# kazuto1011/dusty-gan-v2

Hardware: AMD Instinct MI355X
Metric: range-images/sec (G+D step) on dusty_v2 64x512 (higher is better)
Workload: dtype bf16; 1 GPU; configs[2]: configs/gans/dusty_v2.yaml full G+D train step (G step + D step + lazy R1 + ADA + EMA + Adam), 64x512 synthetic; global_batch=64, per_gpu_batch=64, parallelism=dp1, hip_graph=True, d_epilogue_dtype=fp32, pe_table_precomputed=True

## Files before the change

dusty-gan-v2_amd/csrc/api.hip:

```cpp
#include "common.h"

extern "C" int dgv2_abi_version(void) { return 49; }
```

dusty-gan-v2_amd/csrc/common.h:

```cpp
#pragma once
#include <hip/hip_runtime.h>
#include <stdint.h>
#include <stdlib.h>

#include "../../include/dgv2.h"

typedef __bf16 bf16_t;
typedef __attribute__((ext_vector_type(8))) __bf16 bf16x8;
typedef __attribute__((ext_vector_type(4))) float f32x4;
typedef __attribute__((ext_vector_type(4))) short s16x4;
typedef __attribute__((ext_vector_type(8))) short s16x8;

#define DGV2_WAVE 64

template <int DT> struct dtype_of;
template <> struct dtype_of<DGV2_F32> { typedef float type; };
template <> struct dtype_of<DGV2_BF16> { typedef bf16_t type; };

__device__ __forceinline__ float to_f32(float v) { return v; }
__device__ __forceinline__ float to_f32(bf16_t v) { return (float)v; }
template <typename T> __device__ __forceinline__ T from_f32(float v);
template <> __device__ __forceinline__ float from_f32<float>(float v) { return v; }
template <> __device__ __forceinline__ bf16_t from_f32<bf16_t>(float v) { return (bf16_t)v; }

template <typename T> struct vec16 {
  static constexpr int N = 16 / sizeof(T);
  union {
    uint4 raw;
    T e[16 / sizeof(T)];
  };
  __device__ __forceinline__ void load(const T* p) { raw = *reinterpret_cast<const uint4*>(p); }
  __device__ __forceinline__ void store(T* p) const { *reinterpret_cast<uint4*>(p) = raw; }
  __device__ __forceinline__ void store_nt(T* p) const {
    typedef __attribute__((ext_vector_type(4))) unsigned u32x4;
    const u32x4 v = {raw.x, raw.y, raw.z, raw.w};
    __builtin_nontemporal_store(v, reinterpret_cast<u32x4*>(p));
  }
  __device__ __forceinline__ float get(int i) const { return to_f32(e[i]); }
  __device__ __forceinline__ void set(int i, float v) { e[i] = from_f32<T>(v); }
};

__device__ __forceinline__ int pack_pair_bf16(const float (&va)[4], const float (&vb)[4], int lc, uint4& out) {
  union { uint2 u; bf16_t e[4]; } pa, pb;
#pragma unroll
  for (int r = 0; r < 4; ++r) {
    pa.e[r] = (bf16_t)va[r];
    pb.e[r] = (bf16_t)vb[r];
  }
  const auto lo = __builtin_amdgcn_permlane16_swap(pa.u.x, pb.u.x, false, false);
  const auto hi = __builtin_amdgcn_permlane16_swap(pa.u.y, pb.u.y, false, false);
  out = make_uint4(lo[0], hi[0], lo[1], hi[1]);
  const bool odd = lc & 1;
  return odd ? 16 + 4 * (lc - 1) : 4 * lc;
}

struct fp8_t { uint8_t v; };
#define DGV2_FP8_MAX 448.0f
__device__ __forceinline__ uint2 pack_fp8x8(const float (&f)[8]) {
  float c[8];
#pragma unroll
  for (int i = 0; i < 8; ++i) c[i] = fminf(fmaxf(f[i], -DGV2_FP8_MAX), DGV2_FP8_MAX);
  int lo = __builtin_amdgcn_cvt_pk_fp8_f32(c[0], c[1], 0, false);
  lo = __builtin_amdgcn_cvt_pk_fp8_f32(c[2], c[3], lo, true);
  int hi = __builtin_amdgcn_cvt_pk_fp8_f32(c[4], c[5], 0, false);
  hi = __builtin_amdgcn_cvt_pk_fp8_f32(c[6], c[7], hi, true);
  return make_uint2((unsigned)lo, (unsigned)hi);
}
__device__ __forceinline__ void unpack_fp8x4(unsigned w, float (&f)[4]) {
  typedef __attribute__((ext_vector_type(2))) float f32x2_;
  const f32x2_ a = __builtin_amdgcn_cvt_pk_f32_fp8((int)w, false), b = __builtin_amdgcn_cvt_pk_f32_fp8((int)w, true);
  f[0] = a[0]; f[1] = a[1]; f[2] = b[0]; f[3] = b[1];
}

static inline bool aligned16(const void* p) { return (reinterpret_cast<uintptr_t>(p) & 15) == 0; }

__host__ __device__ __forceinline__ int floordiv(int a, int b) {
  int q = a / b;
  return (a % b != 0 && ((a < 0) != (b < 0))) ? q - 1 : q;
}
__host__ __device__ __forceinline__ int floormod(int a, int b) {
  int r = a % b;
  return r < 0 ? r + b : r;
}

__device__ __forceinline__ float wave_sum(float v) {
#pragma unroll
  for (int o = 32; o > 0; o >>= 1) v += __shfl_xor(v, o, 64);
  return v;
}

__device__ __forceinline__ float block_sum(float v, float* red) {
  v = wave_sum(v);
  if ((threadIdx.x & 63) == 0) red[threadIdx.x >> 6] = v;
  __syncthreads();
  float s = 0.f;
  if (threadIdx.x == 0)
    for (int i = 0; i < (int)(blockDim.x >> 6); ++i) s += red[i];
  return s;
}

__device__ __forceinline__ float sumsq_bf16x8(uint4 q) {
  const unsigned w[4] = {q.x, q.y, q.z, q.w};
  float s = 0.f;
#pragma unroll
  for (int i = 0; i < 4; ++i) {
    const float lo = __uint_as_float(w[i] << 16), hi = __uint_as_float(w[i] & 0xffff0000u);
    s = fmaf(lo, lo, s);
    s = fmaf(hi, hi, s);
  }
  return s;
}

#define DGV2_RETURN_LAST()                 \
  do {                                     \
    hipError_t e__ = hipGetLastError();    \
    return (int)e__;                       \
  } while (0)

#define DGV2_DISPATCH_DTYPE(dtype, ...)                      \
  do {                                                       \
    if ((dtype) == DGV2_F32) {                               \
      typedef float T;                                       \
      __VA_ARGS__;                                           \
    } else if ((dtype) == DGV2_BF16) {                       \
      typedef bf16_t T;                                      \
      __VA_ARGS__;                                           \
    } else {                                                 \
      return DGV2_EINVAL;                                    \
    }                                                        \
  } while (0)

static __global__ void dgv2_zero_kernel(uint32_t* __restrict__ p, size_t n) {
  for (size_t i = blockIdx.x * (size_t)blockDim.x + threadIdx.x; i < n; i += (size_t)gridDim.x * blockDim.x) p[i] = 0u;
}
static inline hipError_t dgv2_zero_async(void* p, size_t bytes, hipStream_t st) {
  const size_t n = bytes / 4;
  if (n == 0) return hipSuccess;
  size_t g = (n + 255) / 256;
  if (g > 1024) g = 1024;
  dgv2_zero_kernel<<<(int)g, 256, 0, st>>>(reinterpret_cast<uint32_t*>(p), n);
  return hipGetLastError();
}
#define hipMemsetAsync(p, value, bytes, st) dgv2_zero_async((p), (bytes), (st))

static inline bool nt_output(int64_t bytes) {
  static const int64_t min_mb = getenv("DGV2_NT_MIN_MB") ? atoll(getenv("DGV2_NT_MIN_MB")) : 64;
  return min_mb > 0 && bytes >= (min_mb << 20);
}

static inline int grid_for(int64_t work, int block, int cap = 256 * 16) {
  int64_t g = (work + block - 1) / block;
  if (g > cap) g = cap;
  if (g < 1) g = 1;
  return (int)g;
}
```

dusty-gan-v2_amd/csrc/fir_mfma.hip:

```cpp
#include <type_traits>

#include "gemm_core.h"

namespace {

constexpr int FM_CT = 32;
constexpr int FM_CB = 32;
constexpr int FM_WIN = FM_CT + 16;
#ifndef DGV2_FIR_RS
#define DGV2_FIR_RS 8
#endif
constexpr int FM_RS = DGV2_FIR_RS;
constexpr int FM_RING = 2 * FM_RS;
static_assert(FM_RS == 8 || FM_RS == 4, "rows per step");
constexpr int FM_XBYTES = FM_RS * FM_WIN * 64;
constexpr int FM_ZROW = 2048 + 64;
constexpr int FM_ZBYTES = FM_RING * FM_ZROW;
constexpr int FM_YROW = 2048 + 16;
constexpr int FM_YBYTES = FM_RS * FM_YROW;
constexpr int FM_NLD = FM_RS * FM_WIN * 4 / 256;

struct FMGeom {
  int B, C, H, W, nt;
  const uint4* bands;
  const bf16_t* ref;
  float alpha, ascale;
  float* partial;
  uint8_t* y8;
};

struct FMTabs {
  int H, W, Eh, Ew;
  const int* idx_h; const float* coef_h; const int* cnt_h;
  const int* idx_w; const float* coef_w; const int* cnt_w;
  int* err;
};

typedef __attribute__((ext_vector_type(4))) unsigned fm_u32x4;
typedef __attribute__((address_space(3))) s16x4 fm_lds_s16x4;

__device__ __forceinline__ unsigned fm_pack2(float a, float b) {
  union { bf16_t h[2]; unsigned u; } p;
  p.h[0] = (bf16_t)a;
  p.h[1] = (bf16_t)b;
  return p.u;
}

__global__ __launch_bounds__(64) void fir_bands_kernel(uint4* __restrict__ bands, FMTabs t) {
  const int lane = threadIdx.x, li = lane & 15, kg = lane >> 4;
  const int nh = t.H / FM_RS + 1;
  float v[8];
#pragma unroll
  for (int j = 0; j < 8; ++j) v[j] = 0.f;
  bool bad = false;
  if ((int)blockIdx.x < nh) {
    const int s = blockIdx.x, ho = s * FM_RS - FM_RS / 2 + li;
    if (li < FM_RS && ho >= 0 && ho < t.H) {
      const int n = t.cnt_h[ho];
      for (int e = 0; e < n; ++e) {
        const int r = t.idx_h[ho * t.Eh + e];
        const float cf = t.coef_h[ho * t.Eh + e];
        if (r < s * FM_RS - FM_RS || r >= s * FM_RS + FM_RS || r < 0 || r >= t.H) bad = true;
#pragma unroll
        for (int j = 0; j < 8; ++j)
          if ((r & (FM_RING - 1)) == 8 * kg + j) v[j] += cf;
      }
    }
  } else {
    const int wt = blockIdx.x - nh, wo = 16 * wt + li;
    const int n = t.cnt_w[wo];
    for (int e = 0; e < n; ++e) {
      int rel = t.idx_w[wo * t.Ew + e] - (16 * wt - 8);
      rel = rel < 0 ? rel + t.W : (rel >= t.W ? rel - t.W : rel);
      const float cf = t.coef_w[wo * t.Ew + e];
      if ((unsigned)rel >= 32u) bad = true;
#pragma unroll
      for (int j = 0; j < 8; ++j)
        if (rel == 8 * kg + j) v[j] += cf;
    }
  }
#pragma unroll
  for (int j = 0; j < 8; ++j)
    if ((float)(bf16_t)v[j] != v[j]) bad = true;
  bands[(int64_t)blockIdx.x * 64 + lane] =
      make_uint4(fm_pack2(v[0], v[1]), fm_pack2(v[2], v[3]), fm_pack2(v[4], v[5]), fm_pack2(v[6], v[7]));
  if (bad) atomicOr(t.err, DGV2_STATUS_FIR_TABLE);
}

template <bool ACT>
__global__ __launch_bounds__(256, 2) void fir_same_mfma_kernel(bf16_t* __restrict__ y, const bf16_t* __restrict__ x, FMGeom g) {
  extern __shared__ __attribute__((aligned(16))) unsigned char smem[];
  unsigned char* Xs = smem;
  unsigned char* Zs = Xs + FM_XBYTES;
  unsigned char* Ys = Zs + FM_ZBYTES;
  const int tid = threadIdx.x, wave = tid >> 6, lane = tid & 63;
  const int li = lane & 15, kg = lane >> 4;
  const int q = li >> 2, p = li & 3;
  int vid = blockIdx.x + gridDim.x * (blockIdx.y + gridDim.y * blockIdx.z);
  {
    const int nblk = gridDim.x * gridDim.y * gridDim.z;
    if ((nblk & 7) == 0) vid = (vid & 7) * (nblk >> 3) + (vid >> 3);
  }
  const int c0col = (vid % (int)gridDim.x) * FM_CT;
  const int cb0 = ((vid / (int)gridDim.x) % (int)gridDim.y) * FM_CB;
  const int b = vid / (int)(gridDim.x * gridDim.y);
  const int64_t img = (int64_t)b * g.H * g.W * g.C;
  const bf16_t* xb = x + img;

  for (int i = tid; i < FM_ZBYTES / 16; i += 256) reinterpret_cast<uint4*>(Zs)[i] = make_uint4(0, 0, 0, 0);
  const int nsteps = g.H / FM_RS;
  const uint4* bands_h = g.bands;
  uint4 tw[2];
  tw[0] = g.bands[(int64_t)(nsteps + 1 + c0col / 16) * 64 + lane];
  tw[1] = g.bands[(int64_t)(nsteps + 2 + c0col / 16) * 64 + lane];

  int goff[FM_NLD];
  int xoff[FM_NLD];
#pragma unroll
  for (int i = 0; i < FM_NLD; ++i) {
    const int id = tid + 256 * i;
    const int o8 = id & 3, j = (id >> 2) % FM_WIN, r = id / (4 * FM_WIN);
    int gc = c0col - 8 + j;
    gc = gc < 0 ? gc + g.W : (gc >= g.W ? gc - g.W : gc);
    goff[i] = gc * g.C + cb0 + o8 * 8;
    xoff[i] = ((r * FM_WIN + j) * 4 + (o8 ^ (((j >> 3) & 1) << 1))) * 16;
  }
  fm_u32x4 rg[FM_NLD];
  auto issue = [&](int s) {
#pragma unroll
    for (int i = 0; i < FM_NLD; ++i) {
      const int r = (tid + 256 * i) / (4 * FM_WIN);
      rg[i] = *reinterpret_cast<const fm_u32x4*>(xb + (int64_t)(s * FM_RS + r) * g.W * g.C + goff[i]);
    }
  };
  auto commit = [&]() {
#pragma unroll
    for (int i = 0; i < FM_NLD; ++i) *reinterpret_cast<fm_u32x4*>(Xs + xoff[i]) = rg[i];
  };
  issue(0);
  commit();
  if (1 < nsteps) issue(1);
  uint4 th = bands_h[lane];
  __syncthreads();

  float bsum[8];
#pragma unroll
  for (int j = 0; j < 8; ++j) bsum[j] = 0.f;

  for (int s = 0; s <= nsteps; ++s) {
    if (s < nsteps) {
      uint4 af[FM_RS];
#pragma unroll
      for (int job = 0; job < FM_RS; ++job) {
        const int rr = job >> 2, ct = (job >> 1) & 1, wt = job & 1;
        const int r = (FM_RS / 4) * wave + rr;
        const int j = 16 * wt + 8 * kg + q;
        const int o8 = (2 * ct + (p >> 1)) ^ ((kg & 1) << 1);
        const unsigned char* a0 = Xs + ((r * FM_WIN + j) * 4 + o8) * 16 + (p & 1) * 8;
        union { uint4 u; s16x4 h[2]; } a;
        a.h[0] = __builtin_amdgcn_ds_read_tr16_b64_v4i16((fm_lds_s16x4*)a0);
        a.h[1] = __builtin_amdgcn_ds_read_tr16_b64_v4i16((fm_lds_s16x4*)(a0 + 4 * 64));
        af[job] = a.u;
      }
      f32x4 acc[FM_RS];
#pragma unroll
      for (int job = 0; job < FM_RS; ++job) {
        acc[job] = (f32x4){0.f, 0.f, 0.f, 0.f};
        Mfma16<bf16_t>::run(acc[job], af[job], tw[job & 1]);
      }
#pragma unroll
      for (int job = 0; job < FM_RS; ++job) {
        const int rr = job >> 2, ct = (job >> 1) & 1, wt = job & 1;
        const int slot = (s * FM_RS + (FM_RS / 4) * wave + rr) & (FM_RING - 1);
        const int wp = 16 * wt + li;
        const int u = (4 * ct + kg) ^ ((wp >> 2) & 7) ^ ((slot >> 3) << 2);
        uint2 pk = make_uint2(fm_pack2(acc[job][0], acc[job][1]), fm_pack2(acc[job][2], acc[job][3]));
        *reinterpret_cast<uint2*>(Zs + slot * FM_ZROW + wp * 64 + u * 8) = pk;
      }
    }
    __syncthreads();
    if (s + 1 < nsteps) commit();
    if (s + 2 < nsteps) issue(s + 2);
    const uint4 th_next = bands_h[(int64_t)min(s + 1, nsteps) * 64 + lane];
    vec16<bf16_t> fref[FM_RS / 2];
    if constexpr (ACT) {
#pragma unroll
      for (int i = 0; i < FM_RS / 2; ++i) {
        const int id = tid + 256 * i;
        const int ho = min(max(s * FM_RS - FM_RS / 2 + (id >> 7), 0), g.H - 1);
        fref[i].load(g.ref + img + ((int64_t)ho * g.W + c0col + ((id >> 2) & 31)) * g.C + cb0 + (id & 3) * 8);
      }
    }

    {
      uint4 af[16];
#pragma unroll
      for (int job = 0; job < 16; ++job) {
        const int wp = 8 * wave + (job >> 1), ct = job & 1;
        const int hi = FM_RS == 8 ? (kg & 1) : 0;
        const int slot = 8 * hi + q;
        const int u = (4 * ct + p) ^ ((wp >> 2) & 7) ^ (hi << 2);
        const unsigned char* a0 = Zs + slot * FM_ZROW + wp * 64 + u * 8;
        union { uint4 u4; s16x4 h[2]; } a;
        a.h[0] = __builtin_amdgcn_ds_read_tr16_b64_v4i16((fm_lds_s16x4*)a0);
        a.h[1] = __builtin_amdgcn_ds_read_tr16_b64_v4i16((fm_lds_s16x4*)(a0 + 4 * FM_ZROW));
        af[job] = a.u4;
      }
      f32x4 acc[16];
#pragma unroll
      for (int job = 0; job < 16; ++job) {
        acc[job] = (f32x4){0.f, 0.f, 0.f, 0.f};
        Mfma16<bf16_t>::run(acc[job], af[job], th);
      }
      if (li < FM_RS) {
#pragma unroll
        for (int job = 0; job < 16; ++job) {
          const int wp = 8 * wave + (job >> 1), ct = job & 1;
          uint2 pk = make_uint2(fm_pack2(acc[job][0], acc[job][1]), fm_pack2(acc[job][2], acc[job][3]));
          *reinterpret_cast<uint2*>(Ys + li * FM_YROW + wp * 64 + (4 * ct + kg) * 8) = pk;
        }
      }
    }
    __syncthreads();

#pragma unroll
    for (int i = 0; i < FM_RS / 2; ++i) {
      const int id = tid + 256 * i;
      const int o8 = id & 3, px = (id >> 2) & 31, n = id >> 7;
      const int ho = s * FM_RS - FM_RS / 2 + n;
      if (ho < 0 || ho >= g.H) continue;
      vec16<bf16_t> o;
      o.raw = *reinterpret_cast<const uint4*>(Ys + n * FM_YROW + px * 64 + o8 * 16);
      const int64_t off = img + ((int64_t)ho * g.W + c0col + px) * g.C + cb0 + o8 * 8;
      if constexpr (ACT) {
#pragma unroll
        for (int j = 0; j < 8; ++j) {
          const float a = o.get(j);
          o.set(j, (fref[i].get(j) > 0.f ? a : a * g.alpha) * g.ascale);
          bsum[j] += o.get(j);
        }
      }
      if constexpr (!ACT) {
        if (g.y8) {
          float f[8];
#pragma unroll
          for (int j = 0; j < 8; ++j) f[j] = o.get(j);
          *reinterpret_cast<uint2*>(g.y8 + off) = pack_fp8x8(f);
          continue;
        }
      }
      if (g.nt) o.store_nt(y + off);
      else o.store(y + off);
    }
    th = th_next;
  }

  if constexpr (ACT) {
    float* fold = reinterpret_cast<float*>(Xs);
    __syncthreads();
#pragma unroll
    for (int j = 0; j < 8; ++j) fold[tid * 8 + j] = bsum[j];
    __syncthreads();
    if (tid < FM_CB) {
      const int o8 = tid >> 3, j = tid & 7;
      float s2 = 0.f;
      for (int t = o8; t < 256; t += 4) s2 += fold[t * 8 + j];
      g.partial[((int64_t)b * gridDim.x + c0col / FM_CT) * g.C + cb0 + tid] = s2;
    }
  }
}

__global__ __launch_bounds__(256) void fm_bias_reduce_kernel(float* __restrict__ gb, const float* __restrict__ partial,
                                                             int nblk, int C) {
  __shared__ float red[16];
  const int c = blockIdx.x;
  float s = 0.f;
#pragma unroll 4
  for (int k = threadIdx.x; k < nblk; k += 256) s += partial[(int64_t)k * C + c];
  s = block_sum(s, red);
  if (threadIdx.x == 0) gb[c] = s;
}

bool fm_covers(int B, int C, int H, int W) {
  return B > 0 && C % FM_CB == 0 && H % FM_RS == 0 && H >= FM_RS && W % FM_CT == 0 && W >= FM_CT && B < 65536 &&
         C / FM_CB < 65536;
}

constexpr size_t FM_LDS = (size_t)FM_XBYTES + FM_ZBYTES + FM_YBYTES;

int64_t fm_band_bytes(int H, int W) { return 1024 * ((int64_t)H / FM_RS + 1 + W / 16); }

}

extern "C" int dgv2_fir_same_mfma_prep(void* bands, int64_t bands_bytes, int64_t* bytes_needed, const int* idx_h,
                                       const float* coef_h, const int* cnt_h, int Eh, const int* idx_w, const float* coef_w,
                                       const int* cnt_w, int Ew, int H, int W, int* status, void* stream) {
  if (H < FM_RS || H % FM_RS || W < FM_CT || W % FM_CT || Eh < 1 || Ew < 1) return DGV2_ENOTSUP;
  const int64_t need = fm_band_bytes(H, W);
  if (bytes_needed) *bytes_needed = need;
  if (!bands) return bytes_needed ? 0 : DGV2_EINVAL;
  if (bands_bytes < need || !aligned16(bands) || !idx_h || !coef_h || !cnt_h || !idx_w || !coef_w || !cnt_w) return DGV2_EINVAL;
  if (!status) return DGV2_EINVAL;
  FMTabs t{H, W, Eh, Ew, idx_h, coef_h, cnt_h, idx_w, coef_w, cnt_w, status};
  fir_bands_kernel<<<(int)(need / 1024), 64, 0, (hipStream_t)stream>>>((uint4*)bands, t);
  DGV2_RETURN_LAST();
}

extern "C" int dgv2_fir_same_mfma(void* y, const void* x, const void* bands, int B, int C, int H, int W, void* stream) {
  if (!y || !x || !bands) return DGV2_EINVAL;
  if (!fm_covers(B, C, H, W)) return DGV2_ENOTSUP;
  if (!aligned16(x) || !aligned16(y) || !aligned16(bands)) return DGV2_EINVAL;
  FMGeom g{B, C, H, W, nt_output((int64_t)B * H * W * C * 2) ? 1 : 0, (const uint4*)bands, nullptr, 1.f, 1.f, nullptr, nullptr};
  auto kern = fir_same_mfma_kernel<false>;
  if (FM_LDS > 64 * 1024) {
    hipError_t e = hipFuncSetAttribute((const void*)kern, hipFuncAttributeMaxDynamicSharedMemorySize, (int)FM_LDS);
    if (e != hipSuccess) return (int)e;
  }
  kern<<<dim3(W / FM_CT, C / FM_CB, B), 256, FM_LDS, (hipStream_t)stream>>>((bf16_t*)y, (const bf16_t*)x, g);
  DGV2_RETURN_LAST();
}

extern "C" int dgv2_fir_same_mfma_q8(void* y8, const void* x, const void* bands, int B, int C, int H, int W, void* stream) {
  if (!y8 || !x || !bands) return DGV2_EINVAL;
  if (!fm_covers(B, C, H, W)) return DGV2_ENOTSUP;
  if (!aligned16(x) || (reinterpret_cast<uintptr_t>(y8) & 7) || !aligned16(bands)) return DGV2_EINVAL;
  FMGeom g{B, C, H, W, 0, (const uint4*)bands, nullptr, 1.f, 1.f, nullptr, (uint8_t*)y8};
  auto kern = fir_same_mfma_kernel<false>;
  if (FM_LDS > 64 * 1024) {
    hipError_t e = hipFuncSetAttribute((const void*)kern, hipFuncAttributeMaxDynamicSharedMemorySize, (int)FM_LDS);
    if (e != hipSuccess) return (int)e;
  }
  kern<<<dim3(W / FM_CT, C / FM_CB, B), 256, FM_LDS, (hipStream_t)stream>>>((bf16_t*)nullptr, (const bf16_t*)x, g);
  DGV2_RETURN_LAST();
}

extern "C" int dgv2_fir_same_mfma_actbwd(void* y, float* gb, float* scratch, int64_t scratch_elems, int64_t* blocks_needed,
                                         const void* x, const void* ref, const void* bands, int B, int C, int H, int W,
                                         float alpha, float scale, void* stream) {
  if (!fm_covers(B, C, H, W)) return DGV2_ENOTSUP;
  const int64_t blocks = (int64_t)B * (W / FM_CT);
  if (blocks_needed) *blocks_needed = blocks;
  if (!scratch) return blocks_needed ? 0 : DGV2_EINVAL;
  if (!y || !gb || !x || !ref || !bands) return DGV2_EINVAL;
  if (scratch_elems < blocks * C || !aligned16(x) || !aligned16(y) || !aligned16(ref) || !aligned16(bands)) return DGV2_EINVAL;
  FMGeom g{B, C, H, W, 0, (const uint4*)bands, (const bf16_t*)ref, alpha, scale, scratch, nullptr};
  auto kern = fir_same_mfma_kernel<true>;
  if (FM_LDS > 64 * 1024) {
    hipError_t e = hipFuncSetAttribute((const void*)kern, hipFuncAttributeMaxDynamicSharedMemorySize, (int)FM_LDS);
    if (e != hipSuccess) return (int)e;
  }
  hipStream_t st = (hipStream_t)stream;
  kern<<<dim3(W / FM_CT, C / FM_CB, B), 256, FM_LDS, st>>>((bf16_t*)y, (const bf16_t*)x, g);
  fm_bias_reduce_kernel<<<C, 256, 0, st>>>(gb, scratch, (int)blocks, C);
  DGV2_RETURN_LAST();
}
```

dusty-gan-v2_amd/csrc/resample.hip:

```cpp
#include "common.h"

namespace {

constexpr int MAXE = 32;
constexpr int TH = 4;
constexpr int TW = 16;

struct AxisParams {
  int L;
  int Lo;
  int k, up, down, p0;
  int wrap;
};

struct SparseRow {
  int cnt;
  int idx[MAXE];
  float coef[MAXE];
};

__device__ __forceinline__ int extend(int j, int L, int wrap) {
  if (wrap) return floormod(j, L);
  return j < 0 ? 0 : (j >= L ? L - 1 : j);
}
// ... 109 lines not shown
extern "C" int dgv2_resample(void* y, const void* x, const float* taps_h, const float* taps_w, int B, int H, int W,
                             int C, int Ho, int Wo, int ldx, int ldy, int kh, int up_h, int down_h, int p0_h, int kw,
                             int up_w, int down_w, int p0_w, int ring, int adjoint, int dtype, void* stream) {
  if (!y || !x || !taps_h || !taps_w) return DGV2_EINVAL;
  if (B <= 0 || H <= 0 || W <= 0 || C <= 0 || Ho <= 0 || Wo <= 0) return DGV2_EINVAL;
  if (kh < 1 || kh > 8 || kw < 1 || kw > 8 || up_h < 1 || up_w < 1 || down_h < 1 || down_w < 1) return DGV2_EINVAL;
  if (ldx < C || ldy < C) return DGV2_EINVAL;
  AxisParams ah = {H, Ho, kh, up_h, down_h, p0_h, 0};
  AxisParams aw = {W, Wo, kw, up_w, down_w, p0_w, ring ? 1 : 0};
  const int in_h = adjoint ? Ho : H, in_w = adjoint ? Wo : W;
  const int out_h = adjoint ? H : Ho, out_w = adjoint ? W : Wo;
  const int tiles = B * ((out_h + TH - 1) / TH) * ((out_w + TW - 1) / TW);
  hipStream_t st = (hipStream_t)stream;
  DGV2_DISPATCH_DTYPE(dtype, {
    constexpr int VN = vec16<T>::N;
    const bool vec = (C % VN == 0) && (ldx % VN == 0) && (ldy % VN == 0) && aligned16(x) && aligned16(y);
    if (vec)
      resample_kernel<T, true><<<tiles, 256, 0, st>>>((T*)y, (const T*)x, taps_h, taps_w, B, C, ldx, ldy, ah, aw,
                                                     adjoint, in_h, in_w, out_h, out_w);
    else
      resample_kernel<T, false><<<tiles, 256, 0, st>>>((T*)y, (const T*)x, taps_h, taps_w, B, C, ldx, ldy, ah, aw,
                                                      adjoint, in_h, in_w, out_h, out_w);
  });
  DGV2_RETURN_LAST();
}

namespace {

template <typename T, int CC>
__global__ __launch_bounds__(256) void resample_tab_smallc_kernel(
    T* __restrict__ y, const T* __restrict__ x, const int* __restrict__ idx_h, const float* __restrict__ coef_h,
    const int* __restrict__ cnt_h, int Eh, const int* __restrict__ idx_w, const float* __restrict__ coef_w,
    const int* __restrict__ cnt_w, int Ew, int B, int in_h, int in_w, int out_h, int out_w,
    const T* __restrict__ resid = nullptr, const float* __restrict__ rscale = nullptr,
    const float* __restrict__ rbias = nullptr) {
  struct alignas(sizeof(T) * CC) Px { T e[CC]; };
  float rs[CC], rb[CC];
#pragma unroll
  for (int j = 0; j < CC; ++j) {
    rs[j] = rscale ? rscale[j] : 1.f;
    rb[j] = rbias ? rbias[j] : 0.f;
  }
  const int64_t total = (int64_t)B * out_h * out_w;
  for (int64_t t = blockIdx.x * (int64_t)blockDim.x + threadIdx.x; t < total; t += (int64_t)gridDim.x * blockDim.x) {
    const int wo = (int)(t % out_w);
    const int64_t r = t / out_w;
    const int ho = (int)(r % out_h);
    const int b = (int)(r / out_h);
    const int nh = cnt_h[ho], nw = cnt_w[wo];
    const Px* xb = reinterpret_cast<const Px*>(x) + (int64_t)b * in_h * in_w;
    float acc[CC];
#pragma unroll
    for (int j = 0; j < CC; ++j) acc[j] = 0.f;
    if (Eh <= 2 && Ew <= 2) {
      const int e1h = Eh > 1 ? 1 : 0, e1w = Ew > 1 ? 1 : 0;
      const int ih0 = idx_h[ho * Eh], ih1 = idx_h[ho * Eh + e1h], iw0 = idx_w[wo * Ew], iw1 = idx_w[wo * Ew + e1w];
      const float ch0 = coef_h[ho * Eh], ch1 = coef_h[ho * Eh + e1h], cw0 = coef_w[wo * Ew], cw1 = coef_w[wo * Ew + e1w];
      const bool h1 = nh > 1, w1 = nw > 1;
      const Px* r0 = xb + (int64_t)ih0 * in_w;
      const Px* r1 = xb + (int64_t)(h1 ? ih1 : ih0) * in_w;
      const Px v00 = r0[iw0], v01 = r0[w1 ? iw1 : iw0], v10 = r1[iw0], v11 = r1[w1 ? iw1 : iw0];
      const bool l0 = nh > 0 && nw > 0;
#pragma unroll
      for (int j = 0; j < CC; ++j) {
        float s = 0.f;
        if (l0) s += (ch0 * cw0) * to_f32(v00.e[j]);
        if (l0 && w1) s += (ch0 * cw1) * to_f32(v01.e[j]);
        if (l0 && h1) s += (ch1 * cw0) * to_f32(v10.e[j]);
        if (l0 && h1 && w1) s += (ch1 * cw1) * to_f32(v11.e[j]);
        acc[j] = s;
      }
    } else {
      for (int a = 0; a < nh; ++a) {
        const float fa = coef_h[ho * Eh + a];
        const Px* xr = xb + (int64_t)idx_h[ho * Eh + a] * in_w;
        for (int c = 0; c < nw; ++c) {
          const float cf = fa * coef_w[wo * Ew + c];
          const Px v = xr[idx_w[wo * Ew + c]];
#pragma unroll
          for (int j = 0; j < CC; ++j) acc[j] += cf * to_f32(v.e[j]);
        }
      }
    }
    Px o;
    if (resid) {
      const Px rv = reinterpret_cast<const Px*>(resid)[t];
#pragma unroll
      for (int j = 0; j < CC; ++j) {
        const float rj = rscale ? to_f32(from_f32<T>(fmaf(to_f32(rv.e[j]), rs[j], rb[j]))) : to_f32(rv.e[j]);
        o.e[j] = from_f32<T>(rj + to_f32(from_f32<T>(acc[j])));
      }
    } else {
#pragma unroll
      for (int j = 0; j < CC; ++j) o.e[j] = from_f32<T>(acc[j]);
    }
    reinterpret_cast<Px*>(y)[t] = o;
  }
}

template <typename T, bool VEC>
__global__ __launch_bounds__(256) void resample_tab_kernel(
    T* __restrict__ y, const T* __restrict__ x, const int* __restrict__ idx_h, const float* __restrict__ coef_h,
    const int* __restrict__ cnt_h, int Eh, const int* __restrict__ idx_w, const float* __restrict__ coef_w,
    const int* __restrict__ cnt_w, int Ew, int B, int C, int ldx, int ldy, int in_h, int in_w, int out_h, int out_w) {
  constexpr int VN = VEC ? vec16<T>::N : 1;
  const int cvecs = (C + VN - 1) / VN;
  const int64_t total = (int64_t)B * out_h * out_w * cvecs;
  for (int64_t t = blockIdx.x * (int64_t)blockDim.x + threadIdx.x; t < total; t += (int64_t)gridDim.x * blockDim.x) {
    const int cv = (int)(t % cvecs);
    int64_t r = t / cvecs;
    const int wo = (int)(r % out_w);
    r /= out_w;
    const int ho = (int)(r % out_h);
    const int b = (int)(r / out_h);
    const int nh = cnt_h[ho], nw = cnt_w[wo];
    const int* ih = idx_h + ho * Eh;
    const float* ch = coef_h + ho * Eh;
    const int* iw = idx_w + wo * Ew;
    const float* cw = coef_w + wo * Ew;
    const T* xb = x + (int64_t)b * in_h * in_w * ldx + cv * VN;
    float acc[VN];
#pragma unroll
    for (int j = 0; j < VN; ++j) acc[j] = 0.f;
    for (int a = 0; a < nh; ++a) {
      const float fa = ch[a];
      const T* xr = xb + (int64_t)ih[a] * in_w * ldx;
      for (int c = 0; c < nw; ++c) {
        const float cf = fa * cw[c];
        const T* p = xr + iw[c] * ldx;
        if (VEC) {
          vec16<T> v;
          v.load(p);
#pragma unroll
          for (int j = 0; j < VN; ++j) acc[j] += cf * v.get(j);
        } else {
          acc[0] += cf * to_f32(p[0]);
        }
      }
    }
    T* q = y + (((int64_t)b * out_h + ho) * out_w + wo) * ldy + cv * VN;
    if (VEC) {
      vec16<T> o;
#pragma unroll
      for (int j = 0; j < VN; ++j) o.set(j, acc[j]);
      o.store(q);
    } else {
      q[0] = from_f32<T>(acc[0]);
    }
  }
}

constexpr int RS_RB = 4;

template <typename T, int EW, bool ACT = false>
__global__ __launch_bounds__(256) void resample_stream_kernel(
    T* __restrict__ y, const T* __restrict__ x, const int* __restrict__ idx_h, const float* __restrict__ coef_h,
    const int* __restrict__ cnt_h, int Eh, const int* __restrict__ idx_w, const float* __restrict__ coef_w,
    const int* __restrict__ cnt_w, int Ew, int B, int C, int ldx, int ldy, int in_h, int in_w, int out_h, int out_w,
    int SHA, float* __restrict__ sumsq, const T* __restrict__ ref = nullptr, float alpha = 1.f, float ascale = 1.f,
    float* __restrict__ bias_partial = nullptr, uint8_t* __restrict__ y8 = nullptr) {
#ifdef DGV2_ABLATE
  const int SH = SHA & 0xffff, ablate = (SHA >> 16) & 0xff;
#else
  const int SH = SHA & 0xffff;
  constexpr int ablate = 0;
#endif
  const bool nt = (SHA >> 30) & 1;
  __shared__ float red[16];
  float ss = 0.f;
  constexpr int VN = vec16<T>::N;
  __shared__ uint4 ring[RS_RB][256];
  const int tid = threadIdx.x;
  const int cvecs = C / VN;
  const int rowvecs = out_w * cvecs;
  const int colblocks = (rowvecs + 255) / 256;
  const int strips = (out_h + SH - 1) / SH;
  int bid = blockIdx.x;
  const int cb = bid % colblocks; bid /= colblocks;
  const int strip = bid % strips;
  const int b = bid / strips;
  const int col = cb * 256 + tid;
  const bool live = col < rowvecs;
  const int wo = live ? col / cvecs : 0;
  const int cv = live ? col - wo * cvecs : 0;

  const int nw = live ? cnt_w[wo] : 0;
  int xo[EW];
  float cw[EW];
  const int xo_any = nw > 0 ? idx_w[wo * Ew] * ldx + cv * VN : 0;
#pragma unroll
  for (int c = 0; c < EW; ++c) {
    xo[c] = xo_any;
    cw[c] = 0.f;
    if (c < nw) {
      xo[c] = idx_w[wo * Ew + c] * ldx + cv * VN;
      cw[c] = coef_w[wo * Ew + c];
    }
  }
  const T* xb = x + (int64_t)b * in_h * in_w * ldx;
  T* yp = y + (int64_t)b * out_h * out_w * ldy + (int64_t)wo * ldy + cv * VN;
  const T* rp = ACT ? ref + (int64_t)b * out_h * out_w * ldy + (int64_t)wo * ldy + cv * VN : nullptr;
  float bsum[VN];
#pragma unroll
  for (int j = 0; j < VN; ++j) bsum[j] = 0.f;
  const int ho0 = strip * SH;
  const int ho1 = min(ho0 + SH, out_h);
  int t0 = -1, t1 = -1, t2 = -1, t3 = -1;
  const int lane = threadIdx.x & 63;
  const int nent = (ho1 - ho0) * Eh;
  const int tb_idx = lane < nent ? idx_h[ho0 * Eh + lane] : 0;
  const float tb_cf = lane < nent ? coef_h[ho0 * Eh + lane] : 0.f;
  const int tb_cnt = lane < ho1 - ho0 ? cnt_h[ho0 + lane] : 0;
  int rlast = -1;
  for (int i = 0; i < ho1 - ho0; ++i) {
    const int n = __builtin_amdgcn_readlane(tb_cnt, i);
    for (int a = 0; a < n; ++a) rlast = max(rlast, __builtin_amdgcn_readlane(tb_idx, i * Eh + a));
  }
  int pr = -1;
  vec16<T> pv[EW];
  auto issue = [&](int r) {
    const T* xr = xb + (int64_t)r * in_w * ldx;
#pragma unroll
    for (int c = 0; c < EW; ++c) pv[c].load(xr + xo[c]);
    pr = r;
  };
  for (int ho = ho0; ho < ho1; ++ho) {
    const int n = __builtin_amdgcn_readlane(tb_cnt, ho - ho0);
    float acc[VN];
#pragma unroll
    for (int j = 0; j < VN; ++j) acc[j] = 0.f;
    for (int a = 0; a < n; ++a) {
      const int e = (ho - ho0) * Eh + a;
      const int r = __builtin_amdgcn_readlane(tb_idx, e);
      const float fa = __int_as_float(__builtin_amdgcn_readlane(__float_as_int(tb_cf), e));
      const int s = r & (RS_RB - 1);
      const int tag = s == 0 ? t0 : (s == 1 ? t1 : (s == 2 ? t2 : t3));
      if (tag != r) {
        if (pr != r && !(ablate & 2)) issue(r);
        float h[VN];
#pragma unroll
        for (int j = 0; j < VN; ++j) h[j] = 0.f;
#pragma unroll
        for (int c = 0; c < EW; ++c)
#pragma unroll
          for (int j = 0; j < VN; ++j) h[j] += cw[c] * pv[c].get(j);
        if (r + 1 <= rlast && !(ablate & 2)) issue(r + 1); else pr = -1;
        {
          vec16<T> hv;
#pragma unroll
          for (int j = 0; j < VN; ++j) hv.set(j, h[j]);
          ring[s][tid] = hv.raw;
        }
        t0 = s == 0 ? r : t0; t1 = s == 1 ? r : t1; t2 = s == 2 ? r : t2; t3 = s == 3 ? r : t3;
      }
      {
        vec16<T> hv;
        hv.raw = ring[s][tid];
#pragma unroll
        for (int j = 0; j < VN; ++j) acc[j] += fa * hv.get(j);
      }
    }
    if (live && !((ablate & 1) && acc[0] != 12345.678f)) {
      vec16<T> o;
      if constexpr (ACT) {
        vec16<T> f;
        f.load(rp + (int64_t)ho * out_w * ldy);
#pragma unroll
        for (int j = 0; j < VN; ++j) {
          o.set(j, (f.get(j) > 0.f ? acc[j] : acc[j] * alpha) * ascale);
          bsum[j] += o.get(j);
        }
      } else {
#pragma unroll
        for (int j = 0; j < VN; ++j) o.set(j, acc[j]);
      }
      if (y) {
        if (nt) o.store_nt(yp + (int64_t)ho * out_w * ldy);
        else o.store(yp + (int64_t)ho * out_w * ldy);
      }
      if constexpr (!ACT && sizeof(T) == 2) {
        if (y8) {
          float f[8];
#pragma unroll
          for (int j = 0; j < 8; ++j) f[j] = acc[j];
          *reinterpret_cast<uint2*>(y8 + ((int64_t)b * out_h + ho) * out_w * ldy + (int64_t)wo * ldy + cv * VN) = pack_fp8x8(f);
        }
      }
      if (sumsq) {
#pragma unroll
        for (int j = 0; j < VN; ++j) ss = fmaf(o.get(j), o.get(j), ss);
      }
    }
  }
  if (sumsq) {
    const float s = block_sum(ss, red);
    if (tid == 0) sumsq[blockIdx.x] = s;
  }
  if constexpr (ACT) {
    float* fold = reinterpret_cast<float*>(&ring[0][0]);
    __syncthreads();
#pragma unroll
    for (int j = 0; j < VN; ++j) fold[tid * VN + j] = live ? bsum[j] : 0.f;
    __syncthreads();
    const int off = (cb * 256) % cvecs;
    for (int c = tid; c < C; c += 256) {
      const int v = c / VN, j = c - v * VN;
      float s2 = 0.f;
      for (int t = (v - off + cvecs) % cvecs; t < 256; t += cvecs) s2 += fold[t * VN + j];
      bias_partial[(int64_t)blockIdx.x * C + c] = s2;
    }
  }
}

template <typename T>
void rs_launch(int Ew, int blocks, hipStream_t st, T* y, const T* x, const int* idx_h, const float* coef_h,
               const int* cnt_h, int Eh, const int* idx_w, const float* coef_w, const int* cnt_w, int B, int C, int ldx,
               int ldy, int in_h, int in_w, int out_h, int out_w, int sha, float* sumsq) {
  switch (Ew) {
    case 1: resample_stream_kernel<T, 1><<<blocks, 256, 0, st>>>(y, x, idx_h, coef_h, cnt_h, Eh, idx_w, coef_w, cnt_w, Ew, B, C, ldx, ldy, in_h, in_w, out_h, out_w, sha, sumsq); break;
    case 2: resample_stream_kernel<T, 2><<<blocks, 256, 0, st>>>(y, x, idx_h, coef_h, cnt_h, Eh, idx_w, coef_w, cnt_w, Ew, B, C, ldx, ldy, in_h, in_w, out_h, out_w, sha, sumsq); break;
    case 3: resample_stream_kernel<T, 3><<<blocks, 256, 0, st>>>(y, x, idx_h, coef_h, cnt_h, Eh, idx_w, coef_w, cnt_w, Ew, B, C, ldx, ldy, in_h, in_w, out_h, out_w, sha, sumsq); break;
    default: resample_stream_kernel<T, 4><<<blocks, 256, 0, st>>>(y, x, idx_h, coef_h, cnt_h, Eh, idx_w, coef_w, cnt_w, Ew, B, C, ldx, ldy, in_h, in_w, out_h, out_w, sha, sumsq); break;
  }
}

template <typename T>
void rs_launch_act(int Ew, int blocks, hipStream_t st, T* y, const T* x, const int* idx_h, const float* coef_h,
                   const int* cnt_h, int Eh, const int* idx_w, const float* coef_w, const int* cnt_w, int B, int C,
                   int ldx, int ldy, int in_h, int in_w, int out_h, int out_w, int sha, const T* ref, float alpha,
                   float ascale, float* partial) {
  switch (Ew) {
    case 1: resample_stream_kernel<T, 1, true><<<blocks, 256, 0, st>>>(y, x, idx_h, coef_h, cnt_h, Eh, idx_w, coef_w, cnt_w, Ew, B, C, ldx, ldy, in_h, in_w, out_h, out_w, sha, nullptr, ref, alpha, ascale, partial); break;
    case 2: resample_stream_kernel<T, 2, true><<<blocks, 256, 0, st>>>(y, x, idx_h, coef_h, cnt_h, Eh, idx_w, coef_w, cnt_w, Ew, B, C, ldx, ldy, in_h, in_w, out_h, out_w, sha, nullptr, ref, alpha, ascale, partial); break;
    case 3: resample_stream_kernel<T, 3, true><<<blocks, 256, 0, st>>>(y, x, idx_h, coef_h, cnt_h, Eh, idx_w, coef_w, cnt_w, Ew, B, C, ldx, ldy, in_h, in_w, out_h, out_w, sha, nullptr, ref, alpha, ascale, partial); break;
    default: resample_stream_kernel<T, 4, true><<<blocks, 256, 0, st>>>(y, x, idx_h, coef_h, cnt_h, Eh, idx_w, coef_w, cnt_w, Ew, B, C, ldx, ldy, in_h, in_w, out_h, out_w, sha, nullptr, ref, alpha, ascale, partial); break;
  }
}

__global__ __launch_bounds__(256) void rs_bias_reduce_kernel(float* __restrict__ gb, const float* __restrict__ partial,
                                                             int nblk, int C) {
  __shared__ float red[16];
  const int c = blockIdx.x;
  float s = 0.f;
#pragma unroll 4
  for (int k = threadIdx.x; k < nblk; k += 256) s += partial[(int64_t)k * C + c];
  s = block_sum(s, red);
  if (threadIdx.x == 0) gb[c] = s;
}

}

extern "C" int dgv2_resample_tab_actbwd(void* y, float* gb, float* scratch, int64_t scratch_elems, int64_t* blocks_needed,
                                        const void* x, const void* ref, const int* idx_h, const float* coef_h,
                                        const int* cnt_h, int Eh, const int* idx_w, const float* coef_w,
                                        const int* cnt_w, int Ew, int B, int C, int in_h, int in_w, int out_h,
                                        int out_w, float alpha, float scale, int dtype, void* stream) {
  if (B <= 0 || C <= 0 || in_h <= 0 || in_w <= 0 || out_h <= 0 || out_w <= 0 || Eh <= 0 || Ew <= 0) return DGV2_EINVAL;
  const int vn = dtype == DGV2_BF16 ? 8 : (dtype == DGV2_F32 ? 4 : 0);
  if (!vn) return DGV2_EINVAL;
  if (C % vn || 256 % (C / vn) || Ew > 4 || Eh > 64) return DGV2_ENOTSUP;
  int SH = out_h >= 32 ? 16 : (out_h >= 8 ? 8 : out_h);
  while (SH > 1 && SH * Eh > 64) SH >>= 1;
  const int64_t blocks = (int64_t)B * ((out_h + SH - 1) / SH) * (((int64_t)out_w * (C / vn) + 255) / 256);
  if (blocks >= (1LL << 31)) return DGV2_ENOTSUP;
  if (blocks_needed) *blocks_needed = blocks;
  if (!scratch) return blocks_needed ? 0 : DGV2_EINVAL;
  if (!y || !gb || !x || !ref || !idx_h || !coef_h || !cnt_h || !idx_w || !coef_w || !cnt_w) return DGV2_EINVAL;
  if (scratch_elems < blocks * C || !aligned16(x) || !aligned16(y) || !aligned16(ref)) return DGV2_EINVAL;
  hipStream_t st = (hipStream_t)stream;
  DGV2_DISPATCH_DTYPE(dtype, {
    rs_launch_act<T>(Ew, (int)blocks, st, (T*)y, (const T*)x, idx_h, coef_h, cnt_h, Eh, idx_w, coef_w, cnt_w, B, C, C, C,
                     in_h, in_w, out_h, out_w, SH, (const T*)ref, alpha, scale, scratch);
  });
  rs_bias_reduce_kernel<<<C, 256, 0, st>>>(gb, scratch, (int)blocks, C);
  DGV2_RETURN_LAST();
}

extern "C" int dgv2_resample_tab(void* y, const void* x, const int* idx_h, const float* coef_h, const int* cnt_h,
                                 int Eh, const int* idx_w, const float* coef_w, const int* cnt_w, int Ew, int B,
                                 int C, int ldx, int ldy, int in_h, int in_w, int out_h, int out_w, int dtype,
                                 void* stream) {
  return dgv2_resample_tab_sq(y, x, idx_h, coef_h, cnt_h, Eh, idx_w, coef_w, cnt_w, Ew, B, C, ldx, ldy, in_h, in_w, out_h,
                              out_w, dtype, nullptr, 0, nullptr, stream);
}

extern "C" int dgv2_resample_tab_add(void* y, const void* x, const void* resid, const int* idx_h, const float* coef_h,
                                     const int* cnt_h, int Eh, const int* idx_w, const float* coef_w, const int* cnt_w,
                                     int Ew, int B, int C, int in_h, int in_w, int out_h, int out_w, int dtype,
                                     void* stream) {
  return dgv2_resample_tab_add_affine(y, x, resid, nullptr, nullptr, idx_h, coef_h, cnt_h, Eh, idx_w, coef_w, cnt_w, Ew, B, C,
                                      in_h, in_w, out_h, out_w, dtype, stream);
}

extern "C" int dgv2_resample_tab_add_affine(void* y, const void* x, const void* resid, const float* rscale,
                                            const float* rbias, const int* idx_h, const float* coef_h, const int* cnt_h,
                                            int Eh, const int* idx_w, const float* coef_w, const int* cnt_w, int Ew, int B,
                                            int C, int in_h, int in_w, int out_h, int out_w, int dtype, void* stream) {
  if ((!rscale) != (!rbias)) return DGV2_EINVAL;
  if (!y || !x || !resid || !idx_h || !coef_h || !cnt_h || !idx_w || !coef_w || !cnt_w) return DGV2_EINVAL;
  if (B <= 0 || C <= 0 || in_h <= 0 || in_w <= 0 || out_h <= 0 || out_w <= 0 || Eh <= 0 || Ew <= 0) return DGV2_EINVAL;
  if (!(C == 1 || C == 2 || C == 4)) return DGV2_ENOTSUP;
  hipStream_t st = (hipStream_t)stream;
  DGV2_DISPATCH_DTYPE(dtype, {
    const uintptr_t al = sizeof(T) * C;
    if (reinterpret_cast<uintptr_t>(x) % al || reinterpret_cast<uintptr_t>(y) % al || reinterpret_cast<uintptr_t>(resid) % al)
      return DGV2_ENOTSUP;
    const int g2 = grid_for((int64_t)B * out_h * out_w, 256, 256 * 64);
    if (C == 1) resample_tab_smallc_kernel<T, 1><<<g2, 256, 0, st>>>((T*)y, (const T*)x, idx_h, coef_h, cnt_h, Eh, idx_w, coef_w, cnt_w, Ew, B, in_h, in_w, out_h, out_w, (const T*)resid, rscale, rbias);
    else if (C == 2) resample_tab_smallc_kernel<T, 2><<<g2, 256, 0, st>>>((T*)y, (const T*)x, idx_h, coef_h, cnt_h, Eh, idx_w, coef_w, cnt_w, Ew, B, in_h, in_w, out_h, out_w, (const T*)resid, rscale, rbias);
    else resample_tab_smallc_kernel<T, 4><<<g2, 256, 0, st>>>((T*)y, (const T*)x, idx_h, coef_h, cnt_h, Eh, idx_w, coef_w, cnt_w, Ew, B, in_h, in_w, out_h, out_w, (const T*)resid, rscale, rbias);
  });
  DGV2_RETURN_LAST();
}

extern "C" int dgv2_resample_tab_q8(void* y8, const void* x, const int* idx_h, const float* coef_h, const int* cnt_h,
                                    int Eh, const int* idx_w, const float* coef_w, const int* cnt_w, int Ew, int B,
                                    int C, int in_h, int in_w, int out_h, int out_w, void* stream) {
  if (!y8 || !x || !idx_h || !coef_h || !cnt_h || !idx_w || !coef_w || !cnt_w) return DGV2_EINVAL;
  if (B <= 0 || C <= 0 || in_h <= 0 || in_w <= 0 || out_h <= 0 || out_w <= 0 || Eh <= 0 || Ew <= 0) return DGV2_EINVAL;
  if ((C & 7) || Ew > 4 || Eh > 64 || !aligned16(x) || (reinterpret_cast<uintptr_t>(y8) & 7)) return DGV2_ENOTSUP;
  typedef bf16_t T;
  int SH = out_h >= 32 ? 16 : (out_h >= 8 ? 8 : out_h);
  while (SH > 1 && SH * Eh > 64) SH >>= 1;
  const int64_t blocks = (int64_t)B * ((out_h + SH - 1) / SH) * (((int64_t)out_w * (C / 8) + 255) / 256);
  if (blocks >= (1LL << 31)) return DGV2_EINVAL;
  hipStream_t st = (hipStream_t)stream;
  uint8_t* q = (uint8_t*)y8;
#define DGV2_RS_Q8(EW)                                                                                                   \
  resample_stream_kernel<T, EW><<<(int)blocks, 256, 0, st>>>((T*)nullptr, (const T*)x, idx_h, coef_h, cnt_h, Eh, idx_w,   \
                                                            coef_w, cnt_w, Ew, B, C, C, C, in_h, in_w, out_h, out_w, SH,  \
                                                            nullptr, nullptr, 1.f, 1.f, nullptr, q)
  switch (Ew) {
    case 1: DGV2_RS_Q8(1); break;
    case 2: DGV2_RS_Q8(2); break;
    case 3: DGV2_RS_Q8(3); break;
    default: DGV2_RS_Q8(4); break;
  }
#undef DGV2_RS_Q8
  DGV2_RETURN_LAST();
}

extern "C" int dgv2_resample_tab_sq(void* y, const void* x, const int* idx_h, const float* coef_h, const int* cnt_h,
                                    int Eh, const int* idx_w, const float* coef_w, const int* cnt_w, int Ew, int B,
                                    int C, int ldx, int ldy, int in_h, int in_w, int out_h, int out_w, int dtype,
                                    float* sumsq, int sumsq_cap, int* sumsq_used, void* stream) {
  if (sumsq_used) *sumsq_used = 0;
  const bool stat_only = !y;
  if ((stat_only && !(sumsq && sumsq_used)) || !x || !idx_h || !coef_h || !cnt_h || !idx_w || !coef_w || !cnt_w) return DGV2_EINVAL;
  if (B <= 0 || C <= 0 || in_h <= 0 || in_w <= 0 || out_h <= 0 || out_w <= 0 || Eh <= 0 || Ew <= 0) return DGV2_EINVAL;
  if (ldx < C || ldy < C) return DGV2_EINVAL;
  hipStream_t st = (hipStream_t)stream;
  DGV2_DISPATCH_DTYPE(dtype, {
    constexpr int VN = vec16<T>::N;
    const bool vec = (C % VN == 0) && (ldx % VN == 0) && (ldy % VN == 0) && aligned16(x) && aligned16(y);
    if (stat_only && !(vec && Ew <= 4 && Eh <= 64)) return DGV2_ENOTSUP;
    const int64_t total = (int64_t)B * out_h * out_w * ((C + (vec ? VN : 1) - 1) / (vec ? VN : 1));
    const int grid = grid_for(total, 256, 256 * 64);
    static const bool no_stream = getenv("DGV2_NO_RSTREAM") != nullptr;
#ifdef DGV2_ABLATE
    static const int rs_ablate = getenv("DGV2_RS_ABLATE") ? atoi(getenv("DGV2_RS_ABLATE")) : 0;
#else
    constexpr int rs_ablate = 0;
#endif
    if (vec && Ew <= 4 && Eh <= 64 && (!no_stream || stat_only)) {
      static const int sh_env = getenv("DGV2_RS_SH") ? atoi(getenv("DGV2_RS_SH")) : 0;
      int SH = out_h >= 32 ? 16 : (out_h >= 8 ? 8 : out_h);
      if (sh_env > 0 && sh_env < SH) SH = sh_env;
      while (SH > 1 && SH * Eh > 64) SH >>= 1;
      const int64_t blocks = (int64_t)B * ((out_h + SH - 1) / SH) * (((int64_t)out_w * (C / VN) + 255) / 256);
      if (blocks >= (1LL << 31)) return DGV2_EINVAL;
      float* sq = (sumsq && sumsq_used && blocks <= sumsq_cap) ? sumsq : nullptr;
      if (stat_only && !sq) return DGV2_ENOTSUP;
      if (sq) *sumsq_used = (int)blocks;
      rs_launch<T>(Ew, (int)blocks, st, (T*)y, (const T*)x, idx_h, coef_h, cnt_h, Eh, idx_w, coef_w, cnt_w, B, C, ldx, ldy, in_h,
                   in_w, out_h, out_w,
                   SH | (rs_ablate << 16) | ((y && nt_output((int64_t)B * out_h * out_w * C * sizeof(T))) ? (1 << 30) : 0), sq);
    } else if (!vec && (C == 1 || C == 2 || C == 4) && ldx == C && ldy == C &&
               (reinterpret_cast<uintptr_t>(x) % (sizeof(T) * C)) == 0 && (reinterpret_cast<uintptr_t>(y) % (sizeof(T) * C)) == 0) {
      const int g2 = grid_for((int64_t)B * out_h * out_w, 256, 256 * 64);
      if (C == 1) resample_tab_smallc_kernel<T, 1><<<g2, 256, 0, st>>>((T*)y, (const T*)x, idx_h, coef_h, cnt_h, Eh, idx_w, coef_w, cnt_w, Ew, B, in_h, in_w, out_h, out_w);
      else if (C == 2) resample_tab_smallc_kernel<T, 2><<<g2, 256, 0, st>>>((T*)y, (const T*)x, idx_h, coef_h, cnt_h, Eh, idx_w, coef_w, cnt_w, Ew, B, in_h, in_w, out_h, out_w);
      else resample_tab_smallc_kernel<T, 4><<<g2, 256, 0, st>>>((T*)y, (const T*)x, idx_h, coef_h, cnt_h, Eh, idx_w, coef_w, cnt_w, Ew, B, in_h, in_w, out_h, out_w);
    } else if (vec)
      resample_tab_kernel<T, true><<<grid, 256, 0, st>>>((T*)y, (const T*)x, idx_h, coef_h, cnt_h, Eh, idx_w, coef_w,
                                                        cnt_w, Ew, B, C, ldx, ldy, in_h, in_w, out_h, out_w);
    else
      resample_tab_kernel<T, false><<<grid, 256, 0, st>>>((T*)y, (const T*)x, idx_h, coef_h, cnt_h, Eh, idx_w, coef_w,
                                                         cnt_w, Ew, B, C, ldx, ldy, in_h, in_w, out_h, out_w);
  });
  DGV2_RETURN_LAST();
}
```

dusty-gan-v2_amd/csrc/stem.hip:

```cpp
#include "common.h"

namespace {

struct StemGeom {
  int B, H, W, O, ring;
  float alpha, scale;
  int nt;
};

__device__ __forceinline__ int stem_wcoord(int w, int W, int ring) {
  if (ring) return w < 0 ? w + W : (w >= W ? w - W : w);
  return w < 0 ? 0 : (w >= W ? W - 1 : w);
}

__device__ __forceinline__ void stem_blur(const float* __restrict__ xb, int h, int w, const StemGeom& g, float& v,
                                          float& u) {
  const float c = xb[h * g.W + w];
  const float up = xb[(h > 0 ? h - 1 : 0) * g.W + w], dn = xb[(h + 1 < g.H ? h + 1 : g.H - 1) * g.W + w];
  const float lf = xb[h * g.W + stem_wcoord(w - 1, g.W, g.ring)], rt = xb[h * g.W + stem_wcoord(w + 1, g.W, g.ring)];
  v = 0.25f * (up + dn) + 0.5f * c;
  u = 0.25f * (lf + rt) + 0.5f * c;
}

template <typename T>
__global__ __launch_bounds__(256) void stem_fwd_kernel(T* __restrict__ y, const float* __restrict__ x,
                                                       const float* __restrict__ w, const float* __restrict__ bias,
                                                       StemGeom g) {
  const int G = g.O / 8;
  const int64_t items = (int64_t)g.B * g.H * g.W * G;
  const int64_t stride = (int64_t)gridDim.x * blockDim.x;
  int64_t i = (int64_t)blockIdx.x * blockDim.x + threadIdx.x;
  const int grp = (int)(i % G);
  float w0[8], w1[8], bs[8];
#pragma unroll
  for (int j = 0; j < 8; ++j) {
    w0[j] = w[(grp * 8 + j) * 2];
    w1[j] = w[(grp * 8 + j) * 2 + 1];
    bs[j] = bias ? bias[grp * 8 + j] : 0.f;
  }
  const int HW = g.H * g.W;
  for (; i < items; i += stride) {
    const int64_t px = i / G;
    const int b = (int)(px / HW), r = (int)(px - (int64_t)b * HW);
    const int h = r / g.W, wc = r - h * g.W;
    float v, u;
    stem_blur(x + (int64_t)b * HW, h, wc, g, v, u);
    T* out = y + px * g.O + grp * 8;
    float f[8];
#pragma unroll
    for (int j = 0; j < 8; ++j) {
      const float t = w0[j] * v + w1[j] * u + bs[j];
      f[j] = (t > 0.f ? t : t * g.alpha) * g.scale;
    }
    if constexpr (sizeof(T) == 2) {
      vec16<T> o;
#pragma unroll
      for (int j = 0; j < 8; ++j) o.set(j, f[j]);
      if (g.nt) o.store_nt(out);
      else o.store(out);
    } else {
      *reinterpret_cast<float4*>(out) = make_float4(f[0], f[1], f[2], f[3]);
      *reinterpret_cast<float4*>(out + 4) = make_float4(f[4], f[5], f[6], f[7]);
    }
  }
}

template <typename T>
__global__ __launch_bounds__(256) void stem_fwd4_kernel(T* __restrict__ y, const float* __restrict__ x,
                                                        const float* __restrict__ w, const float* __restrict__ bias,
                                                        StemGeom g) {
  const int G = g.O / 8, W4 = g.W >> 2;
  const int64_t items = (int64_t)g.B * g.H * W4 * G;
  const int64_t stride = (int64_t)gridDim.x * blockDim.x;
  int64_t i = (int64_t)blockIdx.x * blockDim.x + threadIdx.x;
  const int grp = (int)(i % G);
  float w0[8], w1[8], bs[8];
#pragma unroll
  for (int j = 0; j < 8; ++j) {
    w0[j] = w[(grp * 8 + j) * 2];
    w1[j] = w[(grp * 8 + j) * 2 + 1];
    bs[j] = bias ? bias[grp * 8 + j] : 0.f;
  }
  const int HW4 = g.H * W4;
  for (; i < items; i += stride) {
    const int64_t q = i / G;
    const int b = (int)(q / HW4), r = (int)(q - (int64_t)b * HW4);
    const int h = r / W4, wc = (r - h * W4) << 2;
    const float* xb = x + ((int64_t)b * g.H) * g.W;
    const float4 c4 = *reinterpret_cast<const float4*>(xb + h * g.W + wc);
    const float4 u4 = *reinterpret_cast<const float4*>(xb + (h > 0 ? h - 1 : 0) * g.W + wc);
    const float4 d4 = *reinterpret_cast<const float4*>(xb + (h + 1 < g.H ? h + 1 : g.H - 1) * g.W + wc);
    const float lf = xb[h * g.W + stem_wcoord(wc - 1, g.W, g.ring)], rt = xb[h * g.W + stem_wcoord(wc + 4, g.W, g.ring)];
    const float c[6] = {lf, c4.x, c4.y, c4.z, c4.w, rt};
    const float up[4] = {u4.x, u4.y, u4.z, u4.w}, dn[4] = {d4.x, d4.y, d4.z, d4.w};
    T* out = y + (((int64_t)b * g.H + h) * g.W + wc) * g.O + grp * 8;
#pragma unroll
    for (int k = 0; k < 4; ++k) {
      const float v = 0.25f * (up[k] + dn[k]) + 0.5f * c[k + 1];
      const float u = 0.25f * (c[k] + c[k + 2]) + 0.5f * c[k + 1];
      float f[8];
#pragma unroll
      for (int j = 0; j < 8; ++j) {
        const float t = w0[j] * v + w1[j] * u + bs[j];
        f[j] = (t > 0.f ? t : t * g.alpha) * g.scale;
      }
      if constexpr (sizeof(T) == 2) {
        vec16<T> o;
#pragma unroll
        for (int j = 0; j < 8; ++j) o.set(j, f[j]);
        if (g.nt) o.store_nt(out + k * g.O);
        else o.store(out + k * g.O);
      } else {
        *reinterpret_cast<float4*>(out + k * g.O) = make_float4(f[0], f[1], f[2], f[3]);
        *reinterpret_cast<float4*>(out + k * g.O + 4) = make_float4(f[4], f[5], f[6], f[7]);
      }
    }
  }
}

template <typename T>
struct StemSkip {
  const T* gsk;
  const int* idx_h; const float* coef_h; const int* cnt_h; int Eh;
  const int* idx_w; const float* coef_w; const int* cnt_w; int Ew;
  int Hs, Ws;
};

template <typename T, bool SKIP>
__global__ __launch_bounds__(256) void stem_bwd_kernel(float* __restrict__ partial, float* __restrict__ gxb,
                                                       const T* __restrict__ gy, const T* __restrict__ y,
                                                       const float* __restrict__ x, const float* __restrict__ w,
                                                       StemGeom g, StemSkip<T> sk) {
  __shared__ float red[4][8][24];
  extern __shared__ __attribute__((aligned(16))) unsigned char stem_tabs[];
  const int* t_ih = nullptr; const float* t_ch = nullptr; const int* t_iw = nullptr; const float* t_cw = nullptr;
  if constexpr (SKIP) {
    const int nh_ = g.H * sk.Eh, nw_ = g.W * sk.Ew;
    int* a0 = reinterpret_cast<int*>(stem_tabs);
    float* a1 = reinterpret_cast<float*>(a0 + nh_);
    int* a2 = reinterpret_cast<int*>(a1 + nh_);
    float* a3 = reinterpret_cast<float*>(a2 + nw_);
    for (int t = threadIdx.x; t < nh_; t += 256) {
      a0[t] = sk.idx_h[t];
      a1[t] = sk.coef_h[t];
    }
    for (int t = threadIdx.x; t < nw_; t += 256) {
      a2[t] = sk.idx_w[t];
      a3[t] = sk.coef_w[t];
    }
    __syncthreads();
    t_ih = a0; t_ch = a1; t_iw = a2; t_cw = a3;
  }
  const int G = g.O / 8;
  const int64_t items = (int64_t)g.B * g.H * g.W * G;
  const int64_t stride = (int64_t)gridDim.x * blockDim.x;
  int64_t i = (int64_t)blockIdx.x * blockDim.x + threadIdx.x;
  const int grp = (int)(i % G);
  float w0[8], w1[8];
#pragma unroll
  for (int j = 0; j < 8; ++j) {
    w0[j] = w[(grp * 8 + j) * 2];
    w1[j] = w[(grp * 8 + j) * 2 + 1];
  }
  float acc[24];
#pragma unroll
  for (int j = 0; j < 24; ++j) acc[j] = 0.f;
  const int HW = g.H * g.W;
  const int64_t nloop = (items + stride - 1) / stride;
  for (int64_t it = 0; it < nloop; ++it, i += stride) {
    const bool live = i < items;
    const int64_t px = live ? i / G : 0;
    const int b = (int)(px / HW), r = (int)(px - (int64_t)b * HW);
    const int h = r / g.W, wc = r - h * g.W;
    float v, u;
    stem_blur(x + (int64_t)b * HW, h, wc, g, v, u);
    float gp[8], gs[8];
#pragma unroll
    for (int j = 0; j < 8; ++j) gs[j] = 0.f;
    if constexpr (SKIP) {
      const T* sb = sk.gsk + (int64_t)b * sk.Hs * sk.Ws * g.O + grp * 8;
      const int* ihp = t_ih + h * sk.Eh;
      const float* chp = t_ch + h * sk.Eh;
      const int* iwp = t_iw + wc * sk.Ew;
      const float* cwp = t_cw + wc * sk.Ew;
      const int e1h = sk.Eh > 1 ? 1 : 0, e1w = sk.Ew > 1 ? 1 : 0;
      const float ch0 = chp[0], ch1 = sk.Eh > 1 ? chp[1] : 0.f, cw0 = cwp[0], cw1 = sk.Ew > 1 ? cwp[1] : 0.f;
      const T* r0 = sb + (int64_t)ihp[0] * sk.Ws * g.O;
      const T* r1 = sb + (int64_t)ihp[e1h] * sk.Ws * g.O;
      const int64_t c0 = (int64_t)iwp[0] * g.O, c1 = (int64_t)iwp[e1w] * g.O;
      auto acc8 = [&](const T* sp, float cf) {
        if constexpr (sizeof(T) == 2) {
          vec16<T> v8;
          v8.load(sp);
#pragma unroll
          for (int j = 0; j < 8; ++j) gs[j] = fmaf(cf, v8.get(j), gs[j]);
        } else {
#pragma unroll
          for (int j = 0; j < 8; ++j) gs[j] = fmaf(cf, (float)sp[j], gs[j]);
        }
      };
      acc8(r0 + c0, ch0 * cw0);
      acc8(r0 + c1, ch0 * cw1);
      acc8(r1 + c0, ch1 * cw0);
      acc8(r1 + c1, ch1 * cw1);
      for (int a = 0; a < sk.Eh; ++a)
        for (int c = 0; c < sk.Ew; ++c) {
          if (a < 2 && c < 2) continue;
          const float cf = chp[a] * cwp[c];
          if (cf != 0.f) acc8(sb + (int64_t)ihp[a] * sk.Ws * g.O + (int64_t)iwp[c] * g.O, cf);
        }
    }
    if constexpr (sizeof(T) == 2) {
      vec16<T> a, c;
      a.load(gy + px * g.O + grp * 8);
      c.load(y + px * g.O + grp * 8);
#pragma unroll
      for (int j = 0; j < 8; ++j) gp[j] = (a.get(j) + gs[j]) * (c.get(j) > 0.f ? 1.f : g.alpha) * g.scale;
    } else {
#pragma unroll
      for (int j = 0; j < 8; ++j) {
        const float a = gy[px * g.O + grp * 8 + j], c = y[px * g.O + grp * 8 + j];
        gp[j] = (a + gs[j]) * (c > 0.f ? 1.f : g.alpha) * g.scale;
      }
    }
    float s0 = 0.f, s1 = 0.f;
#pragma unroll
    for (int j = 0; j < 8; ++j) {
      const float p = live ? gp[j] : 0.f;
      acc[j] += p;
      acc[8 + j] += p * v;
      acc[16 + j] += p * u;
      s0 += p * w0[j];
      s1 += p * w1[j];
    }
    for (int o = 1; o < G; o <<= 1) {
      s0 += __shfl_xor(s0, o, 64);
      s1 += __shfl_xor(s1, o, 64);
    }
    if (live && grp == 0) *reinterpret_cast<float2*>(gxb + px * 2) = make_float2(s0, s1);
  }
  const int lane = threadIdx.x & 63, wave = threadIdx.x >> 6;
#pragma unroll
  for (int j = 0; j < 24; ++j) {
    float t = acc[j];
    for (int o = 32; o >= G; o >>= 1) t += __shfl_xor(t, o, 64);
    if (lane < G) red[wave][lane][j] = t;
  }
  __syncthreads();
  for (int t = threadIdx.x; t < G * 24; t += 256) {
    const int gi = t / 24, j = t % 24;
    const float s = red[0][gi][j] + red[1][gi][j] + red[2][gi][j] + red[3][gi][j];
    partial[(int64_t)blockIdx.x * 3 * g.O + (j / 8) * g.O + gi * 8 + (j & 7)] = s;
  }
}

__global__ __launch_bounds__(256) void stem_reduce_kernel(float* __restrict__ gw, float* __restrict__ gb,
                                                          const float* __restrict__ partial, int nblk, int O) {
  __shared__ float red[4];
  const int e = blockIdx.x;
  float s = 0.f;
  for (int k = threadIdx.x; k < nblk; k += 256) s += partial[(int64_t)k * 3 * O + e];
  s = wave_sum(s);
  if ((threadIdx.x & 63) == 0) red[threadIdx.x >> 6] = s;
  __syncthreads();
  if (threadIdx.x == 0) {
    const float t = red[0] + red[1] + red[2] + red[3];
    if (e < O) gb[e] = t;
    else gw[(e % O) * 2 + (e / O - 1)] = t;
  }
}

__global__ __launch_bounds__(256) void stem_blur_adj_kernel(float* __restrict__ gx, const float* __restrict__ gxb,
                                                            StemGeom g) {
  const int64_t n = (int64_t)g.B * g.H * g.W;
  const int HW = g.H * g.W;
  for (int64_t i = (int64_t)blockIdx.x * blockDim.x + threadIdx.x; i < n; i += (int64_t)gridDim.x * blockDim.x) {
    const int b = (int)(i / HW), r = (int)(i - (int64_t)b * HW);
    const int h = r / g.W, w = r - h * g.W;
    const float* gb = gxb + (int64_t)b * HW * 2;
    auto G0 = [&](int hh, int ww) { return gb[(hh * g.W + ww) * 2]; };
    auto G1 = [&](int hh, int ww) { return gb[(hh * g.W + ww) * 2 + 1]; };
    float s = 0.5f * G0(h, w);
    if (h > 0) s += 0.25f * G0(h - 1, w);
    if (h + 1 < g.H) s += 0.25f * G0(h + 1, w);
    if (h == 0) s += 0.25f * G0(0, w);
    if (h == g.H - 1) s += 0.25f * G0(g.H - 1, w);
    s += 0.5f * G1(h, w);
    if (g.ring) {
      s += 0.25f * (G1(h, w > 0 ? w - 1 : g.W - 1) + G1(h, w + 1 < g.W ? w + 1 : 0));
    } else {
      if (w > 0) s += 0.25f * G1(h, w - 1);
      if (w + 1 < g.W) s += 0.25f * G1(h, w + 1);
      if (w == 0) s += 0.25f * G1(h, 0);
      if (w == g.W - 1) s += 0.25f * G1(h, g.W - 1);
    }
    gx[i] = s;
  }
}

constexpr int STEM_BWD_BLOCKS = 1024;

bool stem_ok(int B, int H, int W, int O) {
  return B > 0 && H >= 2 && W >= 2 && (O == 8 || O == 16 || O == 32 || O == 64) && (int64_t)H * W < (1 << 30);
}

}

extern "C" int dgv2_stem_fwd(void* y, const float* x, const float* w, const float* bias, int B, int H, int W, int O,
                             int ring, float alpha, float scale, int ydtype, void* stream) {
  if (!y || !x || !w || !stem_ok(B, H, W, O) || !aligned16(y)) return DGV2_EINVAL;
  StemGeom g{B, H, W, O, ring, alpha, scale, nt_output((int64_t)B * H * W * O * (ydtype == DGV2_BF16 ? 2 : 4)) ? 1 : 0};
  hipStream_t st = (hipStream_t)stream;
  static const bool no4 = getenv("DGV2_STEM_NO4") != nullptr;
  if (W % 4 == 0 && aligned16(x) && !no4) {
    const int64_t items = (int64_t)B * H * (W / 4) * (O / 8);
    const int grid = grid_for(items, 256, 256 * 32);
    if (ydtype == DGV2_BF16) stem_fwd4_kernel<bf16_t><<<grid, 256, 0, st>>>((bf16_t*)y, x, w, bias, g);
    else if (ydtype == DGV2_F32) stem_fwd4_kernel<float><<<grid, 256, 0, st>>>((float*)y, x, w, bias, g);
    else return DGV2_EINVAL;
    DGV2_RETURN_LAST();
  }
  const int64_t items = (int64_t)B * H * W * (O / 8);
  const int grid = grid_for(items, 256, 256 * 32);
  if (ydtype == DGV2_BF16) stem_fwd_kernel<bf16_t><<<grid, 256, 0, st>>>((bf16_t*)y, x, w, bias, g);
  else if (ydtype == DGV2_F32) stem_fwd_kernel<float><<<grid, 256, 0, st>>>((float*)y, x, w, bias, g);
  else return DGV2_EINVAL;
  DGV2_RETURN_LAST();
}

extern "C" int dgv2_stem_bwd_scratch(int64_t* elems, int B, int H, int W, int O) {
  if (!elems || !stem_ok(B, H, W, O)) return DGV2_EINVAL;
  *elems = (int64_t)STEM_BWD_BLOCKS * 3 * O + (int64_t)B * H * W * 2;
  return 0;
}

extern "C" int dgv2_stem_bwd(float* gx, float* gw, float* gb, float* scratch, int64_t scratch_elems, const void* gy,
                             const void* y, const float* x, const float* w, int B, int H, int W, int O, int ring,
                             float alpha, float scale, int dtype, void* stream) {
  return dgv2_stem_bwd_skip(gx, gw, gb, scratch, scratch_elems, gy, y, x, w, nullptr, nullptr, nullptr, nullptr, 0, nullptr,
                            nullptr, nullptr, 0, 0, 0, B, H, W, O, ring, alpha, scale, dtype, stream);
}

extern "C" int dgv2_stem_bwd_skip(float* gx, float* gw, float* gb, float* scratch, int64_t scratch_elems, const void* gy,
                                  const void* y, const float* x, const float* w, const void* gsk, const int* idx_h,
                                  const float* coef_h, const int* cnt_h, int Eh, const int* idx_w, const float* coef_w,
                                  const int* cnt_w, int Ew, int Hs, int Ws, int B, int H, int W, int O, int ring,
                                  float alpha, float scale, int dtype, void* stream) {
  if (!gw || !gb || !scratch || !gy || !y || !x || !w || !stem_ok(B, H, W, O)) return DGV2_EINVAL;
  if (!aligned16(gy) || !aligned16(y) || !aligned16(scratch)) return DGV2_EINVAL;
  if (gsk && (!idx_h || !coef_h || !cnt_h || !idx_w || !coef_w || !cnt_w || Eh < 1 || Ew < 1 || Hs < 1 || Ws < 1 ||
              !aligned16(gsk)))
    return DGV2_EINVAL;
  const size_t tab_bytes = gsk ? 8 * ((size_t)H * Eh + (size_t)W * Ew) : 0;
  if (tab_bytes > 48 * 1024) return DGV2_ENOTSUP;
  const int64_t need = (int64_t)STEM_BWD_BLOCKS * 3 * O + (int64_t)B * H * W * 2;
  if (scratch_elems < need) return DGV2_EINVAL;
  StemGeom g{B, H, W, O, ring, alpha, scale, 0};
  const int64_t items = (int64_t)B * H * W * (O / 8);
  const int grid = grid_for(items, 256, STEM_BWD_BLOCKS);
  float* partial = scratch;
  float* gxb = scratch + (int64_t)STEM_BWD_BLOCKS * 3 * O;
  hipStream_t st = (hipStream_t)stream;
  if (dtype == DGV2_BF16) {
    StemSkip<bf16_t> sk{(const bf16_t*)gsk, idx_h, coef_h, cnt_h, Eh, idx_w, coef_w, cnt_w, Ew, Hs, Ws};
    if (gsk) stem_bwd_kernel<bf16_t, true><<<grid, 256, tab_bytes, st>>>(partial, gxb, (const bf16_t*)gy, (const bf16_t*)y, x, w, g, sk);
    else stem_bwd_kernel<bf16_t, false><<<grid, 256, 0, st>>>(partial, gxb, (const bf16_t*)gy, (const bf16_t*)y, x, w, g, sk);
  } else if (dtype == DGV2_F32) {
    StemSkip<float> sk{(const float*)gsk, idx_h, coef_h, cnt_h, Eh, idx_w, coef_w, cnt_w, Ew, Hs, Ws};
    if (gsk) stem_bwd_kernel<float, true><<<grid, 256, tab_bytes, st>>>(partial, gxb, (const float*)gy, (const float*)y, x, w, g, sk);
    else stem_bwd_kernel<float, false><<<grid, 256, 0, st>>>(partial, gxb, (const float*)gy, (const float*)y, x, w, g, sk);
  } else {
    return DGV2_EINVAL;
  }
  stem_reduce_kernel<<<3 * O, 256, 0, st>>>(gw, gb, partial, grid, O);
  if (gx) stem_blur_adj_kernel<<<grid_for((int64_t)B * H * W, 256, 4096), 256, 0, st>>>(gx, gxb, g);
  DGV2_RETURN_LAST();
}
```

dusty-gan-v2_amd/dgv2_native/__init__.py:

```python
import ctypes
import os

import torch

_HERE = os.path.dirname(os.path.abspath(__file__))
LIB_PATH = os.environ.get("DGV2_LIB_PATH") or os.path.join(os.path.dirname(_HERE), "lib", "libdgv2.so")

F32, BF16 = 0, 1
ABI_VERSION = 49

_c_int, _c_i64, _c_f32, _c_ptr = ctypes.c_int, ctypes.c_int64, ctypes.c_float, ctypes.c_void_p

SIGNATURES = {
    "dgv2_abi_version": [],
    "dgv2_fused_bias_act": [_c_ptr] * 4 + [_c_i64] * 3 + [_c_int, _c_int, _c_f32, _c_f32, _c_int, _c_ptr],
    "dgv2_bias_grad": [_c_ptr, _c_ptr, _c_i64, _c_i64, _c_i64, _c_int, _c_ptr],
    "dgv2_bias_act_bwd": [_c_ptr] * 4 + [_c_i64, _c_int, _c_f32, _c_f32, _c_ptr, _c_i64, _c_int, _c_ptr],
    "dgv2_bias_act_bwd_rs": [_c_ptr] * 4 + [_c_i64, _c_int, _c_f32, _c_f32, _c_ptr, _c_ptr, _c_i64, _c_int, _c_ptr],
    "dgv2_surface_normal": [_c_ptr, _c_ptr] + [_c_int] * 5 + [_c_ptr],
    "dgv2_mbstd_cat_fwd": [_c_ptr] * 3 + [_c_int] * 7 + [_c_ptr],
    "dgv2_mbstd_cat_bwd": [_c_ptr] * 3 + [_c_int] * 7 + [_c_ptr],
    "dgv2_gemm_x3": [_c_ptr, _c_ptr, _c_i64, _c_ptr, _c_ptr, _c_int, _c_int, _c_i64, _c_int, _c_int, _c_i64, _c_i64, _c_i64,
                     _c_int, _c_f32, _c_ptr],
    "dgv2_pe_wgrad_scratch": [_c_ptr] + [_c_int] * 4,
    "dgv2_pe_wgrad": [_c_ptr, _c_ptr, _c_i64, _c_ptr, _c_ptr] + [_c_int] * 4 + [_c_i64, _c_int, _c_ptr],
    "dgv2_mbstd_cat_fwd_x": [_c_ptr] * 3 + [_c_int] * 8 + [_c_ptr],
    "dgv2_mbstd_cat_bwd_x": [_c_ptr] * 3 + [_c_int] * 8 + [_c_ptr],
    "dgv2_scale_cast": [_c_ptr] * 3 + [_c_i64, _c_int, _c_int, _c_int, _c_ptr],
    "dgv2_upfirdn2d": [_c_ptr] * 3 + [_c_int] * 15 + [_c_ptr],
    "dgv2_resample": [_c_ptr] * 4 + [_c_int] * 19 + [_c_ptr],
    "dgv2_resample_tab": [_c_ptr] * 5 + [_c_int] + [_c_ptr] * 3 + [_c_int] * 10 + [_c_ptr],
    "dgv2_resample_tab_add": [_c_ptr] * 6 + [_c_int] + [_c_ptr] * 3 + [_c_int] * 8 + [_c_ptr],
    "dgv2_resample_tab_add_affine": [_c_ptr] * 8 + [_c_int] + [_c_ptr] * 3 + [_c_int] * 8 + [_c_ptr],
    "dgv2_fourier_feature": [_c_ptr] * 5 + [_c_int] * 8 + [_c_ptr],
    "dgv2_downsample_angle": [_c_ptr] * 4 + [_c_int] * 5 + [_c_ptr],
    "dgv2_bmm_nn": [_c_ptr] * 3 + [_c_int] * 6 + [_c_i64, _c_ptr, _c_int, _c_f32, _c_f32, _c_int, _c_int, _c_ptr],
    "dgv2_bmm_tn": [_c_ptr] * 3 + [_c_int] * 7 + [_c_ptr],
    "dgv2_bmm_nn_cat": [_c_ptr] * 4 + [_c_int] * 5 + [_c_ptr, _c_int, _c_f32, _c_f32, _c_int, _c_int, _c_ptr],
    "dgv2_bmm_nn_cat_sq": [_c_ptr] * 4 + [_c_int] * 5 + [_c_ptr, _c_ptr, _c_int, _c_f32, _c_f32, _c_int, _c_int, _c_ptr, _c_int, _c_ptr,
                           _c_ptr],
    "dgv2_bmm_nn_sq": [_c_ptr] * 3 + [_c_int] * 6 + [_c_i64, _c_ptr, _c_ptr, _c_int, _c_f32, _c_f32, _c_ptr, _c_int, _c_int, _c_ptr, _c_int,
                       _c_ptr, _c_ptr],
    "dgv2_modconv_pe_fwd": [_c_ptr] * 4 + [_c_int] * 5 + [_c_ptr, _c_int, _c_f32, _c_f32, _c_int, _c_ptr],
    "dgv2_modconv_pe_fwd_sq": [_c_ptr] * 4 + [_c_int] * 5 + [_c_ptr, _c_ptr, _c_int, _c_f32, _c_f32, _c_int, _c_ptr, _c_int, _c_ptr,
                               _c_ptr],
    "dgv2_modconv_pe_fwd_head": [_c_ptr] * 4 + [_c_int] * 5 + [_c_ptr, _c_ptr, _c_int, _c_f32, _c_f32, _c_int, _c_ptr, _c_int, _c_ptr,
                                 _c_ptr, _c_ptr, _c_ptr],
    "dgv2_kitti_rows": [_c_ptr, _c_ptr, _c_ptr, _c_int, _c_int, _c_ptr],
    "dgv2_kitti_project": [_c_ptr] * 4 + [_c_int] * 4 + [_c_f32, _c_f32, _c_int, _c_ptr],
    "dgv2_fps_scratch": [_c_ptr, _c_int, _c_int],
    "dgv2_fps": [_c_ptr] * 3 + [_c_int] * 3 + [_c_ptr],
    "dgv2_gather_points": [_c_ptr] * 3 + [_c_int] * 4 + [_c_ptr],
    "dgv2_gather_points_grad": [_c_ptr] * 3 + [_c_int] * 4 + [_c_ptr],
    "dgv2_chamfer_fwd": [_c_ptr] * 6 + [_c_int] * 3 + [_c_ptr],
    "dgv2_nn_search": [_c_ptr] * 4 + [_c_int] * 4 + [_c_ptr],
    "dgv2_chamfer_bwd": [_c_ptr] * 8 + [_c_int] * 3 + [_c_ptr],
    "dgv2_emd_approxmatch": [_c_ptr] * 4 + [_c_int] * 3 + [_c_ptr],
    "dgv2_emd_matchcost": [_c_ptr] * 4 + [_c_int] * 3 + [_c_ptr],
    "dgv2_emd_matchcost_grad": [_c_ptr] * 5 + [_c_int] * 3 + [_c_ptr],
    "dgv2_nsgan_loss": [_c_ptr, _c_ptr, _c_ptr, _c_int, _c_int, _c_f32, _c_ptr, _c_ptr, _c_ptr],
    "dgv2_modconv_pe_dgrad_actbwd": [_c_ptr, _c_ptr, _c_ptr, _c_i64] + [_c_ptr] * 5 + [_c_f32, _c_f32] + [_c_int] * 4 + [_c_ptr],
    "dgv2_colmean_lerp": [_c_ptr, _c_ptr, _c_int, _c_int, _c_i64, _c_f32, _c_ptr],
    "dgv2_d_tail_fwd": [_c_ptr] * 6 + [_c_int, _c_int] + [_c_f32] * 4 + [_c_ptr],
    "dgv2_d_tail_bwd": [_c_ptr] * 7 + [_c_int, _c_int] + [_c_f32] * 4 + [_c_ptr],
    "dgv2_rng_fill": [_c_ptr] * 5 + [_c_int, _c_ptr, _c_ptr],
    "dgv2_modconv_up_fwd": [_c_ptr] * 4 + [_c_int] * 7 + [_c_ptr] * 6 + [_c_int, _c_f32, _c_f32, _c_int, _c_ptr, _c_int, _c_ptr,
                            _c_ptr],
    "dgv2_modconv_up_t_lag": [_c_ptr] * 4 + [_c_f32] + [_c_ptr] * 4 + [_c_int] * 9 + [_c_ptr, _c_int, _c_ptr, _c_ptr],
    "dgv2_fir_same_mfma_q8": [_c_ptr] * 3 + [_c_int] * 4 + [_c_ptr],
    "dgv2_resample_tab_q8": [_c_ptr] * 5 + [_c_int] + [_c_ptr] * 3 + [_c_int] * 7 + [_c_ptr],
    "dgv2_fp8_quant_weights": [_c_ptr] * 6 + [_c_int] + [_c_ptr] * 3,
    "dgv2_fp8_dequant": [_c_ptr, _c_ptr, _c_i64, _c_f32, _c_ptr],
    "dgv2_conv_taps_fp8": [_c_ptr] * 4 + [_c_int] * 14 + [_c_ptr, _c_int, _c_ptr, _c_ptr, _c_int, _c_f32, _c_f32, _c_ptr],
    "dgv2_modconv_up_t": [_c_ptr] * 5 + [_c_f32] + [_c_int] * 9 + [_c_ptr],
    "dgv2_up2_lag_sumsq": [_c_ptr] * 5 + [_c_int] * 5 + [_c_ptr, _c_int, _c_ptr, _c_ptr],
    "dgv2_resample_tab_actbwd": [_c_ptr, _c_ptr, _c_ptr, _c_i64, _c_ptr, _c_ptr, _c_ptr] + [_c_ptr] * 3 + [_c_int] + [_c_ptr] * 3
                                + [_c_int] * 7 + [_c_f32, _c_f32, _c_int, _c_ptr],
    "dgv2_fir_same_mfma_prep": [_c_ptr, _c_i64, _c_ptr] + [_c_ptr] * 3 + [_c_int] + [_c_ptr] * 3 + [_c_int] * 3 + [_c_ptr, _c_ptr],
    "dgv2_fir_same_mfma": [_c_ptr] * 3 + [_c_int] * 4 + [_c_ptr],
    "dgv2_fir_same_mfma_actbwd": [_c_ptr, _c_ptr, _c_ptr, _c_i64, _c_ptr, _c_ptr, _c_ptr, _c_ptr] + [_c_int] * 4
                                 + [_c_f32, _c_f32, _c_ptr],
    "dgv2_resample_tab_sq": [_c_ptr] * 5 + [_c_int] + [_c_ptr] * 3 + [_c_int] * 10 + [_c_ptr, _c_int, _c_ptr, _c_ptr],
    "dgv2_bmm_tn_cat": [_c_ptr] * 4 + [_c_int] * 6 + [_c_ptr],
    "dgv2_lerp_list": [_c_ptr] * 3 + [_c_int, _c_f32, _c_ptr],
    "dgv2_adam_prep": [_c_ptr, _c_ptr, _c_f32, _c_f32, _c_ptr],
    "dgv2_adam_step": [_c_ptr] * 5 + [_c_int, _c_ptr] + [_c_f32] * 4 + [_c_ptr],
    "dgv2_pack2d": [_c_ptr] * 4 + [_c_int] * 3 + [_c_ptr],
    "dgv2_unpack2d": [_c_ptr] * 4 + [_c_int] * 3 + [_c_ptr],
    "dgv2_ema_scalar": [_c_ptr] * 3 + [_c_int] + [_c_f32] * 3 + [_c_int, _c_ptr, _c_int, _c_ptr],
    "dgv2_ema_scalar_group": [_c_ptr, _c_ptr, _c_int, _c_ptr, _c_int] + [_c_f32] * 3 + [_c_int, _c_ptr, _c_ptr],
    "dgv2_bmm_nn_small": [_c_ptr] * 4 + [_c_int] * 5 + [_c_ptr],
    "dgv2_bmm_nn_small_act": [_c_ptr] * 4 + [_c_int] * 4 + [_c_ptr, _c_ptr, _c_f32, _c_f32, _c_ptr, _c_ptr, _c_i64, _c_ptr, _c_int,
                              _c_ptr],
    "dgv2_bmm_tn_small": [_c_ptr] * 3 + [_c_int] * 5 + [_c_ptr],
    "dgv2_head_bwd": [_c_ptr] * 5 + [_c_i64] + [_c_ptr] * 7 + [_c_f32, _c_f32] + [_c_int] * 5 + [_c_ptr],
    "dgv2_transpose_list": [_c_ptr] * 5 + [_c_int] * 3 + [_c_ptr],
    "dgv2_mod_prep_all_fwd": [_c_ptr] * 13 + [_c_ptr, _c_int, _c_int, _c_ptr],
    "dgv2_mod_prep_all_bwd": [_c_ptr, _c_i64] + [_c_ptr] * 15 + [_c_ptr, _c_int, _c_int, _c_ptr, _c_i64, _c_ptr],
    "dgv2_mod_prep_all_bwd_scratch": [_c_ptr, _c_ptr, _c_ptr, _c_int, _c_int],
    "dgv2_mod_prep_fwd": [_c_ptr] * 8 + [_c_int] * 9 + [_c_ptr],
    "dgv2_mod_prep_bwd": [_c_ptr] * 11 + [_c_int] * 9 + [_c_ptr],
    "dgv2_sum_squares": [_c_ptr, _c_ptr, _c_i64, _c_int, _c_int, _c_int, _c_ptr],
    "dgv2_conv_fwd": [_c_ptr] * 3 + [_c_int] * 10 + [_c_ptr, _c_int, _c_f32, _c_f32, _c_int, _c_ptr],
    "dgv2_conv_taps": [_c_ptr] * 3 + [_c_int] * 17 + [_c_ptr] + [_c_int] * 3 + [_c_ptr, _c_ptr, _c_int, _c_f32, _c_f32, _c_int,
                                                                               _c_ptr],
    "dgv2_conv_taps_ex": [_c_ptr] * 3 + [_c_int] * 14 + [_c_ptr, _c_int, _c_int, _c_ptr, _c_int, _c_ptr] + [_c_int] * 3
    + [_c_ptr, _c_ptr, _c_int, _c_f32, _c_f32, _c_int, _c_ptr],
    "dgv2_conv_taps_ld": [_c_ptr, _c_int, _c_ptr, _c_ptr] + [_c_int] * 14 + [_c_ptr, _c_int, _c_int, _c_ptr, _c_int, _c_ptr] + [_c_int] * 3
    + [_c_ptr, _c_ptr, _c_int, _c_f32, _c_f32, _c_int, _c_ptr],
    "dgv2_conv_wgrad_direct": [_c_ptr] * 3 + [_c_int] * 10 + [_c_ptr],
    "dgv2_bmm_tn_stream_scratch": [_c_ptr] + [_c_int] * 6,
    "dgv2_bmm_tn_stream": [_c_ptr, _c_ptr, _c_i64, _c_ptr, _c_ptr] + [_c_int] * 6 + [_c_ptr],
    "dgv2_bmm_tn_stream_x": [_c_ptr, _c_ptr, _c_i64, _c_ptr, _c_ptr] + [_c_int] * 7 + [_c_ptr],
    "dgv2_bmm_tn_stream_ld": [_c_ptr, _c_i64, _c_ptr, _c_i64, _c_ptr, _c_ptr] + [_c_int] * 7 + [_c_ptr],
    "dgv2_conv_weight_bank": [_c_ptr] * 8 + [_c_int, _c_int, _c_ptr],
    "dgv2_conv_weight_bank_ex": [_c_ptr] * 10 + [_c_int, _c_int, _c_ptr],
    "dgv2_glin_fwd": [_c_ptr] * 6 + [_c_int] * 3 + [_c_f32, _c_f32, _c_int, _c_f32, _c_int, _c_ptr, _c_ptr],
    "dgv2_glin_dinput": [_c_ptr, _c_int, _c_ptr, _c_i64, _c_ptr, _c_ptr, _c_ptr, _c_ptr, _c_int, _c_int, _c_int, _c_f32, _c_f32,
                         _c_int, _c_ptr],
    "dgv2_glin_dweight": [_c_ptr] * 7 + [_c_int] * 3 + [_c_f32, _c_f32, _c_f32, _c_ptr, _c_ptr],
    "dgv2_conv3x3_dgrad8": [_c_ptr] * 3 + [_c_int] * 5 + [_c_ptr, _c_int, _c_ptr],
    "dgv2_conv3x3_s2_dgrad8": [_c_ptr] * 3 + [_c_int] * 6 + [_c_ptr],
    "dgv2_conv3x3_x3_wgrad_scratch": [_c_ptr] + [_c_int] * 6,
    "dgv2_conv3x3_x3_wgrad": [_c_ptr, _c_ptr, _c_i64] + [_c_ptr] * 2 + [_c_int] * 7 + [_c_f32, _c_int, _c_ptr, _c_ptr],
    "dgv2_conv_x3_images": [_c_ptr] * 3 + [_c_int] * 2 + [_c_ptr],
    "dgv2_conv3x3_x3_dgrad": [_c_ptr] * 4 + [_c_int] * 6 + [_c_ptr, _c_ptr],
    "dgv2_conv3x3_x3_fwd": [_c_ptr] * 3 + [_c_int] * 6 + [_c_ptr, _c_ptr, _c_int, _c_f32, _c_f32, _c_ptr, _c_ptr],
    "dgv2_conv3x3_fwd8": [_c_ptr] * 3 + [_c_int] * 6 + [_c_ptr, _c_ptr, _c_int, _c_f32, _c_f32, _c_int, _c_ptr],
    "dgv2_conv_wgrad_stream_scratch": [_c_ptr] + [_c_int] * 9,
    "dgv2_conv_wgrad_stream": [_c_ptr, _c_ptr, _c_i64, _c_ptr, _c_ptr] + [_c_int] * 10 + [_c_ptr],
    "dgv2_conv_wgrad_stream_pl": [_c_ptr, _c_ptr, _c_i64, _c_ptr, _c_ptr] + [_c_int] * 9 + [_c_f32, _c_int, _c_int, _c_ptr],
    "dgv2_conv_dgrad": [_c_ptr] * 4 + [_c_int] * 11 + [_c_ptr],
    "dgv2_conv_wgrad": [_c_ptr] * 3 + [_c_int] * 11 + [_c_ptr],
    "dgv2_stem_fwd": [_c_ptr] * 4 + [_c_int] * 5 + [_c_f32, _c_f32, _c_int, _c_ptr],
    "dgv2_stem_bwd_scratch": [_c_ptr] + [_c_int] * 4,
    "dgv2_stem_bwd": [_c_ptr] * 4 + [_c_i64] + [_c_ptr] * 4 + [_c_int] * 5 + [_c_f32, _c_f32, _c_int, _c_ptr],
    "dgv2_stem_bwd_skip": [_c_ptr] * 4 + [_c_i64] + [_c_ptr] * 8 + [_c_int] + [_c_ptr] * 3 + [_c_int] * 8 + [_c_f32, _c_f32, _c_int,
                                                                                                        _c_ptr],
    "dgv2_gen_tail_fwd": [_c_ptr] * 7 + [_c_int] * 3 + [_c_f32] * 3 + [_c_ptr],
    "dgv2_gen_tail_bwd": [_c_ptr] * 11 + [_c_int] * 3 + [_c_f32] * 3 + [_c_ptr],
    "dgv2_ada_apply": [_c_ptr] * 8 + [_c_int] * 5 + [_c_ptr],
    "dgv2_ada_sample": [_c_ptr] * 7 + [_c_int] * 3 + [_c_ptr],
    "dgv2_ada_build": [_c_ptr] * 8 + [_c_int] * 4 + [_c_ptr],
    "dgv2_ada_sample_img": [_c_ptr] * 7 + [_c_int, _c_ptr],
    "dgv2_ada_fold": [_c_ptr] * 11 + [_c_int] * 6 + [_c_ptr],
    "dgv2_ada_apply_img": [_c_ptr] * 11 + [_c_int] * 5 + [_c_ptr],
    "dgv2_coords_convert": [_c_ptr] * 4 + [_c_int] * 3 + [_c_f32] * 3 + [_c_int, _c_ptr],
    "dgv2_msml_prepare": [_c_ptr] * 6 + [_c_int] * 5 + [_c_ptr],
    "dgv2_msml_fwd": [_c_ptr] * 7 + [_c_int] * 7 + [_c_ptr],
    "dgv2_msml_bwd": [_c_ptr] * 9 + [_c_int] * 7 + [_c_ptr],
    "dgv2_coords_convert_bwd": [_c_ptr] * 5 + [_c_int] * 3 + [_c_f32, _c_f32, _c_int, _c_ptr],
    "dgv2_fourier_feature_bwd": [_c_ptr] * 6 + [_c_int] * 8 + [_c_ptr],
}


def _load():
    if not os.path.exists(LIB_PATH):
        raise ImportError(
            f"{LIB_PATH} not found: build it with `make` (or __graft_entry__.build()). "
            "The MI355X path has no CPU fallback."
        )
    lib = ctypes.CDLL(LIB_PATH)
    for name, argtypes in SIGNATURES.items():
        fn = getattr(lib, name)
        fn.argtypes = argtypes
        fn.restype = ctypes.c_int
    got = lib.dgv2_abi_version()
    if got != ABI_VERSION:
        raise ImportError(f"libdgv2.so ABI version {got}, binding expects {ABI_VERSION}")
    return lib


lib = _load()


def dtype_code(t):
    if t.dtype == torch.float32:
        return F32
    if t.dtype == torch.bfloat16:
        return BF16
    raise RuntimeError(f"dgv2: unsupported dtype {t.dtype} (float32 / bfloat16 only)")


def check(*tensors):
    for t in tensors:
        if t is None:
            continue
        if not t.is_cuda:
            raise RuntimeError("dgv2: tensor must be a CUDA/HIP tensor (no CPU fallback)")
        if not t.is_contiguous():
            raise RuntimeError("dgv2: tensor must be contiguous")


def ptr(t):
    return None if t is None else t.data_ptr()


def stream():
    return torch.cuda.current_stream().cuda_stream


ENOTSUP = -3


def call(name, *args):
    rc = getattr(lib, name)(*args)
    if rc != 0:
        raise RuntimeError(f"{name} failed with code {rc}")


def try_call(name, *args):
    rc = getattr(lib, name)(*args)
    if rc == ENOTSUP:
        return False
    if rc != 0:
        raise RuntimeError(f"{name} failed with code {rc}")
    return True


STATUS_X_INEXACT, STATUS_FIR_TABLE = 1, 2
_STATUS_TEXT = {
    STATUS_X_INEXACT: "a launch with an x_exact promise (fp32 conv on conv_x3.hip / its weight gradient: 'these input "
                      "channels hold bf16-representable values') staged a value that is not: that launch computed on the "
                      "bf16 rounding of its input",
    STATUS_FIR_TABLE: "dgv2_fir_same_mfma_prep met a table entry outside its contract: the band operands are unusable",
}
_status_words = {}


def status_word(device=None):
    idx = torch.cuda.current_device() if device is None else torch.device(device).index
    idx = torch.cuda.current_device() if idx is None else idx
    w = _status_words.get(idx)
    if w is None:
# ... 22 lines not shown
```

dusty-gan-v2_amd/gans/models/dusty_v2.py:

```python
import math
import os

import numpy as np
import torch
import torch.nn as nn
import torch.nn.functional as F
from torch.nn.modules.utils import _pair

from . import base, dusty_v1, ops
from .ops import native
from .ops.fourier import _CONST_CACHE

LOW = torch.bfloat16


class MappingNetwork(nn.Sequential):

    def __init__(self, in_ch, out_ch, depth=2):
        self.in_ch, self.out_ch, self.depth = in_ch, out_ch, depth
        layers = [ops.PixelNorm()]
        ch = in_ch
        for _ in range(depth):
            layers.append(nn.Sequential(
                ops.EqualLR(nn.Linear(ch, out_ch), gain=math.sqrt(2), lr_mul=0.01),
# ... 570 lines not shown
            hd_h, hd8 = self.conv1.forward_cl(x, act=self.bias_act1, bank=bank, down=spec, q8=True)
        c = 1.0 / math.sqrt(2)
        xs = native.resample_q8(x, self.blur_down)
        h = self.conv2.forward_cl((hd_h, hd8), act=self.bias_act2, act_scale=self.bias_act2.scale * c, bank=bank,
                                  fp8=fp8[self.conv2])
        return self.skip.forward_cl(xs, geom=self.skip_geom, resid=h, wscale=c, bank=bank, fp8=fp8[self.skip])

    def forward_cl(self, x, bank=None, fp8=None, xs=None):
        if (xs is None and fp8 is not None and self.conv2 in fp8 and bank is not None and bank.get(self.conv1) is not None
                and isinstance(self.resample, ops.Resample) and native.fp8_ok(x, self.conv2.out_ch)):
            return self._forward_fp8(x, bank, fp8)
        hd = None
        if bank is not None and bank.get(self.conv1) is not None and isinstance(self.resample, ops.Resample):
            if x.requires_grad and xs is None:
                hd, x = self.conv1.forward_cl(x, act=self.bias_act1, bank=bank, fork=True, down=self.resample.spec)
            else:
                hd = self.conv1.forward_cl(x, act=self.bias_act1, bank=bank, down=self.resample.spec)
        else:
            h = self.conv1.forward_cl(x, act=self.bias_act1, bank=bank)
        c = 1.0 / math.sqrt(2)
        if xs is None:
            xs = native.resample(x, self.blur_down)
        if native.conv_resid_ok(xs, self.skip_geom) and self.skip._params_bias()[0] is None:
            h = self.conv2.forward_cl(self.resample.forward_cl(h) if hd is None else hd, act=self.bias_act2,
                                      act_scale=self.bias_act2.scale * c, bank=bank)
            return self.skip.forward_cl(xs, geom=self.skip_geom, resid=h, wscale=c, bank=bank)
        h = self.conv2.forward_cl(self.resample.forward_cl(h) if hd is None else hd, act=self.bias_act2, bank=bank)
        s = self.skip.forward_cl(xs, geom=self.skip_geom, bank=bank)
        return (h + s) * c

    def forward(self, x):
        return ops.from_cl(self.forward_cl(ops.to_cl(x)))


class Discriminator(nn.Module):

    def __init__(self, in_ch: int, ch_base: int = 32, ch_max: int = 512, mbdis_group: int = 4, mbdis_feat: int = 1,
                 resolution=(64, 512), ring=True, num_fp16_layers=-1, pre_blur=True):
        super().__init__()
        res_in = _pair(256 if resolution is None else resolution)
        n_down = int(np.log2(min(res_in) / 4))
        res_out = tuple(map(lambda x: x >> n_down, res_in))

        def ch(i):
            return min(ch_base << i, ch_max)

        kw = dict(bias=False, ring=ring, equal_lr=True)
        self.num_fp16_layers = num_fp16_layers
        self.epilogue_dtype = os.environ.get("DGV2_D_EPILOGUE", "fp32")
        self.fp8_branches = os.environ.get("DGV2_FP8", "0") == "1"
        c_in = in_ch * 2 if pre_blur else in_ch
        layers = [ops.BlurVH(ring=ring)] if pre_blur else []
        layers += [ops.Conv2d(c_in, ch(0), 1, 1, 0, **kw)]
        layers += [ops.FusedLeakyReLU(ch(0))]
        layers += [ResidualBlock(ch(i), ch(i + 1)) for i in range(n_down)]
        self.layers = nn.Sequential(*layers)
        self.epilogue = nn.Sequential(
            ops.MinibatchStdDev(group=mbdis_group, features=mbdis_feat),
            ops.Conv2d(ch(4) + mbdis_feat, ch(4), 3, 1, 1, **kw),
            ops.FusedLeakyReLU(ch(4)),
            nn.Flatten(),
            ops.EqualLR(nn.Linear(ch(4) * int(np.prod(res_out)), ch(4), bias=False)),
            ops.FusedLeakyReLU(ch(4)),
            ops.EqualLR(nn.Linear(ch(4), 1)),
        )

    def _weight_bank(self):
        if self.num_fp16_layers not in (-1, 0):
            return None
        dt = LOW if self.num_fp16_layers == -1 else torch.float32
        vec = 32 if dt == LOW else 16
        items = []
        for layer in self.layers:
            if isinstance(layer, ResidualBlock):
                items += layer.bank_entries(vec)
        mb, conv = self.epilogue[0], self.epilogue[1]
        cin = conv.in_ch
        edt = self._epilogue_dtype()
        evec = 32 if edt == LOW else 16
        epi = (conv, conv.bank_entry(pad_in_to=(cin + evec - 1) // evec * evec))
        if edt == dt:
            items.append(epi)
        if len(items) > 32:
            return None
        prepared = native.conv_weight_bank([e for _, e in items], dt,
                                           image8=[dt == LOW and (True if m.geom.stride == 1 else "fwd") for m, _ in items])
        bank = {m: native.PreparedConv(e[1], e[2], *images) for (m, e), images in zip(items, prepared)}
        if edt != dt:
            images, = native.conv_weight_bank([epi[1]], edt, image8=[True])
            bank[conv] = native.PreparedConv(epi[1][1], epi[1][2], *images)
        return bank

    def _fp8_bank(self):
        items = []
        for layer in self.layers:
            if isinstance(layer, ResidualBlock):
                items += layer.fp8_entries(32)
        if not items or len(items) > 16:
            return None
        prepared = native.fp8_quant_weights([e for _, e in items])
        return {m: wd for (m, _), wd in zip(items, prepared)}

    def _epilogue_dtype(self):
        if self.epilogue_dtype not in ("fp32", "bf16"):
            raise ValueError(f"epilogue_dtype must be 'fp32' or 'bf16', got {self.epilogue_dtype!r}")
        return LOW if (self.epilogue_dtype == "bf16" and self.num_fp16_layers == -1) else torch.float32

    def _fused_stem(self, h, layers, down=None):
        blur, conv, act = layers[0], layers[1], layers[2]
        w, b, _ = conv._params()
        low = self.num_fp16_layers > 1 or self.num_fp16_layers == -1
        return native.stem(h, w, act.bias, blur.blur_h.spec.ring, act.negative_slope, act.scale,
                           LOW if low else torch.float32, down=down)

    _cut = None

    def head_parameters(self):
        return [p for m in self.epilogue[4:] for p in m.parameters()]

    def take_cut(self):
        cut, self._cut = self._cut, None
        return cut

    _bank_keep = None

    def forward(self, h, splits=1, double_backward=False, features_only=False, cut=False, reuse_bank=False):
        layers = list(self.layers)
        i = 0
        keep = self._bank_keep if (reuse_bank and not double_backward and h.is_cuda) else None
        if keep is not None and keep[0] == (self.num_fp16_layers, self._epilogue_dtype(), self.fp8_branches):
            bank, fp8 = keep[1], keep[2]
        else:
            r1_bank = double_backward and _R1_BANK and self.num_fp16_layers == -1
            bank = None if ((double_backward and not r1_bank) or not h.is_cuda) else self._weight_bank()
            fp8 = self._fp8_bank() if (bank is not None and self.fp8_branches and self.num_fp16_layers == -1) else None
            if bank is not None:
                self._bank_keep = ((self.num_fp16_layers, self._epilogue_dtype(), self.fp8_branches), bank, fp8)
        fused = (not double_backward and h.is_cuda and h.shape[1] == 1 and len(layers) > 3
                 and isinstance(layers[0], ops.BlurVH) and isinstance(layers[1], ops.Conv2d)
                 and isinstance(layers[2], ops.FusedLeakyReLU) and layers[2].bias is not None
                 and layers[1]._params_bias()[0] is None and tuple(layers[1].raw_weight().shape[1:]) == (2, 1, 1)
                 and layers[1].raw_weight().shape[0] in (8, 16, 32, 64))
        xs0 = None
        if fused:
            blk0 = layers[3] if len(layers) > 3 and isinstance(layers[3], ResidualBlock) else None
            want = (blk0 is not None and _STEM_SKIP and torch.is_grad_enabled() and fp8 is None
                    and (self.num_fp16_layers == -1 or self.num_fp16_layers == 0))
            x = self._fused_stem(h, layers, down=blk0.blur_down if want else None)
            if want:
                x, xs0 = x
            i = 3
        else:
            x = ops.to_cl(h.float())
        while i < len(layers):
            low = (self.num_fp16_layers > i) or (self.num_fp16_layers == -1)
            x = x.to(LOW if low else torch.float32)
            layer = layers[i]
            nxt = layers[i + 1] if i + 1 < len(layers) else None
            if isinstance(layer, ops.Conv2d) and isinstance(nxt, ops.FusedLeakyReLU):
                x = layer.forward_cl(x, act=nxt)
                i += 2
            elif isinstance(layer, ResidualBlock):
                x = layer.forward_cl(x, bank=bank, fp8=fp8, xs=xs0)
                xs0 = None
                i += 1
            else:
                x = layer.forward_cl(x)
                i += 1
        if features_only:
            return x
        mb, conv, act1, _, lin1, act2, lin2 = self.epilogue
        edt = self._epilogue_dtype()
        trunk_low, n_trunk = x.dtype == LOW, int(x.shape[3])
        cin = x.shape[3] + mb.features
        vec = 32 if edt == LOW else 16
        cpad = (cin + vec - 1) // vec * vec
        if (not double_backward and cpad > x.shape[3]
                and native.mbstd_cat_ok(x, mb.group, splits, mb.features, cpad, out_dtype=edt)):
            x = native.mbstd_cat(x, mb.group, splits, cpad, out_dtype=edt)
        else:
            x = mb.forward_cl(x.to(edt).float(), pad_to=cpad, splits=splits).to(edt)
        if edt == torch.float32 and trunk_low and x.dtype == torch.float32:
            x._dgv2_exact = n_trunk
        x = conv.forward_cl(x, pad_in_to=cpad, act=act1, bank=bank)
        x = native.flatten_nchw(x) if (x.is_cuda and not double_backward) else ops.from_cl(x).flatten(1)
        if cut:
            leaf = x.detach().requires_grad_(True)
            self._cut = (x, leaf)
            x = leaf
        if edt == LOW and lin1.module.bias is None and lin1.gain_ == 1.0:
            x = native.linear_low(x, lin1.module.weight, lin1.scale) if x.is_cuda else \
                F.linear(x, lin1.module.weight.to(LOW)).float() * lin1.scale
        elif x.is_cuda and lin1.module.bias is None and lin1.gain_ == 1.0 and x.shape[1] >= 8192:
            x = native.linear_f32(x.float(), lin1.module.weight, lin1.scale)
        else:
            x = lin1(x.float())
        if not double_backward and native.d_tail_ok(x, act2, lin2):
            return native.d_tail(x, act2, lin2)
        x = act2.forward_cl(x)
        return lin2(x)
```

dusty-gan-v2_amd/gans/models/ops/native/conv.py:

```python
import contextlib
import os
from typing import NamedTuple, Optional

import torch
from torch.autograd import Function

import dgv2_native as N
from . import act_resample as _act_resample
from .act_resample import *
from .modgemm import *


class ConvGeom:
    def __init__(self, kh, kw, stride, pad, ring):
        self.kh, self.kw, self.stride, self.pad, self.ring = kh, kw, stride, pad, int(bool(ring))

    def out_hw(self, H, W):
        return (H + 2 * self.pad - self.kh) // self.stride + 1, (W + 2 * self.pad - self.kw) // self.stride + 1

    @property
    def ring3x3(self):
        return bool(self.ring) and (self.kh, self.kw, self.pad) == (3, 3, 1)


# ... 628 lines not shown
    @staticmethod
    def backward(ctx, g):
        (x,) = ctx.saved_tensors
        group, splits, cpad, out_dtype = ctx.cfg
        B, H, W, C = x.shape
        if torch.is_grad_enabled():
            m = B // (splits * group)
            xf, gf = x.float(), g.float()
            y = xf.reshape(splits, group, m, H, W, C)
            d = y - y.mean(1, keepdim=True)
            sd = torch.sqrt((d * d).mean(1, keepdim=True) + 1e-8)
            gst = gf[..., C].reshape(splits, group, m, H * W).sum(dim=(1, 3))
            term = gst[:, None, :, None, None, None] / float(H * W * C) * d / (group * sd)
            return (gf[..., :C] + term.reshape(B, H, W, C)).to(x.dtype), None, None, None, None
        g = g.contiguous().to(out_dtype)
        gx = torch.empty_like(x)
        N.call("dgv2_mbstd_cat_bwd_x", N.ptr(gx), N.ptr(g), N.ptr(x), B, H * W, C, cpad, splits, group, _dt(x), _dt(g),
               N.stream())
        return gx, None, None, None, None


def mbstd_cat_ok(x, group, splits, features, cpad, out_dtype=None):
    vn = 8 if x.dtype == torch.bfloat16 else 4
    B, C = x.shape[0], x.shape[3]
    g = min(B // splits, group)
    mixed_ok = out_dtype in (None, x.dtype) or (x.dtype == torch.bfloat16 and out_dtype == torch.float32)
    return (x.is_cuda and features == 1 and x.dtype in (torch.bfloat16, torch.float32) and C % vn == 0 and cpad % vn == 0
            and cpad > C and 1 <= g <= 8 and B % (splits * g) == 0 and mixed_ok)


def mbstd_cat(x, group, splits, cpad, out_dtype=None):
    g = min(x.shape[0] // splits, group)
    return _MbstdCat.apply(x, g, splits, cpad, out_dtype)


class _FlattenNCHW(Function):

    @staticmethod
    def forward(ctx, x):
        x = x.contiguous()
        B, H, W, C = x.shape
        out = torch.empty((B, C * H * W), device=x.device, dtype=x.dtype)
        N.check(x)
        N.call("dgv2_transpose_list", _ptr_array([out]), _ptr_array([x]), _int_array([H * W]), _int_array([C]),
               _int_array([C]), 1, B, x.element_size(), N.stream())
        ctx.shape = (B, H, W, C)
        return out

    @staticmethod
    def backward(ctx, g):
        B, H, W, C = ctx.shape
        if torch.is_grad_enabled():
            return g.reshape(B, C, H, W).permute(0, 2, 3, 1).contiguous()
        g = g.contiguous()
        gx = torch.empty((B, H, W, C), device=g.device, dtype=g.dtype)
        N.call("dgv2_transpose_list", _ptr_array([gx]), _ptr_array([g]), _int_array([C]), _int_array([H * W]),
               _int_array([H * W]), 1, B, g.element_size(), N.stream())
        return gx


def flatten_nchw(x):
    return _FlattenNCHW.apply(x)


class _ScaledHandle(Function):

    @staticmethod
    def forward(ctx, param, scale, cpad):
        ctx.scale, ctx.C = scale, param.shape[1]
        O, C, kh, kw = param.shape
        return torch.empty((O, kh, kw, max(C, cpad)), device=param.device, dtype=param.dtype)

    @staticmethod
    def backward(ctx, g):
        gp = g[..., :ctx.C].permute(0, 3, 1, 2)
        out = torch.empty(gp.shape, device=g.device, dtype=g.dtype)
        return torch.mul(gp, ctx.scale, out=out), None, None


def scaled_handle(param, scale, cpad=0, bank=None):
    h = _ScaledHandle.apply(param, float(scale), int(cpad))
    h._dgv2_bank = (bank, None)
    return h


def conv8t_image_ok(p, cpad, dtype):
    return (dtype == torch.bfloat16 and tuple(p.shape[2:]) == (3, 3) and cpad % 64 == 0 and p.shape[0] % 32 == 0
            and p.shape[0] >= 64)


def conv8_image_ok(p, cpad, dtype):
    return (dtype == torch.bfloat16 and tuple(p.shape[2:]) == (3, 3) and p.shape[0] % 64 == 0 and cpad % 32 == 0
            and cpad >= 64)


def convx3_image_ok(p, cpad, dtype):
    return (dtype == torch.float32 and _CONV_X3 and tuple(p.shape[2:]) == (3, 3) and p.shape[0] % 64 == 0 and cpad % 8 == 0
            and cpad >= 64)


def convx3t_image_ok(p, cpad, dtype):
    return (dtype == torch.float32 and _CONV_X3 and tuple(p.shape[2:]) == (3, 3) and p.shape[0] % 32 == 0 and p.shape[0] >= 64
            and cpad >= 64 and p.shape[1] % 64 <= 4 and p.shape[1] // 64 == cpad // 64)


def conv_weight_bank(entries, dtype, image8=None):
    L = len(entries)
    dev = entries[0][0].device
    dims = [(p.shape[0], p.shape[1], int(cp), p.shape[2] * p.shape[3]) for p, _, cp in entries]
    sizes = [o * kk * cp for o, _, cp, kk in dims]
    flat_f = torch.empty(sum(sizes), device=dev, dtype=dtype)
    flat_t = torch.empty(sum(sizes), device=dev, dtype=dtype)
    x3 = dtype == torch.float32
    flags = image8 if image8 is not None else [False] * L
    want = [bool(f) and (convx3_image_ok if x3 else conv8_image_ok)(p, cp, dtype) for f, (p, _, cp) in zip(flags, entries)]
    want_t = [f is True and (convx3t_image_ok if x3 else conv8t_image_ok)(p, cp, dtype) for f, (p, _, cp) in zip(flags, entries)]
    if x3:
        n8 = [3 * (o // 64) * ((cp + 31) // 32) * 2304 * 8 for o, _, cp, _ in dims]
        n8t = [3 * (cp // 64) * (o // 32) * 2304 * 8 for o, _, cp, _ in dims]
    else:
        n8 = n8t = sizes
    idt = torch.bfloat16 if x3 else dtype
    flat_8 = torch.empty(sum(n for n, f in zip(n8, want) if f), device=dev, dtype=idt) if any(want) else None
    flat_8t = torch.empty(sum(n for n, f in zip(n8t, want_t) if f), device=dev, dtype=idt) if any(want_t) else None
    wfs, wts, w8s, w8ts, off, off8, off8t = [], [], [], [], 0, 0, 0
    for (o, c, cp, kk), n, m8, m8t, f, ft in zip(dims, sizes, n8, n8t, want, want_t):
        wfs.append(flat_f[off:off + n].view(o, kk, cp))
        wts.append(flat_t[off:off + n].view(cp, kk, o))
        w8s.append(flat_8[off8:off8 + m8] if f else None)
        w8ts.append(flat_8t[off8t:off8t + m8t] if ft else None)
        if ft and x3:
            w8ts[-1]._dgv2_clive = int(c)
        off += n
        off8 += m8 if f else 0
        off8t += m8t if ft else 0
    srcs = [p.detach() for p, _, _ in entries]
    N.check(*srcs)
    rest = (_ptr_array(srcs), _int_array([d[0] for d in dims]), _int_array([d[1] for d in dims]),
            _int_array([d[2] for d in dims]), _int_array([d[3] for d in dims]),
            (_ct.c_float * L)(*[float(s) for _, s, _ in entries]), L, N.dtype_code(flat_f), N.stream())
    if image8 is None:
        N.call("dgv2_conv_weight_bank", _ptr_array(wfs), _ptr_array(wts), *rest)
        return list(zip(wfs, wts))
    N.call("dgv2_conv_weight_bank_ex", _ptr_array(wfs), _ptr_array(wts), _ptr_array(w8s), _ptr_array(w8ts), *rest)
    return list(zip(wfs, wts, w8s, w8ts))


_ACTBWD_BLOCKS = {}


_FUSED_ACTBWD = os.environ.get("DGV2_NO_FUSED_ACTBWD") is None


def _resample_actbwd(g, out, spec, in_hw, alpha, scale):
    if not _FUSED_ACTBWD or g.dtype != out.dtype:
        return None
    B, H, W, C = out.shape
    Ho, Wo = spec.out_size(H, W)
    (ih_idx, ih_coef, ih_cnt, Eh), (iw_idx, iw_coef, iw_cnt, Ew) = spec.tables(H, W, True, g.device)
    tabs = (N.ptr(ih_idx), N.ptr(ih_coef), N.ptr(ih_cnt), Eh, N.ptr(iw_idx), N.ptr(iw_coef), N.ptr(iw_cnt), Ew)
    bands = None
    if _act_resample._FIR_MFMA and g.dtype == torch.bfloat16 and (Ho, Wo) == (H, W) and C % 32 == 0:
        bands = spec.bands(H, W, True, g.device)
    mfma = bands is not None
    entry = "dgv2_fir_same_mfma_actbwd" if mfma else "dgv2_resample_tab_actbwd"
    tabs = (N.ptr(bands),) if mfma else tabs
    geo = (B, C, H, W) if mfma else (B, C, Ho, Wo, H, W)
    tail = (alpha, scale) if mfma else (alpha, scale, _dt(g))
    key = (entry, B, H, W, C, Eh, Ew, _dt(g))
    if key not in _ACTBWD_BLOCKS:
        nb = _ct.c_int64(0)
        ok = N.try_call(entry, None, None, None, 0, _ct.addressof(nb), None, None, *tabs, *geo, *tail, N.stream())
        _ACTBWD_BLOCKS[key] = nb.value if ok else 0
    nblk = _ACTBWD_BLOCKS[key]
    if nblk == 0:
        return None
    g = g.contiguous()
    N.check(g, out)
    gpre = torch.empty_like(out)
    gb = torch.empty(C, device=g.device, dtype=torch.float32)
    scratch = torch.empty(nblk * C, device=g.device, dtype=torch.float32)
    N.call(entry, N.ptr(gpre), N.ptr(gb), N.ptr(scratch), scratch.numel(), None, N.ptr(g), N.ptr(out), *tabs, *geo, *tail,
           N.stream())
    return gpre, gb


class _Conv(Function):

    @staticmethod
    def forward(ctx, x, w, bias, resid, x8, ep):
        ctx.set_materialize_grads(False)
        assert (ep.act is not None) == (bias is not None) and ep.resid == (resid is not None) and not (ep.act and ep.resid)
        assert ep.act is not None or (ep.down is None and not ep.fork), "blur/down and fork belong to the activation's forms"
        assert ep.fp8 is None or (ep.down is None and not ep.fork), "an e4m3 input has no blur/down or fork form"
        alpha, scale = ep.act or (0.2, 1.0)
        act = 0 if ep.act is None else 3
        if bias is not None:
            ctx.size_b = bias.numel()
            bias = bias.detach().float().contiguous()
        if resid is not None:
            resid = resid.contiguous()
        if ep.fp8 is not None:
            from .fp8 import _conv_fwd_fp8
            _weights(ctx, w, torch.bfloat16)
            x = x8
            out = _conv_fwd_fp8(x8, ep.fp8[0], ep.fp8[1], ep.geom, bias, act, alpha, scale, resid)
        else:
            x = x.contiguous()
            wc, w8 = _weights(ctx, w, x.dtype)
            out = _conv_fwd_raw(x, wc, ep.geom, bias, act, alpha, scale, resid, w8, ep.x_exact)
        ctx.save_for_backward(x, w, *(() if ep.act is None else (out,)))
        ctx.ep = ep
        if ep.down is None:
            y = (out,)
        elif ep.q8:
            from .fp8 import _handle, _resample_q8_raw
            y8 = _resample_q8_raw(out, ep.down, tuple(out.shape[1:3]))
            if y8 is None:
                raise RuntimeError("dgv2: no e4m3 resampling kernel covers this shape (check native.fp8_ok first)")
            ctx.mark_non_differentiable(y8)
            y = (_handle(y8.shape, x.device), y8)
        else:
            y = (_resample_raw(out, ep.down, False, tuple(out.shape[1:3])),)
        if ep.fork:
            y += (x.view_as(x),)
        return y if len(y) > 1 else y[0]

    @staticmethod
    def backward(ctx, gy, *rest):
        ep = ctx.ep
        gx_sibling = rest[-1] if ep.fork else None
        if gy is None:
            return gx_sibling, None, None, None, None, None
        x, w, *out = ctx.saved_tensors
        want_gw = ctx.needs_input_grad[1] if ep.first_order else want_param_grad(ctx, 1)
        gb = None
        if ep.act is not None:
            out, (alpha, scale) = out[0], ep.act
            fused = None
            if ep.down is not None:
                in_hw = tuple(out.shape[1:3])
                if not torch.is_grad_enabled():
                    fused = _resample_actbwd(gy.to(out.dtype), out, ep.down, in_hw, alpha, scale)
                if fused is None:
                    gy = _Resample.apply(gy, ep.down, True, in_hw)
            want_gb = ep.first_order or want_param_grad(ctx, 2)
            gy, gb = fused or _BiasActBackward.apply(gy, out, want_gb, alpha, scale, 1, ctx.size_b)
        wt, w8t, gscale = ctx.bank
        gx, gw = gx_sibling, None
        if ep.fp8 is not None:
            from .fp8 import fp8_dequant
            if ep.resid:
                gy = gy.contiguous()
            if ctx.needs_input_grad[0]:
                gx = _dgrad(gy, w, ep.geom, tuple(x.shape), wt, None, gscale)
            if want_gw:
                gw = _ConvWgrad.apply(gy, fp8_dequant(x), ep.geom, gscale)
        else:
            if ctx.needs_input_grad[0]:
                gx = _dgrad(gy, w, ep.geom, tuple(x.shape), wt, gx_sibling, gscale, w8t)
            if want_gw:
                x3 = None
                if gy.dtype == torch.float32 and w8t is not None and w8t.dtype == torch.bfloat16:
                    x3 = getattr(w8t, "_dgv2_clive", None)
                gw = _ConvWgrad.apply(gy, x, ep.geom, gscale, x3, ep.x_exact, _wgrad_out(w, gscale))
        return gx, gw, gb, (gy if ep.resid and ctx.needs_input_grad[3] else None), None, None


def conv_ring_ep(x, w, ep, bias=None, resid=None):
    x, x8 = x if ep.fp8 is not None else (x, None)
    return _Conv.apply(x, w, bias, resid, x8, ep)


def conv_ring(x, w, geom):
    return conv_ring_ep(x, w, ConvEpilogue(geom))


def conv_resid_ok(x, geom):
    return _direct_ok(geom, x.shape[3] % _kstep(x) == 0)

__all__ = [n_ for n_ in dir() if not n_.startswith("__")]
```

dusty-gan-v2_amd/gans/models/ops/native/stem_tail_ada.py:

```python
import math
import os

import torch
from torch.autograd import Function

import dgv2_native as N
from .act_resample import *
from .modgemm import *
from .conv import *


class _Stem(Function):

    @staticmethod
    def forward(ctx, x, w, bias, ring, alpha, scale, out_dtype, down=None):
        H, W_ = ctx_hw = _stem_hw(x)
        B = x.shape[0]
        x3 = x.detach().float().reshape(B, -1).contiguous()
        O = w.shape[0]
        w32 = w.detach().float().reshape(O, 2).contiguous()
        b32 = bias.detach().float().contiguous()
        y = torch.empty((B, H, W_, O), device=x.device, dtype=out_dtype)
        N.check(x3, w32, b32)
        N.call("dgv2_stem_fwd", N.ptr(y), N.ptr(x3), N.ptr(w32), N.ptr(b32), B, H, W_, O, int(ring), alpha, scale,
               _dt(y), N.stream())
        ctx.save_for_backward(x3, w32, y)
        ctx.cfg = (ctx_hw, ring, alpha, scale, tuple(x.shape), w.shape, down)
        if down is None:
            return y
        ctx.set_materialize_grads(False)
        return y, _resample_raw(y, down, False, (H, W_))

    @staticmethod
    @torch.autograd.function.once_differentiable
    def backward(ctx, gy, gsk=None):
        x3, w32, y = ctx.saved_tensors
        (H, W_), ring, alpha, scale, xshape, wshape, down = ctx.cfg
        B, O = x3.shape[0], w32.shape[0]
        if gy is None:
            gy = torch.zeros_like(y)
        gy = gy.contiguous().to(y.dtype)
        key = (B, H, W_, O)
        if key not in _STEM_SCRATCH:
            n = _ct.c_int64(0)
            N.call("dgv2_stem_bwd_scratch", _ct.addressof(n), B, H, W_, O)
            _STEM_SCRATCH[key] = n.value
        scratch = torch.empty(_STEM_SCRATCH[key], device=gy.device, dtype=torch.float32)
        gw = torch.empty((O, 2), device=gy.device, dtype=torch.float32)
        gb = torch.empty(O, device=gy.device, dtype=torch.float32)
        gx = torch.empty((B, H * W_), device=gy.device, dtype=torch.float32) if ctx.needs_input_grad[0] else None
        if gsk is not None:
            gsk = gsk.contiguous().to(y.dtype)
            Hs, Ws = down.out_size(H, W_)
            (ih, chh, nh, Eh), (iw, cw, nw, Ew) = down.tables(H, W_, True, gy.device)
            N.check(gsk)
            N.call("dgv2_stem_bwd_skip", N.ptr(gx), N.ptr(gw), N.ptr(gb), N.ptr(scratch), scratch.numel(), N.ptr(gy), N.ptr(y),
                   N.ptr(x3), N.ptr(w32), N.ptr(gsk), N.ptr(ih), N.ptr(chh), N.ptr(nh), Eh, N.ptr(iw), N.ptr(cw), N.ptr(nw), Ew,
                   Hs, Ws, B, H, W_, O, int(ring), alpha, scale, _dt(y), N.stream())
        else:
            N.call("dgv2_stem_bwd", N.ptr(gx), N.ptr(gw), N.ptr(gb), N.ptr(scratch), scratch.numel(), N.ptr(gy), N.ptr(y),
                   N.ptr(x3), N.ptr(w32), B, H, W_, O, int(ring), alpha, scale, _dt(y), N.stream())
        return (None if gx is None else gx.reshape(xshape)), gw.reshape(wshape), gb, None, None, None, None, None


_STEM_SCRATCH = {}


def _stem_hw(x):
    if x.ndim != 4 or 1 not in (x.shape[1], x.shape[3]):
        raise RuntimeError("dgv2 stem: expected a one-channel image batch")
    return (x.shape[2], x.shape[3]) if x.shape[1] == 1 else (x.shape[1], x.shape[2])


def stem(x, w, bias, ring=True, alpha=0.2, scale=math.sqrt(2.0), out_dtype=torch.float32, down=None):
    return _Stem.apply(x, w, bias, bool(ring), float(alpha), float(scale), out_dtype, down)


class _GenTail(Function):
    @staticmethod
    def forward(ctx, skip, shift, u, out_scale, raydrop_const, temperature):
        skip = skip.contiguous()
        B, H, W, _ = skip.shape
        N.check(skip, shift, u)
        outs = [torch.empty((B, 1, H, W), device=skip.device, dtype=torch.float32) for _ in range(4)]
        ctx.set_materialize_grads(False)
        image, image_orig, logit, mask = outs
        N.call("dgv2_gen_tail_fwd", N.ptr(image), N.ptr(image_orig), N.ptr(logit), N.ptr(mask), N.ptr(skip),
               N.ptr(shift), N.ptr(u), B, H, W, out_scale, raydrop_const, temperature, N.stream())
        ctx.save_for_backward(image_orig, logit, mask, u, shift)
        ctx.cfg = (out_scale, raydrop_const, temperature)
        return image, image_orig, logit, mask

    @staticmethod
    def backward(ctx, g_image, g_image_orig, g_logit, g_mask):
        image_orig, logit, mask, u, shift = ctx.saved_tensors
        out_scale, raydrop_const, temperature = ctx.cfg
        B, _, H, W = image_orig.shape
        gs = [None if g is None else g.contiguous().float() for g in (g_image, g_image_orig, g_logit, g_mask)]
        g_skip = torch.empty((B, H, W, 2), device=u.device, dtype=torch.float32)
        scratch = torch.empty_like(g_skip) if shift is not None else None
        N.call("dgv2_gen_tail_bwd", N.ptr(g_skip), N.ptr(scratch), N.ptr(gs[0]), N.ptr(gs[1]), N.ptr(gs[2]),
               N.ptr(gs[3]), N.ptr(image_orig), N.ptr(logit), N.ptr(mask), N.ptr(u), N.ptr(shift), B, H, W,
               out_scale, raydrop_const, temperature, N.stream())
        return g_skip, None, None, None, None, None


def gen_tail(skip, shift, u, out_scale=0.25, raydrop_const=-1.0, temperature=1.0):
    return _GenTail.apply(skip, shift, u, float(out_scale), float(raydrop_const), float(temperature))


def gumbel_uniform(shape, device):
    return torch.rand(shape, device=device).clamp_(_EPS_U, 1.0 - _EPS_U)


class _AdaApply(Function):
    @staticmethod
    def forward(ctx, x, Ay, kx, off, sgn, a, c, transpose, out=None):
        x = x.contiguous().float()
        B, _, H, W = x.shape
        N.check(x, Ay, kx, off, sgn, a, c, out)
        if out is not None and (out.shape != x.shape or out.dtype != torch.float32):
            raise ValueError("ada_apply: `out` must be a contiguous fp32 tensor shaped like the input")
        y = torch.empty_like(x) if out is None else out
        N.call("dgv2_ada_apply", N.ptr(y), N.ptr(x), N.ptr(Ay), N.ptr(kx), N.ptr(off), N.ptr(sgn), N.ptr(a),
               N.ptr(c), B, H, W, kx.shape[1], int(transpose), N.stream())
        ctx.save_for_backward(Ay, kx, off, sgn, a, c)
        ctx.transpose = transpose
        return y

    @staticmethod
    def backward(ctx, g):
        Ay, kx, off, sgn, a, _ = ctx.saved_tensors
        gx = _AdaApply.apply(g, Ay, kx, off, sgn, a, None, not ctx.transpose)
        return gx, None, None, None, None, None, None, None, None


def ada_apply(x, Ay, kx, off, sgn, a, c, out=None):
    if out is not None and torch.is_grad_enabled() and x.requires_grad:
        raise RuntimeError("ada_apply(out=...) is for passes that record no graph")
    return _AdaApply.apply(x, Ay, kx, off, sgn, a, c, False, out)


def ada_sample(B, H, W, p, policy, device, u=None, n=None):
    u = torch.rand(B, 16, device=device) if u is None else u.float().contiguous()
    n = torch.randn(B, 8, device=device) if n is None else n.float().contiguous()
    if tuple(u.shape) != (B, 16) or tuple(n.shape) != (B, 8):
        raise ValueError(f"ada_sample: u {tuple(u.shape)} / n {tuple(n.shape)} for B = {B}")
    N.check(u, n)
    gaff = torch.empty((B, 4), device=device, dtype=torch.float32)
    a = torch.empty(B, device=device, dtype=torch.float32)
    c = torch.empty(B, device=device, dtype=torch.float32)
    pol = (_ct.c_float * 11)(*policy)
    N.call("dgv2_ada_sample", N.ptr(gaff), N.ptr(a), N.ptr(c), N.ptr(u), N.ptr(n), N.ptr(p), pol, B, H, W, N.stream())
    return gaff, a, c


def ada_build(gaff, M1y, M1x, taps, H, W, K):
    B = gaff.shape[0]
    dev = gaff.device
    Ay = torch.empty((B, H, H), device=dev, dtype=torch.float32)
    kx = torch.empty((B, K), device=dev, dtype=torch.float32)
    off = torch.empty(B, device=dev, dtype=torch.int32)
    sgn = torch.empty(B, device=dev, dtype=torch.int32)
    N.check(gaff, M1y, M1x, taps)
    N.call("dgv2_ada_build", N.ptr(Ay), N.ptr(kx), N.ptr(off), N.ptr(sgn), N.ptr(gaff), N.ptr(M1y), N.ptr(M1x),
           N.ptr(taps), B, H, W, K, N.stream())
    return Ay, kx, off, sgn


class _AdaApplyImg(Function):

    @staticmethod
    def forward(ctx, x, Ay, kx, off, sgn, a, c, cut, sigma, eps, transpose, out=None):
        x = x.contiguous().float()
        B, _, H, W = x.shape
        N.check(x, Ay, kx, off, sgn, a, c, cut, sigma, eps, out)
        if out is not None and (out.shape != x.shape or out.dtype != torch.float32):
            raise ValueError("ada_apply_img: `out` must be a contiguous fp32 tensor shaped like the input")
        if eps is not None and (eps.numel() != x.numel() or eps.dtype != torch.float32):
            raise ValueError("ada_apply_img: `eps` must be an fp32 tensor with one normal per pixel")
        y = torch.empty_like(x) if out is None else out
        N.call("dgv2_ada_apply_img", N.ptr(y), N.ptr(x), N.ptr(Ay), N.ptr(kx), N.ptr(off), N.ptr(sgn), N.ptr(a), N.ptr(c),
               N.ptr(cut), N.ptr(sigma), N.ptr(eps), B, H, W, kx.shape[1], int(transpose), N.stream())
        ctx.save_for_backward(Ay, kx, off, sgn, a, cut)
        ctx.transpose = transpose
        return y

    @staticmethod
    def backward(ctx, g):
        Ay, kx, off, sgn, a, cut = ctx.saved_tensors
        gx = _AdaApplyImg.apply(g, Ay, kx, off, sgn, a, None, cut, None, None, not ctx.transpose)
        return (gx,) + (None,) * 11


def ada_apply_img(x, Ay, kx, off, sgn, a, c, cut=None, sigma=None, eps=None, out=None):
    if out is not None and torch.is_grad_enabled() and x.requires_grad:
        raise RuntimeError("ada_apply_img(out=...) is for passes that record no graph")
    if (sigma is None) != (eps is None):
        raise ValueError("ada_apply_img: sigma and eps come together")
    return _AdaApplyImg.apply(x, Ay, kx, off, sgn, a, c, cut, sigma, eps, False, out)


def ada_sample_img(B, p, policy, device, u2=None, n2=None):
    u2 = torch.rand(B, 8, device=device) if u2 is None else u2.float().contiguous()
    n2 = torch.randn(B, 8, device=device) if n2 is None else n2.float().contiguous()
    if tuple(u2.shape) != (B, 8) or tuple(n2.shape) != (B, 8):
        raise ValueError(f"ada_sample_img: u2 {tuple(u2.shape)} / n2 {tuple(n2.shape)} for B = {B}")
    N.check(u2, n2, p)
    g = torch.empty((B, 4), device=device, dtype=torch.float32)
    sigma = torch.empty(B, device=device, dtype=torch.float32)
    cut = torch.empty((B, 4), device=device, dtype=torch.float32)
    pol = (_ct.c_float * 3)(*policy)
    N.call("dgv2_ada_sample_img", N.ptr(g), N.ptr(sigma), N.ptr(cut), N.ptr(u2), N.ptr(n2), N.ptr(p), pol, B, N.stream())
    return g, sigma, cut
# ... 45 lines not shown
```

include/dgv2.h:

```cpp
#ifndef DGV2_H
#define DGV2_H

#include <stdint.h>

#ifdef __cplusplus
extern "C" {
#endif

#define DGV2_F32 0
#define DGV2_BF16 1
#define DGV2_FP8 2
#define DGV2_EINVAL (-1)
#define DGV2_ENOTSUP (-3)

#define DGV2_STATUS_X_INEXACT 1
#define DGV2_STATUS_FIR_TABLE 2

int dgv2_abi_version(void);

int dgv2_fused_bias_act(void* y, const void* x, const void* bias, const void* ref,
                        int64_t size_x, int64_t step_b, int64_t size_b,
                        int act, int grad, float alpha, float scale, int dtype, void* stream);

int dgv2_bias_grad(float* gb, const void* x, int64_t size_x, int64_t step_b, int64_t size_b,
                   int dtype, void* stream);

int dgv2_bias_act_bwd(void* gx, float* gb, const void* gy, const void* ref, int64_t rows, int C,
                      float alpha, float scale, float* scratch, int64_t scratch_elems, int dtype,
                      void* stream);
int dgv2_bias_act_bwd_rs(void* gx, float* gb, const void* gy, const void* ref, int64_t rows, int C,
                         float alpha, float scale, const float* row_scale, float* scratch,
                         int64_t scratch_elems, int dtype, void* stream);
int dgv2_scale_cast(void* y, const void* x, const float* row_scale, int64_t n, int C, int xdtype, int ydtype,
                    void* stream);

int dgv2_upfirdn2d(void* out, const void* in, const float* kernel,
                   int major, int in_h, int in_w, int minor, int kh, int kw,
                   int up_x, int up_y, int down_x, int down_y,
                   int pad_x0, int pad_x1, int pad_y0, int pad_y1, int dtype, void* stream);

int dgv2_resample(void* y, const void* x, const float* taps_h, const float* taps_w,
                  int B, int H, int W, int C, int Ho, int Wo, int ldx, int ldy,
                  int kh, int up_h, int down_h, int p0_h,
                  int kw, int up_w, int down_w, int p0_w,
                  int ring, int adjoint, int dtype, void* stream);

int dgv2_resample_tab(void* y, const void* x, const int* idx_h, const float* coef_h, const int* cnt_h,
                      int Eh, const int* idx_w, const float* coef_w, const int* cnt_w, int Ew,
                      int B, int C, int ldx, int ldy, int in_h, int in_w, int out_h, int out_w,
                      int dtype, void* stream);

int dgv2_resample_tab_add(void* y, const void* x, const void* resid, const int* idx_h, const float* coef_h,
                          const int* cnt_h, int Eh, const int* idx_w, const float* coef_w, const int* cnt_w, int Ew,
                          int B, int C, int in_h, int in_w, int out_h, int out_w, int dtype, void* stream);
int dgv2_resample_tab_add_affine(void* y, const void* x, const void* resid, const float* rscale, const float* rbias,
                                 const int* idx_h, const float* coef_h, const int* cnt_h, int Eh, const int* idx_w,
                                 const float* coef_w, const int* cnt_w, int Ew, int B, int C, int in_h, int in_w, int out_h,
                                 int out_w, int dtype, void* stream);

int dgv2_resample_tab_sq(void* y, const void* x, const int* idx_h, const float* coef_h, const int* cnt_h,
                         int Eh, const int* idx_w, const float* coef_w, const int* cnt_w, int Ew,
                         int B, int C, int ldx, int ldy, int in_h, int in_w, int out_h, int out_w,
                         int dtype, float* sumsq, int sumsq_cap, int* sumsq_used, void* stream);

int dgv2_resample_tab_actbwd(void* y, float* gb, float* scratch, int64_t scratch_elems, int64_t* blocks_needed,
                             const void* x, const void* ref, const int* idx_h, const float* coef_h,
                             const int* cnt_h, int Eh, const int* idx_w, const float* coef_w, const int* cnt_w,
                             int Ew, int B, int C, int in_h, int in_w, int out_h, int out_w, float alpha,
                             float scale, int dtype, void* stream);

int dgv2_fir_same_mfma_prep(void* bands, int64_t bands_bytes, int64_t* bytes_needed, const int* idx_h, const float* coef_h,
                            const int* cnt_h, int Eh, const int* idx_w, const float* coef_w, const int* cnt_w, int Ew,
                            int H, int W, int* status, void* stream);
int dgv2_fir_same_mfma(void* y, const void* x, const void* bands, int B, int C, int H, int W, void* stream);
int dgv2_fir_same_mfma_actbwd(void* y, float* gb, float* scratch, int64_t scratch_elems, int64_t* blocks_needed,
                              const void* x, const void* ref, const void* bands, int B, int C, int H, int W, float alpha,
                              float scale, void* stream);

int dgv2_fourier_feature(void* out, const float* angle, const float* shift,
                         const float* freqs, const float* phase,
                         int B, int Ba, int H, int W, int F, int ld, int c0, int dtype, void* stream);

int dgv2_downsample_angle(float* out, const float* in, const float* shift, const float* taps,
                          int B, int Ba, int H, int W, int ring, void* stream);

int dgv2_bmm_nn(void* y, const void* x, const void* w, int B, int P, int I, int O,
                int ldx, int ldy, int64_t wstride, const float* bias, int act, float alpha, float scale,
                int dtype, int ydtype, void* stream);
int dgv2_bmm_tn(float* gw, const void* gy, const void* x, int B, int P, int I, int O,
                int ldgy, int ldx, int dtype, void* stream);

int dgv2_bmm_nn_cat(void* y, const void* xa, const void* xs, const void* w, int B, int P, int Ka, int Ks,
                    int O, const float* bias, int act, float alpha, float scale, int dtype, int ydtype,
                    void* stream);
int dgv2_modconv_up_fwd(void* y, const void* t, const void* xs, const void* wimg, int B, int Hout, int Wout, int Hin,
                        int Win, int Ks, int O, const int* idx_h, const float* coef_h, const int* idx_w,
                        const float* coef_w, const float* bias, const float* in_scale, int act, float alpha, float scale,
                        int dtype, float* sumsq, int sumsq_cap, int* sumsq_used, void* stream);
int dgv2_modconv_up_t(void* tcm, void* wimg, const void* h, const void* w, const float* row_scale, float gain, int B,
                      int Hlow, int Wlow, int Ka, int Ks, int O, int I, int koff, int dtype, void* stream);
int dgv2_modconv_up_t_lag(void* tcm, void* wimg, const void* h, const void* w, float gain, const float* ghd,
                          const float* gho, const float* gwd, const float* gwo, int B, int Hlow, int Wlow, int Ka, int Ks,
                          int O, int I, int koff, int dtype, float* sumsq, int sumsq_cap, int* sumsq_used, void* stream);
int dgv2_up2_lag_sumsq(const void* h, const float* ghd, const float* gho, const float* gwd, const float* gwo, int B,
                       int Hin, int Win, int C, int dtype, float* sumsq, int sumsq_cap, int* sumsq_used, void* stream);
int dgv2_bmm_nn_sq(void* y, const void* x, const void* w, int B, int P, int I, int O, int ldx, int ldy,
                   int64_t wstride, const float* row_scale, const float* bias, int act, float alpha, float scale,
                   const void* resid , int dtype, int ydtype,
                   float* sumsq, int sumsq_cap, int* sumsq_used, void* stream);
int dgv2_bmm_nn_cat_sq(void* y, const void* xa, const void* xs, const void* w, int B, int P, int Ka, int Ks,
                       int O, const float* row_scale, const float* bias, int act, float alpha, float scale, int dtype, int ydtype,
                       float* sumsq, int sumsq_cap, int* sumsq_used, void* stream);
int dgv2_bmm_tn_cat(float* gw, const void* gy, const void* xa, const void* xs, int B, int P, int Ka, int Ks,
                    int O, int dtype, void* stream);
int dgv2_bmm_tn_small(float* gw, const void* gy, const void* x, int B, int P, int I, int O, int dtype,
                      void* stream);
int dgv2_bmm_nn_small(void* y, const void* x, const void* w, const void* resid, int B, int P, int O, int K,
                      int dtype, void* stream);
int dgv2_bmm_nn_small_act(void* y, const void* x, const void* w, const void* resid, int B, int P, int O, int K,
                          const void* ref, const float* row_scale, float alpha, float ascale, float* gb,
                          float* scratch, int64_t scratch_elems, int64_t* blocks_needed, int dtype, void* stream);
int dgv2_head_bwd(void* y, float* gw, float* gbh, float* gb_up, float* scratch, int64_t scratch_elems,
                  int64_t* blocks_needed, const float* gyf, const float* cvec, const void* w, const void* resid,
                  const void* ref, const float* row_scale, float alpha, float ascale, int B, int P, int O, int K, int dtype,
                  void* stream);

int dgv2_modconv_pe_fwd(void* y, const void* xa, const void* xs, const void* w, int B, int P, int Ka, int Ks,
                        int O, const float* bias, int act, float alpha, float scale, int dtype, void* stream);
int dgv2_modconv_pe_fwd_sq(void* y, const void* xa, const void* xs, const void* w, int B, int P, int Ka, int Ks,
                           int O, const float* row_scale, const float* bias, int act, float alpha, float scale, int dtype, float* sumsq,
                           int sumsq_cap, int* sumsq_used, void* stream);
int dgv2_modconv_pe_fwd_head(void* y, const void* xa, const void* xs, const void* w, int B, int P, int Ka, int Ks,
                             int O, const float* row_scale, const float* bias, int act, float alpha, float scale, int dtype,
                             float* sumsq, int sumsq_cap, int* sumsq_used, const void* head_w, float* head_out, void* stream);

int dgv2_modconv_pe_dgrad_actbwd(void* gpre, float* gb, float* scratch, int64_t scratch_elems, int64_t* rows_needed,
                                 const void* gy, const void* wt, const void* yref, const float* up_scale, float alpha,
                                 float scale, int B, int P, int K, int dtype, void* stream);

int dgv2_lerp_list(float* const* dst, const float* const* src, const int* n, int L, float weight, void* stream);
int dgv2_adam_prep(float* sc, float* step, float b1, float b2, void* stream);
int dgv2_adam_step(float* const* p, const float* const* g, float* const* m, float* const* v, const int* n,
                   int L, const float* sc, float lr, float b1, float b2, float eps, void* stream);

int dgv2_pack2d(float* packed, const float* const* src, const int* rows, const int* cols, int L, int Rmax,
                int Cmax, void* stream);
int dgv2_unpack2d(float* const* dst, const float* packed, const int* rows, const int* cols, int L, int Rmax,
                  int Cmax, void* stream);

int dgv2_ema_scalar(float* ema, float* snapshot, const float* sumsq, int nsum, float add, float inv_count,
                    float weight, int update, float* cvec, int ncvec, void* stream);
int dgv2_ema_scalar_group(float* const* emas, const int* rows, int n, const float* sumsq, int nsum, float add,
                          float inv_count, float weight, int update, float* cvec, void* stream);
int dgv2_mod_prep_fwd(void* wb, float* dsave, float* stats, const float* W, const float* s,
                      const float* ema_var, const float* shift, const float* fw, int B, int O, int I,
                      int Otot, int row_off, int demod, int cin, int F, int wb_dtype, void* stream);
int dgv2_mod_prep_bwd(float* gW, float* gs, float* corr, const float* G, const float* W, const float* s,
                      const float* stats, const float* dsave, const float* ema_var, const float* shift,
                      const float* fw, int B, int O, int I, int Otot, int row_off, int demod, int cin,
                      int F, int corr_elems, void* stream);

int dgv2_mod_prep_all_fwd(void* const* wb, float* const* dsave, float* stats, float* rot, const float* const* W,
                          const float* const* s, const float* const* fw, const int* O, const int* I,
                          const int* Otot, const int* row_off, const int* cin, const int* flags,
                          const float* shift, int B, int L, void* stream);
int dgv2_mod_prep_all_bwd(float* flat, int64_t flat_elems, float* const* out, const int* ncorr,
                          const float* const* G, const float* const* W, const float* const* s,
                          const float* stats, const float* rot, float* const* dsave,
                          const float* const* fw, const int* O, const int* I, const int* Otot,
                          const int* row_off, const int* cin, const int* flags, const float* shift, int B,
                          int L, float* scratch, int64_t scratch_elems, void* stream);
int dgv2_mod_prep_all_bwd_scratch(int64_t* elems, const int* O, const int* I, int B, int L);

int dgv2_transpose_list(void* const* dst, const void* const* src, const int* rows, const int* cols,
                        const int* ld, int L, int B, int elem_size, void* stream);

int dgv2_sum_squares(float* acc, const void* x, int64_t N, int C, int ld, int dtype, void* stream);

int dgv2_mbstd_cat_fwd(void* out, float* scratch, const void* x, int B, int P, int C, int Cp, int splits,
                       int group, int dtype, void* stream);
int dgv2_mbstd_cat_bwd(void* gx, const void* gout, const void* x, int B, int P, int C, int Cp, int splits,
                       int group, int dtype, void* stream);
int dgv2_gemm_x3(float* c, float* scratch, int64_t scratch_elems, const float* a, const float* b, int I, int J,
                 int64_t T, int a_trans, int b_trans, int64_t lda, int64_t ldb, int64_t ldo, int splits, float scale,
                 void* stream);
int dgv2_pe_wgrad_scratch(int64_t* elems, int B, int P, int O, int Ks);
int dgv2_pe_wgrad(float* gw, float* scratch, int64_t scratch_elems, const void* g, const void* pe, int B, int P, int O,
                  int Ks, int64_t ldo, int col0, void* stream);
int dgv2_mbstd_cat_fwd_x(void* out, float* scratch, const void* x, int B, int P, int C, int Cp, int splits, int group,
                         int xdtype, int ydtype, void* stream);
int dgv2_mbstd_cat_bwd_x(void* gx, const void* gout, const void* x, int B, int P, int C, int Cp, int splits, int group,
                         int xdtype, int gdtype, void* stream);

int dgv2_conv_fwd(void* y, const void* x, const void* w, int B, int H, int W, int C, int O,
                  int kh, int kw, int stride, int pad, int ring,
                  const float* bias, int act, float alpha, float scale, int dtype, void* stream);
int dgv2_conv_dgrad(void* gx, void* gxp_scratch, const void* gy, const void* wt,
                    int B, int H, int W, int C, int O,
                    int kh, int kw, int stride, int pad, int ring, int dtype, void* stream);
int dgv2_conv_wgrad(float* gw, const void* gy, const void* x, int B, int H, int W, int C, int O,
                    int kh, int kw, int stride, int pad, int ring, int dtype, void* stream);

int dgv2_conv_wgrad_direct(float* gw, const void* gy, const void* x, int B, int H, int W, int C, int O,
                           int k, int stride, int pad, int ring, int dtype, void* stream);

int dgv2_bmm_tn_stream_scratch(int64_t* elems, int B, int H, int W, int C, int O, int dtype);
int dgv2_bmm_tn_stream(float* gw, float* scratch, int64_t scratch_elems, const void* gy, const void* x,
                       int B, int H, int W, int C, int O, int dtype, void* stream);
int dgv2_bmm_tn_stream_x(float* gw, float* scratch, int64_t scratch_elems, const void* gy, const void* x,
                         int x_shared, int B, int H, int W, int C, int O, int dtype, void* stream);
int dgv2_bmm_tn_stream_ld(float* gw, int64_t ldo, float* scratch, int64_t scratch_elems, const void* gy, const void* x,
                          int x_shared, int B, int H, int W, int C, int O, int dtype, void* stream);

int dgv2_conv_weight_bank(void* const* wf, void* const* wt, const float* const* src, const int* O,
                          const int* C, const int* Cpad, const int* kk, const float* scale, int L,
                          int dtype, void* stream);
int dgv2_conv_weight_bank_ex(void* const* wf, void* const* wt, void* const* w8, void* const* w8t,
                             const float* const* src, const int* O, const int* C, const int* Cpad, const int* kk,
                             const float* scale, int L, int dtype, void* stream);
int dgv2_conv3x3_fwd8(void* y, const void* x, const void* w8, int B, int Hin, int Win, int Cin, int O, int stride,
                      const float* bias, const void* resid, int act, float alpha, float scale, int dtype, void* stream);
int dgv2_conv3x3_dgrad8(void* gx, const void* gy, const void* w8t, int B, int H, int W, int C, int O, const void* resid,
                        int dtype, void* stream);
int dgv2_conv3x3_s2_dgrad8(void* gx, const void* gy, const void* wt, int B, int Hg, int Wg, int C, int O, int dtype,
                           void* stream);

int dgv2_conv3x3_x3_fwd(void* y, const void* x, const void* w3, int B, int H, int W, int Cx, int x_exact, int O,
                        const float* bias, const void* resid, int act, float alpha, float scale, int* status,
                        void* stream);
int dgv2_conv3x3_x3_dgrad(void* gx, const void* gy, const void* w3t, const void* wt, int B, int H, int W, int C, int ldx,
                          int O, const void* resid, void* stream);
int dgv2_conv3x3_x3_wgrad(float* gw, float* scratch, int64_t scratch_elems, const void* gy, const void* x, int B, int H,
                          int W, int C, int clive, int x_exact, int O, float scale, int param_layout, int* status,
                          void* stream);
int dgv2_conv3x3_x3_wgrad_scratch(int64_t* elems, int B, int H, int W, int C, int clive, int O);
int dgv2_conv_x3_images(void* w3, void* w3t, const void* w, int O, int Cp, void* stream);

int dgv2_conv_wgrad_stream_scratch(int64_t* elems, int B, int H, int W, int C, int O, int k, int stride,
                                   int pad, int dtype);
int dgv2_conv_wgrad_stream(float* gw, float* scratch, int64_t scratch_elems, const void* gy, const void* x,
                           int B, int H, int W, int C, int O, int k, int stride, int pad, int ring,
                           int dtype, void* stream);
int dgv2_conv_wgrad_stream_pl(float* gw, float* scratch, int64_t scratch_elems, const void* gy, const void* x,
                              int B, int H, int W, int C, int O, int k, int stride, int pad, int ring,
                              float scale, int param_layout, int dtype, void* stream);

int dgv2_conv_taps(void* y, const void* x, const void* w, int B, int Hin, int Win, int Cin,
                   int Hg, int Wg, int O, int Hy, int Wy, int in_stride, int ioff_h, int ioff_w,
                   int out_stride, int ooff_h, int ooff_w, int ntaps, int wtaps, const int* taps_host,
                   int hzero, int ring, int accumulate, const float* bias, const void* resid, int act,
                   float alpha, float scale, int dtype, void* stream);
int dgv2_conv_taps_ex(void* y, const void* x, const void* w, int B, int Hin, int Win, int Cin, int Hg,
                      int Wg, int O, int Hy, int Wy, int in_stride, int ioff_h, int ioff_w,
                      int out_stride, int ncls, const int* cls_host, int ntaps, int wtaps,
                      const int* taps_host, int nextra, const int* extras_host, int hzero, int ring,
                      int accumulate, const float* bias, const void* resid, int act, float alpha,
                      float scale, int dtype, void* stream);
int dgv2_conv_taps_ld(void* y, int ldy, const void* x, const void* w, int B, int Hin, int Win, int Cin, int Hg,
                      int Wg, int O, int Hy, int Wy, int in_stride, int ioff_h, int ioff_w, int out_stride, int ncls,
                      const int* cls_host, int ntaps, int wtaps, const int* taps_host, int nextra,
                      const int* extras_host, int hzero, int ring, int accumulate, const float* bias,
                      const void* resid, int act, float alpha, float scale, int dtype, void* stream);

int dgv2_stem_fwd(void* y, const float* x, const float* w, const float* bias, int B, int H, int W, int O,
                  int ring, float alpha, float scale, int ydtype, void* stream);
int dgv2_stem_bwd_scratch(int64_t* elems, int B, int H, int W, int O);
int dgv2_stem_bwd(float* gx, float* gw, float* gb, float* scratch, int64_t scratch_elems, const void* gy,
                  const void* y, const float* x, const float* w, int B, int H, int W, int O, int ring,
                  float alpha, float scale, int dtype, void* stream);
int dgv2_stem_bwd_skip(float* gx, float* gw, float* gb, float* scratch, int64_t scratch_elems, const void* gy, const void* y,
                       const float* x, const float* w, const void* gsk, const int* idx_h, const float* coef_h,
                       const int* cnt_h, int Eh, const int* idx_w, const float* coef_w, const int* cnt_w, int Ew, int Hs,
                       int Ws, int B, int H, int W, int O, int ring, float alpha, float scale, int dtype, void* stream);

int dgv2_gen_tail_fwd(float* image, float* image_orig, float* logit, float* mask,
                      const float* skip, const float* shift, const float* u,
                      int B, int H, int W, float out_scale, float raydrop_const, float temperature,
                      void* stream);
int dgv2_gen_tail_bwd(float* g_skip, float* scratch, const float* g_image, const float* g_image_orig,
                      const float* g_logit, const float* g_mask,
                      const float* image_orig, const float* logit, const float* mask, const float* u,
                      const float* shift, int B, int H, int W, float out_scale, float raydrop_const,
                      float temperature, void* stream);

int dgv2_ada_apply(float* y, const float* x, const float* Ay, const float* kx, const int* off,
                   const int* sgn, const float* a, const float* c, int B, int H, int W, int K,
                   int transpose, void* stream);

int dgv2_ada_sample(float* gaff, float* a, float* c, const float* u, const float* n, const float* p,
                    const float* policy_host, int B, int H, int W, void* stream);
int dgv2_ada_build(float* Ay, float* kx, int* off, int* sgn, const float* gaff, const float* M1y,
                   const float* M1x, const float* taps, int B, int H, int W, int K, void* stream);

int dgv2_ada_sample_img(float* g, float* sigma, float* cut, const float* u2, const float* n2, const float* p,
                        const float* policy_host, int B, void* stream);
int dgv2_ada_fold(float* Ay2, float* kx2, int* off2, float* c2, const float* Ay, const float* kx, const int* off,
                  const int* sgn, const float* c, const float* g, const float* fbank, int B, int H, int W, int K,
                  int NB, int T, void* stream);
int dgv2_ada_apply_img(float* y, const float* x, const float* Ay, const float* kx, const int* off, const int* sgn,
                       const float* a, const float* c, const float* cut, const float* sigma, const float* eps, int B,
                       int H, int W, int K, int transpose, void* stream);

int dgv2_coords_convert(float* out, const float* in, const float* mask, const float* angle,
                        int B, int H, int W, float min_depth, float max_depth, float raydrop_const,
                        int mode, void* stream);

int dgv2_surface_normal(float* out, const float* points, int B, int H, int W, int d, int mode, void* stream);

int dgv2_nsgan_loss(float* stats, float* gy, const float* y, int n_real, int n_fake, float gy_scale, float* sign_cum,
                    float* n_cum, void* stream);

int dgv2_d_tail_fwd(float* y, float* a, const float* h, const float* b1, const float* w2, const float* b2, int B, int K,
                    float alpha, float act_scale, float scale2, float gain2, void* stream);
int dgv2_d_tail_bwd(float* gh, float* gb1, float* gw2, float* gb2, const float* gy, const float* a, const float* w2,
                    int B, int K, float alpha, float act_scale, float scale2, float gain2, void* stream);

int dgv2_colmean_lerp(float* dst, const float* src, int B, int K, int64_t ld, float w, void* stream);

int dgv2_rng_fill(float* const* out, const int64_t* count, const int* kind, const float* a, const float* b, int nseg,
                  uint64_t* state, void* stream);

int dgv2_kitti_rows(int* row, int* counts, const float* pts, int n, int H, void* stream);
int dgv2_kitti_project(float* out, unsigned long long* key, const float* pts, const int* row, int n, int H, int W,
                       int Wout, float min_depth, float max_depth, int apply_mask, void* stream);

int dgv2_fps_scratch(int64_t* floats, int B, int n);
int dgv2_fps(int* idxs, float* temp, const float* xyz, int B, int n, int m, void* stream);
int dgv2_gather_points(float* out, const float* points, const int* idx, int B, int C, int n, int m, void* stream);
int dgv2_gather_points_grad(float* grad_points, const float* grad_out, const int* idx, int B, int C, int n, int m,
                            void* stream);

int dgv2_chamfer_fwd(float* dist1, int* idx1, float* dist2, int* idx2, const float* xyz1, const float* xyz2, int B,
                     int n, int m, void* stream);
int dgv2_nn_search(float* dist, int* idx, const float* xyz, const float* ref, int B, int n, int m, int ref_shared,
                   void* stream);
int dgv2_chamfer_bwd(float* gxyz1, float* gxyz2, const float* xyz1, const float* xyz2, const float* gdist1,
                     const float* gdist2, const int* idx1, const int* idx2, int B, int n, int m, void* stream);

int dgv2_emd_approxmatch(float* match, float* temp, const float* xyz1, const float* xyz2, int B, int n, int m,
                         void* stream);
int dgv2_emd_matchcost(float* cost, const float* match, const float* xyz1, const float* xyz2, int B, int n, int m,
                       void* stream);
int dgv2_emd_matchcost_grad(float* grad1, float* grad2, const float* match, const float* xyz1, const float* xyz2, int B,
                            int n, int m, void* stream);

int dgv2_fir_same_mfma_q8(void* y8, const void* x, const void* bands, int B, int C, int H, int W, void* stream);
int dgv2_resample_tab_q8(void* y8, const void* x, const int* idx_h, const float* coef_h, const int* cnt_h, int Eh,
                         const int* idx_w, const float* coef_w, const int* cnt_w, int Ew, int B, int C, int in_h,
                         int in_w, int out_h, int out_w, void* stream);
int dgv2_fp8_quant_weights(void* const* w8, const void* const* src, const int* O, const int* C, const int* kk,
                           const float* eq, int n, float* descale, void* amax, void* stream);
int dgv2_fp8_dequant(void* y, const void* x, int64_t n, float scale, void* stream);
int dgv2_conv_taps_fp8(void* y, const void* x8, const void* w8, const float* acc_scale, int B, int Hin, int Win, int Cin,
                       int Hg, int Wg, int O, int Hy, int Wy, int in_stride, int ioff_h, int ioff_w, int ntaps, int wtaps,
                       const int* taps_host, int ring, const float* bias, const void* resid, int act, float alpha,
                       float scale, void* stream);

int dgv2_glin_fwd(float* const* y, const float* const* x, const float* const* w, const float* const* bias, const int* N,
                  const int* lda, int L, int B, int K, float alpha, float beta, int act, float slope, int prenorm,
                  float* rnorm, void* stream);
int dgv2_glin_dinput(float* dx, int ldx, float* scratch, int64_t scratch_elems, const float* const* g,
                     const float* const* yact, const float* const* w, const int* N, int L, int B, int K, float alpha,
                     float slope, int accumulate, void* stream);
int dgv2_glin_dweight(float* const* dw, float* const* dbias, const float* const* g, const float* const* yact,
                      const float* const* x, const int* N, const int* ldx, int L, int B, int K, float alpha, float beta,
                      float slope, const float* rnorm, void* stream);

int dgv2_msml_prepare(float* refp, float* maskp, float* normp, float* invm, const float* ref, const float* mask, int B,
                      int C, int H, int W, int L, void* stream);
int dgv2_msml_fwd(float* loss, float* genp, const float* gen, const float* refp, const float* maskp, const float* normp,
                  const float* invm, int B, int C, int H, int W, int L, int metric, int relative, void* stream);
int dgv2_msml_bwd(float* ggen, float* gscratch, const float* gloss, const float* gen, const float* genp,
                  const float* refp, const float* maskp, const float* normp, const float* invm, int B, int C, int H, int W,
                  int L, int metric, int relative, void* stream);
int dgv2_coords_convert_bwd(float* gx, const float* gout, const float* in, const float* mask, const float* angle, int B,
                            int H, int W, float min_depth, float max_depth, int mode, void* stream);
int dgv2_fourier_feature_bwd(float* g_angle, const void* g, const float* angle, const float* shift, const float* freqs,
                             const float* phase, int B, int Ba, int H, int W, int F, int ld, int c0, int dtype,
                             void* stream);

#ifdef __cplusplus
}
#endif
#endif
```

Measured before the change: 5352 range-images/s.

## Save 1-bit leaky-ReLU sign masks instead of bf16 activations for backward

Forward kernels for the stem, the resample and the FIR MFMA path now also write a bitmask holding the sign of each activation, one bit per channel. The matching backward kernels read these mask bits in place of the bf16 reference tensor when choosing the leaky-ReLU slope. Autograd saves the mask rather than the full activation. This cuts saved-activation memory and backward read bandwidth by about 16x for those tensors, at the cost of extra mask writes in forward. The masked nodes can no longer be differentiated a second time, so a guard is added for that case.

```diff
diff --git a/dusty-gan-v2_amd/csrc/api.hip b/dusty-gan-v2_amd/csrc/api.hip
--- a/dusty-gan-v2_amd/csrc/api.hip
+++ b/dusty-gan-v2_amd/csrc/api.hip
@@ -1,3 +1,3 @@
 #include "common.h"
 
-extern "C" int dgv2_abi_version(void) { return 49; }
+extern "C" int dgv2_abi_version(void) { return 50; }
diff --git a/dusty-gan-v2_amd/csrc/common.h b/dusty-gan-v2_amd/csrc/common.h
--- a/dusty-gan-v2_amd/csrc/common.h
+++ b/dusty-gan-v2_amd/csrc/common.h
@@ -39,6 +39,17 @@
   __device__ __forceinline__ float get(int i) const { return to_f32(e[i]); }
   __device__ __forceinline__ void set(int i, float v) { e[i] = from_f32<T>(v); }
 };
+
+__device__ __forceinline__ unsigned act_mask_byte(const uint4& v) {
+  const unsigned w[4] = {v.x, v.y, v.z, v.w};
+  unsigned m = 0;
+#pragma unroll
+  for (int k = 0; k < 4; ++k) {
+    m |= (__uint_as_float(w[k] << 16) > 0.f ? 1u : 0u) << (2 * k);
+    m |= (__uint_as_float(w[k] & 0xffff0000u) > 0.f ? 1u : 0u) << (2 * k + 1);
+  }
+  return m;
+}
 
 __device__ __forceinline__ int pack_pair_bf16(const float (&va)[4], const float (&vb)[4], int lc, uint4& out) {
   union { uint2 u; bf16_t e[4]; } pa, pb;
diff --git a/dusty-gan-v2_amd/csrc/fir_mfma.hip b/dusty-gan-v2_amd/csrc/fir_mfma.hip
--- a/dusty-gan-v2_amd/csrc/fir_mfma.hip
+++ b/dusty-gan-v2_amd/csrc/fir_mfma.hip
@@ -27,6 +27,7 @@
   float alpha, ascale;
   float* partial;
   uint8_t* y8;
+  void* mask;
 };
 
 struct FMTabs {
@@ -87,7 +88,7 @@
   if (bad) atomicOr(t.err, DGV2_STATUS_FIR_TABLE);
 }
 
-template <bool ACT>
+template <bool ACT, bool MASK = false>
 __global__ __launch_bounds__(256, 2) void fir_same_mfma_kernel(bf16_t* __restrict__ y, const bf16_t* __restrict__ x, FMGeom g) {
   extern __shared__ __attribute__((aligned(16))) unsigned char smem[];
   unsigned char* Xs = smem;
@@ -133,12 +134,26 @@
       rg[i] = *reinterpret_cast<const fm_u32x4*>(xb + (int64_t)(s * FM_RS + r) * g.W * g.C + goff[i]);
     }
   };
-  auto commit = [&]() {
+  auto commit = [&](int s) {
 #pragma unroll
     for (int i = 0; i < FM_NLD; ++i) *reinterpret_cast<fm_u32x4*>(Xs + xoff[i]) = rg[i];
+    if constexpr (!ACT && MASK) {
+      unsigned* mk = static_cast<unsigned*>(g.mask);
+#pragma unroll
+      for (int i = 0; i < FM_NLD; ++i) {
+        const int id = tid + 256 * i;
+        const int j = (id >> 2) % FM_WIN, r = id / (4 * FM_WIN);
+        const uint4 v = make_uint4(rg[i][0], rg[i][1], rg[i][2], rg[i][3]);
+        int m = (int)(act_mask_byte(v) << (8 * (id & 3)));
+        m |= __builtin_amdgcn_mov_dpp(m, 0xB1, 0xf, 0xf, true);
+        m |= __builtin_amdgcn_mov_dpp(m, 0x4E, 0xf, 0xf, true);
+        if ((id & 3) == 0 && j >= 8 && j < 8 + FM_CT)
+          mk[(((int64_t)b * g.H + s * FM_RS + r) * g.W + c0col + j - 8) * (g.C >> 5) + (cb0 >> 5)] = (unsigned)m;
+      }
+    }
   };
   issue(0);
-  commit();
+  commit(0);
   if (1 < nsteps) issue(1);
   uint4 th = bands_h[lane];
   __syncthreads();
@@ -179,16 +194,21 @@
       }
     }
     __syncthreads();
-    if (s + 1 < nsteps) commit();
+    if (s + 1 < nsteps) commit(s + 1);
     if (s + 2 < nsteps) issue(s + 2);
     const uint4 th_next = bands_h[(int64_t)min(s + 1, nsteps) * 64 + lane];
     vec16<bf16_t> fref[FM_RS / 2];
+    unsigned fbits[FM_RS / 2];
     if constexpr (ACT) {
 #pragma unroll
       for (int i = 0; i < FM_RS / 2; ++i) {
         const int id = tid + 256 * i;
         const int ho = min(max(s * FM_RS - FM_RS / 2 + (id >> 7), 0), g.H - 1);
-        fref[i].load(g.ref + img + ((int64_t)ho * g.W + c0col + ((id >> 2) & 31)) * g.C + cb0 + (id & 3) * 8);
+        if constexpr (MASK)
+          fbits[i] = static_cast<const uint8_t*>(g.mask)[(((int64_t)b * g.H + ho) * g.W + c0col + ((id >> 2) & 31)) * (g.C >> 3) +
+                                                         (cb0 >> 3) + (id & 3)];
+        else
+          fref[i].load(g.ref + img + ((int64_t)ho * g.W + c0col + ((id >> 2) & 31)) * g.C + cb0 + (id & 3) * 8);
       }
     }
 
@@ -236,7 +256,10 @@
 #pragma unroll
         for (int j = 0; j < 8; ++j) {
           const float a = o.get(j);
-          o.set(j, (fref[i].get(j) > 0.f ? a : a * g.alpha) * g.ascale);
+          bool pos;
+          if constexpr (MASK) pos = (fbits[i] >> j) & 1u;
+          else pos = fref[i].get(j) > 0.f;
+          o.set(j, (pos ? a : a * g.alpha) * g.ascale);
           bsum[j] += o.get(j);
         }
       }
@@ -310,7 +333,7 @@
   if (!y || !x || !bands) return DGV2_EINVAL;
   if (!fm_covers(B, C, H, W)) return DGV2_ENOTSUP;
   if (!aligned16(x) || !aligned16(y) || !aligned16(bands)) return DGV2_EINVAL;
-  FMGeom g{B, C, H, W, nt_output((int64_t)B * H * W * C * 2) ? 1 : 0, (const uint4*)bands, nullptr, 1.f, 1.f, nullptr, nullptr};
+  FMGeom g{B, C, H, W, nt_output((int64_t)B * H * W * C * 2) ? 1 : 0, (const uint4*)bands, nullptr, 1.f, 1.f, nullptr, nullptr, nullptr};
   auto kern = fir_same_mfma_kernel<false>;
   if (FM_LDS > 64 * 1024) {
     hipError_t e = hipFuncSetAttribute((const void*)kern, hipFuncAttributeMaxDynamicSharedMemorySize, (int)FM_LDS);
@@ -320,11 +343,26 @@
   DGV2_RETURN_LAST();
 }
 
+extern "C" int dgv2_fir_same_mfma_mask(void* y, void* mask, const void* x, const void* bands, int B, int C, int H, int W,
+                                       void* stream) {
+  if (!y || !mask || !x || !bands) return DGV2_EINVAL;
+  if (!fm_covers(B, C, H, W)) return DGV2_ENOTSUP;
+  if (!aligned16(x) || !aligned16(y) || !aligned16(bands) || (reinterpret_cast<uintptr_t>(mask) & 3)) return DGV2_EINVAL;
+  FMGeom g{B, C, H, W, nt_output((int64_t)B * H * W * C * 2) ? 1 : 0, (const uint4*)bands, nullptr, 1.f, 1.f, nullptr, nullptr, mask};
+  auto kern = fir_same_mfma_kernel<false, true>;
+  if (FM_LDS > 64 * 1024) {
+    hipError_t e = hipFuncSetAttribute((const void*)kern, hipFuncAttributeMaxDynamicSharedMemorySize, (int)FM_LDS);
+    if (e != hipSuccess) return (int)e;
+  }
+  kern<<<dim3(W / FM_CT, C / FM_CB, B), 256, FM_LDS, (hipStream_t)stream>>>((bf16_t*)y, (const bf16_t*)x, g);
+  DGV2_RETURN_LAST();
+}
+
 extern "C" int dgv2_fir_same_mfma_q8(void* y8, const void* x, const void* bands, int B, int C, int H, int W, void* stream) {
   if (!y8 || !x || !bands) return DGV2_EINVAL;
   if (!fm_covers(B, C, H, W)) return DGV2_ENOTSUP;
   if (!aligned16(x) || (reinterpret_cast<uintptr_t>(y8) & 7) || !aligned16(bands)) return DGV2_EINVAL;
-  FMGeom g{B, C, H, W, 0, (const uint4*)bands, nullptr, 1.f, 1.f, nullptr, (uint8_t*)y8};
+  FMGeom g{B, C, H, W, 0, (const uint4*)bands, nullptr, 1.f, 1.f, nullptr, (uint8_t*)y8, nullptr};
   auto kern = fir_same_mfma_kernel<false>;
   if (FM_LDS > 64 * 1024) {
     hipError_t e = hipFuncSetAttribute((const void*)kern, hipFuncAttributeMaxDynamicSharedMemorySize, (int)FM_LDS);
@@ -334,17 +372,19 @@
   DGV2_RETURN_LAST();
 }
 
-extern "C" int dgv2_fir_same_mfma_actbwd(void* y, float* gb, float* scratch, int64_t scratch_elems, int64_t* blocks_needed,
-                                         const void* x, const void* ref, const void* bands, int B, int C, int H, int W,
-                                         float alpha, float scale, void* stream) {
+static int fm_actbwd(void* y, float* gb, float* scratch, int64_t scratch_elems, int64_t* blocks_needed, const void* x,
+                     const void* ref, const void* bands, int B, int C, int H, int W, float alpha, float scale, bool masked,
+                     void* stream) {
   if (!fm_covers(B, C, H, W)) return DGV2_ENOTSUP;
   const int64_t blocks = (int64_t)B * (W / FM_CT);
   if (blocks_needed) *blocks_needed = blocks;
   if (!scratch) return blocks_needed ? 0 : DGV2_EINVAL;
   if (!y || !gb || !x || !ref || !bands) return DGV2_EINVAL;
-  if (scratch_elems < blocks * C || !aligned16(x) || !aligned16(y) || !aligned16(ref) || !aligned16(bands)) return DGV2_EINVAL;
-  FMGeom g{B, C, H, W, 0, (const uint4*)bands, (const bf16_t*)ref, alpha, scale, scratch, nullptr};
-  auto kern = fir_same_mfma_kernel<true>;
+  if (scratch_elems < blocks * C || !aligned16(x) || !aligned16(y) || !aligned16(bands)) return DGV2_EINVAL;
+  if (masked ? (reinterpret_cast<uintptr_t>(ref) & 3) != 0 : !aligned16(ref)) return DGV2_EINVAL;
+  FMGeom g{B, C, H, W, 0, (const uint4*)bands, masked ? nullptr : (const bf16_t*)ref, alpha, scale, scratch, nullptr,
+           masked ? const_cast<void*>(ref) : nullptr};
+  auto kern = masked ? fir_same_mfma_kernel<true, true> : fir_same_mfma_kernel<true>;
   if (FM_LDS > 64 * 1024) {
     hipError_t e = hipFuncSetAttribute((const void*)kern, hipFuncAttributeMaxDynamicSharedMemorySize, (int)FM_LDS);
     if (e != hipSuccess) return (int)e;
@@ -354,3 +394,15 @@
   fm_bias_reduce_kernel<<<C, 256, 0, st>>>(gb, scratch, (int)blocks, C);
   DGV2_RETURN_LAST();
 }
+
+extern "C" int dgv2_fir_same_mfma_actbwd(void* y, float* gb, float* scratch, int64_t scratch_elems, int64_t* blocks_needed,
+                                         const void* x, const void* ref, const void* bands, int B, int C, int H, int W,
+                                         float alpha, float scale, void* stream) {
+  return fm_actbwd(y, gb, scratch, scratch_elems, blocks_needed, x, ref, bands, B, C, H, W, alpha, scale, false, stream);
+}
+
+extern "C" int dgv2_fir_same_mfma_actbwd_mask(void* y, float* gb, float* scratch, int64_t scratch_elems,
+                                              int64_t* blocks_needed, const void* x, const void* mask, const void* bands,
+                                              int B, int C, int H, int W, float alpha, float scale, void* stream) {
+  return fm_actbwd(y, gb, scratch, scratch_elems, blocks_needed, x, mask, bands, B, C, H, W, alpha, scale, true, stream);
+}
diff --git a/dusty-gan-v2_amd/csrc/resample.hip b/dusty-gan-v2_amd/csrc/resample.hip
--- a/dusty-gan-v2_amd/csrc/resample.hip
+++ b/dusty-gan-v2_amd/csrc/resample.hip
@@ -285,13 +285,14 @@
 
 constexpr int RS_RB = 4;
 
-template <typename T, int EW, bool ACT = false>
+template <typename T, int EW, bool ACT = false, bool MASK = false>
 __global__ __launch_bounds__(256) void resample_stream_kernel(
     T* __restrict__ y, const T* __restrict__ x, const int* __restrict__ idx_h, const float* __restrict__ coef_h,
     const int* __restrict__ cnt_h, int Eh, const int* __restrict__ idx_w, const float* __restrict__ coef_w,
     const int* __restrict__ cnt_w, int Ew, int B, int C, int ldx, int ldy, int in_h, int in_w, int out_h, int out_w,
     int SHA, float* __restrict__ sumsq, const T* __restrict__ ref = nullptr, float alpha = 1.f, float ascale = 1.f,
-    float* __restrict__ bias_partial = nullptr, uint8_t* __restrict__ y8 = nullptr) {
+    float* __restrict__ bias_partial = nullptr, uint8_t* __restrict__ y8 = nullptr, uint8_t* __restrict__ amask = nullptr,
+    int cself = -1) {
 #ifdef DGV2_ABLATE
   const int SH = SHA & 0xffff, ablate = (SHA >> 16) & 0xff;
 #else
@@ -332,7 +333,10 @@
   }
   const T* xb = x + (int64_t)b * in_h * in_w * ldx;
   T* yp = y + (int64_t)b * out_h * out_w * ldy + (int64_t)wo * ldy + cv * VN;
-  const T* rp = ACT ? ref + (int64_t)b * out_h * out_w * ldy + (int64_t)wo * ldy + cv * VN : nullptr;
+  const T* rp = ACT && !MASK ? ref + (int64_t)b * out_h * out_w * ldy + (int64_t)wo * ldy + cv * VN : nullptr;
+  uint8_t* mp = MASK ? amask + (int64_t)b * out_h * out_w * cvecs + (int64_t)wo * cvecs + cv : nullptr;
+  bool selfok = false;
+  if constexpr (MASK && !ACT) selfok = cself >= 0 && cself < nw && idx_w[wo * Ew + cself] == wo;
   float bsum[VN];
 #pragma unroll
   for (int j = 0; j < VN; ++j) bsum[j] = 0.f;
@@ -377,6 +381,19 @@
         for (int c = 0; c < EW; ++c)
 #pragma unroll
           for (int j = 0; j < VN; ++j) h[j] += cw[c] * pv[c].get(j);
+        if constexpr (MASK && !ACT) {
+          if (r >= ho0 && r < ho1 && live) {
+            uint4 own = make_uint4(0, 0, 0, 0);
+            if (selfok) {
+#pragma unroll
+              for (int c = 0; c < EW; ++c)
+                if (c == cself) own = pv[c].raw;
+            } else {
+              own = *reinterpret_cast<const uint4*>(xb + ((int64_t)r * in_w + wo) * ldx + cv * VN);
+            }
+            mp[(int64_t)r * out_w * cvecs] = (uint8_t)act_mask_byte(own);
+          }
+        }
         if (r + 1 <= rlast && !(ablate & 2)) issue(r + 1); else pr = -1;
         {
           vec16<T> hv;
@@ -397,10 +414,15 @@
       vec16<T> o;
       if constexpr (ACT) {
         vec16<T> f;
-        f.load(rp + (int64_t)ho * out_w * ldy);
+        unsigned fbits = 0;
+        if constexpr (MASK) fbits = mp[(int64_t)ho * out_w * cvecs];
+        else f.load(rp + (int64_t)ho * out_w * ldy);
 #pragma unroll
         for (int j = 0; j < VN; ++j) {
-          o.set(j, (f.get(j) > 0.f ? acc[j] : acc[j] * alpha) * ascale);
+          bool pos;
+          if constexpr (MASK) pos = (fbits >> j) & 1u;
+          else pos = f.get(j) > 0.f;
+          o.set(j, (pos ? acc[j] : acc[j] * alpha) * ascale);
           bsum[j] += o.get(j);
         }
       } else {
@@ -455,6 +477,30 @@
     case 3: resample_stream_kernel<T, 3><<<blocks, 256, 0, st>>>(y, x, idx_h, coef_h, cnt_h, Eh, idx_w, coef_w, cnt_w, Ew, B, C, ldx, ldy, in_h, in_w, out_h, out_w, sha, sumsq); break;
     default: resample_stream_kernel<T, 4><<<blocks, 256, 0, st>>>(y, x, idx_h, coef_h, cnt_h, Eh, idx_w, coef_w, cnt_w, Ew, B, C, ldx, ldy, in_h, in_w, out_h, out_w, sha, sumsq); break;
   }
+}
+
+void rs_launch_mask(bool act, int Ew, int blocks, hipStream_t st, bf16_t* y, const bf16_t* x, const int* idx_h,
+                    const float* coef_h, const int* cnt_h, int Eh, const int* idx_w, const float* coef_w, const int* cnt_w,
+                    int B, int C, int in_h, int in_w, int out_h, int out_w, int sha, uint8_t* amask, int cself, float alpha,
+                    float ascale, float* partial) {
+#define DGV2_RS_MASK(EW)                                                                                                  \
+  do {                                                                                                                    \
+    if (act)                                                                                                              \
+      resample_stream_kernel<bf16_t, EW, true, true><<<blocks, 256, 0, st>>>(                                             \
+          y, x, idx_h, coef_h, cnt_h, Eh, idx_w, coef_w, cnt_w, Ew, B, C, C, C, in_h, in_w, out_h, out_w, sha, nullptr,   \
+          nullptr, alpha, ascale, partial, nullptr, amask, -1);                                                           \
+    else                                                                                                                  \
+      resample_stream_kernel<bf16_t, EW, false, true><<<blocks, 256, 0, st>>>(                                            \
+          y, x, idx_h, coef_h, cnt_h, Eh, idx_w, coef_w, cnt_w, Ew, B, C, C, C, in_h, in_w, out_h, out_w, sha, nullptr,   \
+          nullptr, 1.f, 1.f, nullptr, nullptr, amask, cself);                                                             \
+  } while (0)
+  switch (Ew) {
+    case 1: DGV2_RS_MASK(1); break;
+    case 2: DGV2_RS_MASK(2); break;
+    case 3: DGV2_RS_MASK(3); break;
+    default: DGV2_RS_MASK(4); break;
+  }
+#undef DGV2_RS_MASK
 }
 
 template <typename T>
@@ -483,11 +529,11 @@
 
 }
 
-extern "C" int dgv2_resample_tab_actbwd(void* y, float* gb, float* scratch, int64_t scratch_elems, int64_t* blocks_needed,
-                                        const void* x, const void* ref, const int* idx_h, const float* coef_h,
-                                        const int* cnt_h, int Eh, const int* idx_w, const float* coef_w,
-                                        const int* cnt_w, int Ew, int B, int C, int in_h, int in_w, int out_h,
-                                        int out_w, float alpha, float scale, int dtype, void* stream) {
+static int rs_actbwd(void* y, float* gb, float* scratch, int64_t scratch_elems, int64_t* blocks_needed, const void* x,
+                     const void* ref, const int* idx_h, const float* coef_h, const int* cnt_h, int Eh, const int* idx_w,
+                     const float* coef_w, const int* cnt_w, int Ew, int B, int C, int in_h, int in_w, int out_h, int out_w,
+                     float alpha, float scale, int dtype, bool masked, void* stream) {
+  if (masked && (dtype != DGV2_BF16 || C % 32)) return DGV2_ENOTSUP;
   if (B <= 0 || C <= 0 || in_h <= 0 || in_w <= 0 || out_h <= 0 || out_w <= 0 || Eh <= 0 || Ew <= 0) return DGV2_EINVAL;
   const int vn = dtype == DGV2_BF16 ? 8 : (dtype == DGV2_F32 ? 4 : 0);
   if (!vn) return DGV2_EINVAL;
@@ -499,13 +545,56 @@
   if (blocks_needed) *blocks_needed = blocks;
   if (!scratch) return blocks_needed ? 0 : DGV2_EINVAL;
   if (!y || !gb || !x || !ref || !idx_h || !coef_h || !cnt_h || !idx_w || !coef_w || !cnt_w) return DGV2_EINVAL;
-  if (scratch_elems < blocks * C || !aligned16(x) || !aligned16(y) || !aligned16(ref)) return DGV2_EINVAL;
+  if (scratch_elems < blocks * C || !aligned16(x) || !aligned16(y)) return DGV2_EINVAL;
+  if (masked ? (reinterpret_cast<uintptr_t>(ref) & 3) != 0 : !aligned16(ref)) return DGV2_EINVAL;
   hipStream_t st = (hipStream_t)stream;
+  if (masked) {
+    rs_launch_mask(true, Ew, (int)blocks, st, (bf16_t*)y, (const bf16_t*)x, idx_h, coef_h, cnt_h, Eh, idx_w, coef_w, cnt_w, B, C,
+                   in_h, in_w, out_h, out_w, SH, static_cast<uint8_t*>(const_cast<void*>(ref)), -1, alpha, scale, scratch);
+    rs_bias_reduce_kernel<<<C, 256, 0, st>>>(gb, scratch, (int)blocks, C);
+    DGV2_RETURN_LAST();
+  }
   DGV2_DISPATCH_DTYPE(dtype, {
     rs_launch_act<T>(Ew, (int)blocks, st, (T*)y, (const T*)x, idx_h, coef_h, cnt_h, Eh, idx_w, coef_w, cnt_w, B, C, C, C,
                      in_h, in_w, out_h, out_w, SH, (const T*)ref, alpha, scale, scratch);
   });
   rs_bias_reduce_kernel<<<C, 256, 0, st>>>(gb, scratch, (int)blocks, C);
+  DGV2_RETURN_LAST();
+}
+
+extern "C" int dgv2_resample_tab_actbwd(void* y, float* gb, float* scratch, int64_t scratch_elems, int64_t* blocks_needed,
+                                        const void* x, const void* ref, const int* idx_h, const float* coef_h,
+                                        const int* cnt_h, int Eh, const int* idx_w, const float* coef_w,
+                                        const int* cnt_w, int Ew, int B, int C, int in_h, int in_w, int out_h,
+                                        int out_w, float alpha, float scale, int dtype, void* stream) {
+  return rs_actbwd(y, gb, scratch, scratch_elems, blocks_needed, x, ref, idx_h, coef_h, cnt_h, Eh, idx_w, coef_w, cnt_w, Ew, B, C,
+                   in_h, in_w, out_h, out_w, alpha, scale, dtype, false, stream);
+}
+
+extern "C" int dgv2_resample_tab_actbwd_mask(void* y, float* gb, float* scratch, int64_t scratch_elems,
+                                             int64_t* blocks_needed, const void* x, const void* mask, const int* idx_h,
+                                             const float* coef_h, const int* cnt_h, int Eh, const int* idx_w,
+                                             const float* coef_w, const int* cnt_w, int Ew, int B, int C, int in_h, int in_w,
+                                             int out_h, int out_w, float alpha, float scale, int dtype, void* stream) {
+  return rs_actbwd(y, gb, scratch, scratch_elems, blocks_needed, x, mask, idx_h, coef_h, cnt_h, Eh, idx_w, coef_w, cnt_w, Ew, B, C,
+                   in_h, in_w, out_h, out_w, alpha, scale, dtype, true, stream);
+}
+
+extern "C" int dgv2_resample_tab_mask(void* y, void* mask, const void* x, const int* idx_h, const float* coef_h,
+                                      const int* cnt_h, int Eh, const int* idx_w, const float* coef_w, const int* cnt_w,
+                                      int Ew, int B, int C, int H, int W, int self_tap, void* stream) {
+  if (!y || !mask || !x || !idx_h || !coef_h || !cnt_h || !idx_w || !coef_w || !cnt_w) return DGV2_EINVAL;
+  if (B <= 0 || C <= 0 || H <= 0 || W <= 0 || Eh <= 0 || Ew <= 0) return DGV2_EINVAL;
+  static const bool no_stream = getenv("DGV2_NO_RSTREAM") != nullptr;
+  if (C % 32 || Ew > 4 || Eh > 64 || no_stream || !aligned16(x) || !aligned16(y)) return DGV2_ENOTSUP;
+  if (reinterpret_cast<uintptr_t>(mask) & 3) return DGV2_EINVAL;
+  int SH = H >= 32 ? 16 : (H >= 8 ? 8 : H);
+  while (SH > 1 && SH * Eh > 64) SH >>= 1;
+  const int64_t blocks = (int64_t)B * ((H + SH - 1) / SH) * (((int64_t)W * (C / 8) + 255) / 256);
+  if (blocks >= (1LL << 31)) return DGV2_EINVAL;
+  rs_launch_mask(false, Ew, (int)blocks, (hipStream_t)stream, (bf16_t*)y, (const bf16_t*)x, idx_h, coef_h, cnt_h, Eh, idx_w,
+                 coef_w, cnt_w, B, C, H, W, H, W, SH | (nt_output((int64_t)B * H * W * C * 2) ? (1 << 30) : 0),
+                 static_cast<uint8_t*>(mask), self_tap, 1.f, 1.f, nullptr);
   DGV2_RETURN_LAST();
 }
 
diff --git a/dusty-gan-v2_amd/csrc/stem.hip b/dusty-gan-v2_amd/csrc/stem.hip
--- a/dusty-gan-v2_amd/csrc/stem.hip
+++ b/dusty-gan-v2_amd/csrc/stem.hip
@@ -65,10 +65,10 @@
   }
 }
 
-template <typename T>
+template <typename T, bool MASK = false>
 __global__ __launch_bounds__(256) void stem_fwd4_kernel(T* __restrict__ y, const float* __restrict__ x,
                                                         const float* __restrict__ w, const float* __restrict__ bias,
-                                                        StemGeom g) {
+                                                        StemGeom g, uint8_t* __restrict__ mask = nullptr) {
   const int G = g.O / 8, W4 = g.W >> 2;
   const int64_t items = (int64_t)g.B * g.H * W4 * G;
   const int64_t stride = (int64_t)gridDim.x * blockDim.x;
@@ -110,6 +110,7 @@
         for (int j = 0; j < 8; ++j) o.set(j, f[j]);
         if (g.nt) o.store_nt(out + k * g.O);
         else o.store(out + k * g.O);
+        if constexpr (MASK) mask[(((int64_t)b * g.H + h) * g.W + wc + k) * G + grp] = (uint8_t)act_mask_byte(o.raw);
       } else {
         *reinterpret_cast<float4*>(out + k * g.O) = make_float4(f[0], f[1], f[2], f[3]);
         *reinterpret_cast<float4*>(out + k * g.O + 4) = make_float4(f[4], f[5], f[6], f[7]);
@@ -126,7 +127,7 @@
   int Hs, Ws;
 };
 
-template <typename T, bool SKIP>
+template <typename T, bool SKIP, bool MASK = false>
 __global__ __launch_bounds__(256) void stem_bwd_kernel(float* __restrict__ partial, float* __restrict__ gxb,
                                                        const T* __restrict__ gy, const T* __restrict__ y,
                                                        const float* __restrict__ x, const float* __restrict__ w,
@@ -213,9 +214,15 @@
     if constexpr (sizeof(T) == 2) {
       vec16<T> a, c;
       a.load(gy + px * g.O + grp * 8);
-      c.load(y + px * g.O + grp * 8);
-#pragma unroll
-      for (int j = 0; j < 8; ++j) gp[j] = (a.get(j) + gs[j]) * (c.get(j) > 0.f ? 1.f : g.alpha) * g.scale;
+      if constexpr (MASK) {
+        const unsigned m = reinterpret_cast<const uint8_t*>(y)[px * G + grp];
+#pragma unroll
+        for (int j = 0; j < 8; ++j) gp[j] = (a.get(j) + gs[j]) * ((m >> j) & 1u ? 1.f : g.alpha) * g.scale;
+      } else {
+        c.load(y + px * g.O + grp * 8);
+#pragma unroll
+        for (int j = 0; j < 8; ++j) gp[j] = (a.get(j) + gs[j]) * (c.get(j) > 0.f ? 1.f : g.alpha) * g.scale;
+      }
     } else {
 #pragma unroll
       for (int j = 0; j < 8; ++j) {
@@ -328,6 +335,18 @@
   DGV2_RETURN_LAST();
 }
 
+extern "C" int dgv2_stem_fwd_mask(void* y, void* mask, const float* x, const float* w, const float* bias, int B, int H, int W,
+                                  int O, int ring, float alpha, float scale, int ydtype, void* stream) {
+  if (!y || !mask || !x || !w || !stem_ok(B, H, W, O) || !aligned16(y) || (reinterpret_cast<uintptr_t>(mask) & 3)) return DGV2_EINVAL;
+  static const bool no4 = getenv("DGV2_STEM_NO4") != nullptr;
+  if (ydtype != DGV2_BF16 || O % 32 || W % 4 || !aligned16(x) || no4) return DGV2_ENOTSUP;
+  StemGeom g{B, H, W, O, ring, alpha, scale, nt_output((int64_t)B * H * W * O * 2) ? 1 : 0};
+  const int64_t items = (int64_t)B * H * (W / 4) * (O / 8);
+  const int grid = grid_for(items, 256, 256 * 32);
+  stem_fwd4_kernel<bf16_t, true><<<grid, 256, 0, (hipStream_t)stream>>>((bf16_t*)y, x, w, bias, g, (uint8_t*)mask);
+  DGV2_RETURN_LAST();
+}
+
 extern "C" int dgv2_stem_bwd_scratch(int64_t* elems, int B, int H, int W, int O) {
   if (!elems || !stem_ok(B, H, W, O)) return DGV2_EINVAL;
   *elems = (int64_t)STEM_BWD_BLOCKS * 3 * O + (int64_t)B * H * W * 2;
@@ -341,13 +360,15 @@
                             nullptr, nullptr, 0, 0, 0, B, H, W, O, ring, alpha, scale, dtype, stream);
 }
 
-extern "C" int dgv2_stem_bwd_skip(float* gx, float* gw, float* gb, float* scratch, int64_t scratch_elems, const void* gy,
-                                  const void* y, const float* x, const float* w, const void* gsk, const int* idx_h,
-                                  const float* coef_h, const int* cnt_h, int Eh, const int* idx_w, const float* coef_w,
-                                  const int* cnt_w, int Ew, int Hs, int Ws, int B, int H, int W, int O, int ring,
-                                  float alpha, float scale, int dtype, void* stream) {
+static int stem_bwd_impl(float* gx, float* gw, float* gb, float* scratch, int64_t scratch_elems, const void* gy, const void* y,
+                         const float* x, const float* w, const void* gsk, const int* idx_h, const float* coef_h,
+                         const int* cnt_h, int Eh, const int* idx_w, const float* coef_w, const int* cnt_w, int Ew, int Hs,
+                         int Ws, int B, int H, int W, int O, int ring, float alpha, float scale, int dtype, bool masked,
+                         void* stream) {
   if (!gw || !gb || !scratch || !gy || !y || !x || !w || !stem_ok(B, H, W, O)) return DGV2_EINVAL;
-  if (!aligned16(gy) || !aligned16(y) || !aligned16(scratch)) return DGV2_EINVAL;
+  if (masked && (dtype != DGV2_BF16 || O % 32)) return DGV2_ENOTSUP;
+  if (!aligned16(gy) || !aligned16(scratch)) return DGV2_EINVAL;
+  if (masked ? (reinterpret_cast<uintptr_t>(y) & 3) != 0 : !aligned16(y)) return DGV2_EINVAL;
   if (gsk && (!idx_h || !coef_h || !cnt_h || !idx_w || !coef_w || !cnt_w || Eh < 1 || Ew < 1 || Hs < 1 || Ws < 1 ||
               !aligned16(gsk)))
     return DGV2_EINVAL;
@@ -363,7 +384,10 @@
   hipStream_t st = (hipStream_t)stream;
   if (dtype == DGV2_BF16) {
     StemSkip<bf16_t> sk{(const bf16_t*)gsk, idx_h, coef_h, cnt_h, Eh, idx_w, coef_w, cnt_w, Ew, Hs, Ws};
-    if (gsk) stem_bwd_kernel<bf16_t, true><<<grid, 256, tab_bytes, st>>>(partial, gxb, (const bf16_t*)gy, (const bf16_t*)y, x, w, g, sk);
+    if (masked) {
+      if (gsk) stem_bwd_kernel<bf16_t, true, true><<<grid, 256, tab_bytes, st>>>(partial, gxb, (const bf16_t*)gy, (const bf16_t*)y, x, w, g, sk);
+      else stem_bwd_kernel<bf16_t, false, true><<<grid, 256, 0, st>>>(partial, gxb, (const bf16_t*)gy, (const bf16_t*)y, x, w, g, sk);
+    } else if (gsk) stem_bwd_kernel<bf16_t, true><<<grid, 256, tab_bytes, st>>>(partial, gxb, (const bf16_t*)gy, (const bf16_t*)y, x, w, g, sk);
     else stem_bwd_kernel<bf16_t, false><<<grid, 256, 0, st>>>(partial, gxb, (const bf16_t*)gy, (const bf16_t*)y, x, w, g, sk);
   } else if (dtype == DGV2_F32) {
     StemSkip<float> sk{(const float*)gsk, idx_h, coef_h, cnt_h, Eh, idx_w, coef_w, cnt_w, Ew, Hs, Ws};
@@ -376,3 +400,21 @@
   if (gx) stem_blur_adj_kernel<<<grid_for((int64_t)B * H * W, 256, 4096), 256, 0, st>>>(gx, gxb, g);
   DGV2_RETURN_LAST();
 }
+
+extern "C" int dgv2_stem_bwd_skip(float* gx, float* gw, float* gb, float* scratch, int64_t scratch_elems, const void* gy,
+                                  const void* y, const float* x, const float* w, const void* gsk, const int* idx_h,
+                                  const float* coef_h, const int* cnt_h, int Eh, const int* idx_w, const float* coef_w,
+                                  const int* cnt_w, int Ew, int Hs, int Ws, int B, int H, int W, int O, int ring,
+                                  float alpha, float scale, int dtype, void* stream) {
+  return stem_bwd_impl(gx, gw, gb, scratch, scratch_elems, gy, y, x, w, gsk, idx_h, coef_h, cnt_h, Eh, idx_w, coef_w, cnt_w, Ew,
+                       Hs, Ws, B, H, W, O, ring, alpha, scale, dtype, false, stream);
+}
+
+extern "C" int dgv2_stem_bwd_skip_mask(float* gx, float* gw, float* gb, float* scratch, int64_t scratch_elems, const void* gy,
+                                       const void* mask, const float* x, const float* w, const void* gsk, const int* idx_h,
+                                       const float* coef_h, const int* cnt_h, int Eh, const int* idx_w, const float* coef_w,
+                                       const int* cnt_w, int Ew, int Hs, int Ws, int B, int H, int W, int O, int ring,
+                                       float alpha, float scale, int dtype, void* stream) {
+  return stem_bwd_impl(gx, gw, gb, scratch, scratch_elems, gy, mask, x, w, gsk, idx_h, coef_h, cnt_h, Eh, idx_w, coef_w, cnt_w, Ew,
+                       Hs, Ws, B, H, W, O, ring, alpha, scale, dtype, true, stream);
+}
diff --git a/dusty-gan-v2_amd/dgv2_native/__init__.py b/dusty-gan-v2_amd/dgv2_native/__init__.py
--- a/dusty-gan-v2_amd/dgv2_native/__init__.py
+++ b/dusty-gan-v2_amd/dgv2_native/__init__.py
@@ -7,7 +7,7 @@
 LIB_PATH = os.environ.get("DGV2_LIB_PATH") or os.path.join(os.path.dirname(_HERE), "lib", "libdgv2.so")
 
 F32, BF16 = 0, 1
-ABI_VERSION = 49
+ABI_VERSION = 50
 
 _c_int, _c_i64, _c_f32, _c_ptr = ctypes.c_int, ctypes.c_int64, ctypes.c_float, ctypes.c_void_p
 
@@ -80,6 +80,15 @@
     "dgv2_fir_same_mfma": [_c_ptr] * 3 + [_c_int] * 4 + [_c_ptr],
     "dgv2_fir_same_mfma_actbwd": [_c_ptr, _c_ptr, _c_ptr, _c_i64, _c_ptr, _c_ptr, _c_ptr, _c_ptr] + [_c_int] * 4
                                  + [_c_f32, _c_f32, _c_ptr],
+    "dgv2_resample_tab_actbwd_mask": [_c_ptr, _c_ptr, _c_ptr, _c_i64, _c_ptr, _c_ptr, _c_ptr] + [_c_ptr] * 3 + [_c_int] + [_c_ptr] * 3
+                                     + [_c_int] * 7 + [_c_f32, _c_f32, _c_int, _c_ptr],
+    "dgv2_resample_tab_mask": [_c_ptr] * 6 + [_c_int] + [_c_ptr] * 3 + [_c_int] * 6 + [_c_ptr],
+    "dgv2_fir_same_mfma_mask": [_c_ptr] * 4 + [_c_int] * 4 + [_c_ptr],
+    "dgv2_fir_same_mfma_actbwd_mask": [_c_ptr, _c_ptr, _c_ptr, _c_i64, _c_ptr, _c_ptr, _c_ptr, _c_ptr] + [_c_int] * 4
+                                      + [_c_f32, _c_f32, _c_ptr],
+    "dgv2_stem_fwd_mask": [_c_ptr] * 5 + [_c_int] * 5 + [_c_f32, _c_f32, _c_int, _c_ptr],
+    "dgv2_stem_bwd_skip_mask": [_c_ptr] * 4 + [_c_i64] + [_c_ptr] * 8 + [_c_int] + [_c_ptr] * 3 + [_c_int] * 8 + [_c_f32, _c_f32,
+                                                                                                             _c_int, _c_ptr],
     "dgv2_resample_tab_sq": [_c_ptr] * 5 + [_c_int] + [_c_ptr] * 3 + [_c_int] * 10 + [_c_ptr, _c_int, _c_ptr, _c_ptr],
     "dgv2_bmm_tn_cat": [_c_ptr] * 4 + [_c_int] * 6 + [_c_ptr],
     "dgv2_lerp_list": [_c_ptr] * 3 + [_c_int, _c_f32, _c_ptr],
diff --git a/dusty-gan-v2_amd/gans/models/dusty_v2.py b/dusty-gan-v2_amd/gans/models/dusty_v2.py
--- a/dusty-gan-v2_amd/gans/models/dusty_v2.py
+++ b/dusty-gan-v2_amd/gans/models/dusty_v2.py
@@ -746,21 +746,22 @@
             i = 3
         else:
             x = ops.to_cl(h.float())
-        while i < len(layers):
-            low = (self.num_fp16_layers > i) or (self.num_fp16_layers == -1)
-            x = x.to(LOW if low else torch.float32)
-            layer = layers[i]
-            nxt = layers[i + 1] if i + 1 < len(layers) else None
-            if isinstance(layer, ops.Conv2d) and isinstance(nxt, ops.FusedLeakyReLU):
-                x = layer.forward_cl(x, act=nxt)
-                i += 2
-            elif isinstance(layer, ResidualBlock):
-                x = layer.forward_cl(x, bank=bank, fp8=fp8, xs=xs0)
-                xs0 = None
-                i += 1
-            else:
-                x = layer.forward_cl(x)
-                i += 1
+        with native.first_order_pass(not double_backward):
+            while i < len(layers):
+                low = (self.num_fp16_layers > i) or (self.num_fp16_layers == -1)
+                x = x.to(LOW if low else torch.float32)
+                layer = layers[i]
+                nxt = layers[i + 1] if i + 1 < len(layers) else None
+                if isinstance(layer, ops.Conv2d) and isinstance(nxt, ops.FusedLeakyReLU):
+                    x = layer.forward_cl(x, act=nxt)
+                    i += 2
+                elif isinstance(layer, ResidualBlock):
+                    x = layer.forward_cl(x, bank=bank, fp8=fp8, xs=xs0)
+                    xs0 = None
+                    i += 1
+                else:
+                    x = layer.forward_cl(x)
+                    i += 1
         if features_only:
             return x
         mb, conv, act1, _, lin1, act2, lin2 = self.epilogue
diff --git a/dusty-gan-v2_amd/gans/models/ops/native/conv.py b/dusty-gan-v2_amd/gans/models/ops/native/conv.py
--- a/dusty-gan-v2_amd/gans/models/ops/native/conv.py
+++ b/dusty-gan-v2_amd/gans/models/ops/native/conv.py
@@ -804,37 +804,85 @@
 _FUSED_ACTBWD = os.environ.get("DGV2_NO_FUSED_ACTBWD") is None
 
 
-def _resample_actbwd(g, out, spec, in_hw, alpha, scale):
-    if not _FUSED_ACTBWD or g.dtype != out.dtype:
-        return None
-    B, H, W, C = out.shape
+_ACT_MASK = os.environ.get("DGV2_NO_ACT_MASK") is None
+_FIRST_ORDER_PASS = [False]
+
+
+@contextlib.contextmanager
+def first_order_pass(on=True):
+    old = _FIRST_ORDER_PASS[0]
+    _FIRST_ORDER_PASS[0] = bool(on)
+    try:
+        yield
+    finally:
+        _FIRST_ORDER_PASS[0] = old
+
+
+def act_mask_ok(t):
+    return _ACT_MASK and t.is_cuda and t.dtype == torch.bfloat16 and t.ndim == 4 and t.shape[3] % 32 == 0
+
+
+def _actbwd_plan(shape, dtype, device, spec, masked):
+    B, H, W, C = shape
     Ho, Wo = spec.out_size(H, W)
-    (ih_idx, ih_coef, ih_cnt, Eh), (iw_idx, iw_coef, iw_cnt, Ew) = spec.tables(H, W, True, g.device)
+    (ih_idx, ih_coef, ih_cnt, Eh), (iw_idx, iw_coef, iw_cnt, Ew) = spec.tables(H, W, True, device)
     tabs = (N.ptr(ih_idx), N.ptr(ih_coef), N.ptr(ih_cnt), Eh, N.ptr(iw_idx), N.ptr(iw_coef), N.ptr(iw_cnt), Ew)
     bands = None
-    if _act_resample._FIR_MFMA and g.dtype == torch.bfloat16 and (Ho, Wo) == (H, W) and C % 32 == 0:
-        bands = spec.bands(H, W, True, g.device)
+    if _act_resample._FIR_MFMA and dtype == torch.bfloat16 and (Ho, Wo) == (H, W) and C % 32 == 0:
+        bands = spec.bands(H, W, True, device)
     mfma = bands is not None
-    entry = "dgv2_fir_same_mfma_actbwd" if mfma else "dgv2_resample_tab_actbwd"
+    entry = ("dgv2_fir_same_mfma_actbwd" if mfma else "dgv2_resample_tab_actbwd") + ("_mask" if masked else "")
     tabs = (N.ptr(bands),) if mfma else tabs
     geo = (B, C, H, W) if mfma else (B, C, Ho, Wo, H, W)
-    tail = (alpha, scale) if mfma else (alpha, scale, _dt(g))
-    key = (entry, B, H, W, C, Eh, Ew, _dt(g))
+    dt = N.BF16 if dtype == torch.bfloat16 else N.F32
+    key = (entry, B, H, W, C, Eh, Ew, dt)
     if key not in _ACTBWD_BLOCKS:
         nb = _ct.c_int64(0)
+        tail = (0.2, 1.0) if mfma else (0.2, 1.0, dt)
         ok = N.try_call(entry, None, None, None, 0, _ct.addressof(nb), None, None, *tabs, *geo, *tail, N.stream())
         _ACTBWD_BLOCKS[key] = nb.value if ok else 0
-    nblk = _ACTBWD_BLOCKS[key]
+    return entry, tabs, geo, mfma, _ACTBWD_BLOCKS[key]
+
+
+def _resample_actbwd(g, out, spec, in_hw, alpha, scale, mask=None):
+    shape, dtype = (tuple(out), g.dtype) if mask is not None else (tuple(out.shape), out.dtype)
+    if not _FUSED_ACTBWD or g.dtype != dtype:
+        return None
+    entry, tabs, geo, mfma, nblk = _actbwd_plan(shape, dtype, g.device, spec, mask is not None)
     if nblk == 0:
         return None
+    C = shape[3]
+    tail = (alpha, scale) if mfma else (alpha, scale, _dt(g))
     g = g.contiguous()
-    N.check(g, out)
-    gpre = torch.empty_like(out)
+    ref = out if mask is None else mask
+    N.check(g, ref)
+    gpre = torch.empty(shape, device=g.device, dtype=dtype)
     gb = torch.empty(C, device=g.device, dtype=torch.float32)
     scratch = torch.empty(nblk * C, device=g.device, dtype=torch.float32)
-    N.call(entry, N.ptr(gpre), N.ptr(gb), N.ptr(scratch), scratch.numel(), None, N.ptr(g), N.ptr(out), *tabs, *geo, *tail,
+    N.call(entry, N.ptr(gpre), N.ptr(gb), N.ptr(scratch), scratch.numel(), None, N.ptr(g), N.ptr(ref), *tabs, *geo, *tail,
            N.stream())
     return gpre, gb
+
+
+def _resample_mask(out, spec):
+    B, H, W, C = out.shape
+    if not (act_mask_ok(out) and _FUSED_ACTBWD and spec.out_size(H, W) == (H, W)):
+        return None
+    if _actbwd_plan(tuple(out.shape), out.dtype, out.device, spec, True)[4] == 0:
+        return None
+    y = torch.empty_like(out)
+    mask = torch.empty((B, H, W, C // 32), device=out.device, dtype=torch.int32)
+    bands = spec.bands(H, W, False, out.device) if _act_resample._FIR_MFMA else None
+    if bands is not None and N.try_call("dgv2_fir_same_mfma_mask", N.ptr(y), N.ptr(mask), N.ptr(out), N.ptr(bands), B, C, H, W,
+                                        N.stream()):
+        return y, mask
+    (ih, chh, nh, Eh), (iw, cw, nw, Ew) = spec.tables(H, W, False, out.device)
+    k, up, down, p0, _ = spec.axes[1]
+    self_tap = p0 if (up == 1 and down == 1 and 0 <= p0 < k) else -1
+    if N.try_call("dgv2_resample_tab_mask", N.ptr(y), N.ptr(mask), N.ptr(out), N.ptr(ih), N.ptr(chh), N.ptr(nh), Eh, N.ptr(iw),
+                  N.ptr(cw), N.ptr(nw), Ew, B, C, H, W, self_tap, N.stream()):
+        return y, mask
+    return None
 
 
 class _Conv(Function):
@@ -861,9 +909,15 @@
             x = x.contiguous()
             wc, w8 = _weights(ctx, w, x.dtype)
             out = _conv_fwd_raw(x, wc, ep.geom, bias, act, alpha, scale, resid, w8, ep.x_exact)
-        ctx.save_for_backward(x, w, *(() if ep.act is None else (out,)))
+        ym = None
+        if ep.act is not None and ep.down is not None and not ep.q8 and _FIRST_ORDER_PASS[0]:
+            ym = _resample_mask(out, ep.down)
+        ctx.mask_shape = None if ym is None else tuple(out.shape)
+        ctx.save_for_backward(x, w, *(() if ep.act is None else (out if ym is None else ym[1],)))
         ctx.ep = ep
-        if ep.down is None:
+        if ym is not None:
+            y = (ym[0],)
+        elif ep.down is None:
             y = (out,)
         elif ep.q8:
             from .fp8 import _handle, _resample_q8_raw
@@ -890,7 +944,14 @@
         if ep.act is not None:
             out, (alpha, scale) = out[0], ep.act
             fused = None
-            if ep.down is not None:
+            if ctx.mask_shape is not None:
+                if torch.is_grad_enabled():
+                    raise RuntimeError("dgv2: this conv node kept an activation mask (native.first_order_pass): its "
+                                       "backward cannot be differentiated again")
+                fused = _resample_actbwd(gy.to(x.dtype), ctx.mask_shape, ep.down, ctx.mask_shape[1:3], alpha, scale, mask=out)
+                if fused is None:
+                    raise RuntimeError("dgv2: no masked activation-backward kernel covers a shape its forward accepted")
+            elif ep.down is not None:
                 in_hw = tuple(out.shape[1:3])
                 if not torch.is_grad_enabled():
                     fused = _resample_actbwd(gy.to(out.dtype), out, ep.down, in_hw, alpha, scale)
diff --git a/dusty-gan-v2_amd/gans/models/ops/native/stem_tail_ada.py b/dusty-gan-v2_amd/gans/models/ops/native/stem_tail_ada.py
--- a/dusty-gan-v2_amd/gans/models/ops/native/stem_tail_ada.py
+++ b/dusty-gan-v2_amd/gans/models/ops/native/stem_tail_ada.py
@@ -7,6 +7,7 @@
 import dgv2_native as N
 from .act_resample import *
 from .modgemm import *
+from . import conv as _conv
 from .conv import *
 
 
@@ -22,9 +23,18 @@
         b32 = bias.detach().float().contiguous()
         y = torch.empty((B, H, W_, O), device=x.device, dtype=out_dtype)
         N.check(x3, w32, b32)
-        N.call("dgv2_stem_fwd", N.ptr(y), N.ptr(x3), N.ptr(w32), N.ptr(b32), B, H, W_, O, int(ring), alpha, scale,
-               _dt(y), N.stream())
-        ctx.save_for_backward(x3, w32, y)
+        mask = None
+        if _conv.act_mask_ok(y):
+            mask = torch.empty((B, H, W_, O // 32), device=x.device, dtype=torch.int32)
+            if not N.try_call("dgv2_stem_fwd_mask", N.ptr(y), N.ptr(mask), N.ptr(x3), N.ptr(w32), N.ptr(b32), B, H, W_, O,
+                              int(ring), alpha, scale, _dt(y), N.stream()):
+                mask = None
+        if mask is None:
+            N.call("dgv2_stem_fwd", N.ptr(y), N.ptr(x3), N.ptr(w32), N.ptr(b32), B, H, W_, O, int(ring), alpha, scale,
+                   _dt(y), N.stream())
+        ctx.masked = mask is not None
+        ctx.y_meta = (y.dtype, tuple(y.shape))
+        ctx.save_for_backward(x3, w32, y if mask is None else mask)
         ctx.cfg = (ctx_hw, ring, alpha, scale, tuple(x.shape), w.shape, down)
         if down is None:
             return y
@@ -37,9 +47,10 @@
         x3, w32, y = ctx.saved_tensors
         (H, W_), ring, alpha, scale, xshape, wshape, down = ctx.cfg
         B, O = x3.shape[0], w32.shape[0]
+        ydtype, yshape = ctx.y_meta
         if gy is None:
-            gy = torch.zeros_like(y)
-        gy = gy.contiguous().to(y.dtype)
+            gy = torch.zeros(yshape, device=y.device, dtype=ydtype)
+        gy = gy.contiguous().to(ydtype)
         key = (B, H, W_, O)
         if key not in _STEM_SCRATCH:
             n = _ct.c_int64(0)
@@ -50,16 +61,20 @@
         gb = torch.empty(O, device=gy.device, dtype=torch.float32)
         gx = torch.empty((B, H * W_), device=gy.device, dtype=torch.float32) if ctx.needs_input_grad[0] else None
         if gsk is not None:
-            gsk = gsk.contiguous().to(y.dtype)
+            gsk = gsk.contiguous().to(ydtype)
             Hs, Ws = down.out_size(H, W_)
             (ih, chh, nh, Eh), (iw, cw, nw, Ew) = down.tables(H, W_, True, gy.device)
             N.check(gsk)
-            N.call("dgv2_stem_bwd_skip", N.ptr(gx), N.ptr(gw), N.ptr(gb), N.ptr(scratch), scratch.numel(), N.ptr(gy), N.ptr(y),
+            N.call("dgv2_stem_bwd_skip_mask" if ctx.masked else "dgv2_stem_bwd_skip", N.ptr(gx), N.ptr(gw), N.ptr(gb), N.ptr(scratch), scratch.numel(), N.ptr(gy), N.ptr(y),
                    N.ptr(x3), N.ptr(w32), N.ptr(gsk), N.ptr(ih), N.ptr(chh), N.ptr(nh), Eh, N.ptr(iw), N.ptr(cw), N.ptr(nw), Ew,
-                   Hs, Ws, B, H, W_, O, int(ring), alpha, scale, _dt(y), N.stream())
+                   Hs, Ws, B, H, W_, O, int(ring), alpha, scale, _dt(gy), N.stream())
+        elif ctx.masked:
+            N.call("dgv2_stem_bwd_skip_mask", N.ptr(gx), N.ptr(gw), N.ptr(gb), N.ptr(scratch), scratch.numel(), N.ptr(gy),
+                   N.ptr(y), N.ptr(x3), N.ptr(w32), None, None, None, None, 0, None, None, None, 0, 0, 0, B, H, W_, O, int(ring),
+                   alpha, scale, _dt(gy), N.stream())
         else:
             N.call("dgv2_stem_bwd", N.ptr(gx), N.ptr(gw), N.ptr(gb), N.ptr(scratch), scratch.numel(), N.ptr(gy), N.ptr(y),
-                   N.ptr(x3), N.ptr(w32), B, H, W_, O, int(ring), alpha, scale, _dt(y), N.stream())
+                   N.ptr(x3), N.ptr(w32), B, H, W_, O, int(ring), alpha, scale, _dt(gy), N.stream())
         return (None if gx is None else gx.reshape(xshape)), gw.reshape(wshape), gb, None, None, None, None, None
 
 
diff --git a/include/dgv2.h b/include/dgv2.h
--- a/include/dgv2.h
+++ b/include/dgv2.h
@@ -15,6 +15,8 @@
 
 #define DGV2_STATUS_X_INEXACT 1
 #define DGV2_STATUS_FIR_TABLE 2
+
+#define DGV2_ACT_MASK_BYTES(B, H, W, C) ((int64_t)(B) * (H) * (W) * ((C) / 8))
 
 int dgv2_abi_version(void);
 
@@ -69,6 +71,15 @@
                              int Ew, int B, int C, int in_h, int in_w, int out_h, int out_w, float alpha,
                              float scale, int dtype, void* stream);
 
+int dgv2_resample_tab_actbwd_mask(void* y, float* gb, float* scratch, int64_t scratch_elems, int64_t* blocks_needed,
+                                  const void* x, const void* mask, const int* idx_h, const float* coef_h,
+                                  const int* cnt_h, int Eh, const int* idx_w, const float* coef_w, const int* cnt_w,
+                                  int Ew, int B, int C, int in_h, int in_w, int out_h, int out_w, float alpha,
+                                  float scale, int dtype, void* stream);
+int dgv2_resample_tab_mask(void* y, void* mask, const void* x, const int* idx_h, const float* coef_h, const int* cnt_h,
+                           int Eh, const int* idx_w, const float* coef_w, const int* cnt_w, int Ew, int B, int C,
+                           int H, int W, int self_tap, void* stream);
+
 int dgv2_fir_same_mfma_prep(void* bands, int64_t bands_bytes, int64_t* bytes_needed, const int* idx_h, const float* coef_h,
                             const int* cnt_h, int Eh, const int* idx_w, const float* coef_w, const int* cnt_w, int Ew,
                             int H, int W, int* status, void* stream);
@@ -76,6 +87,10 @@
 int dgv2_fir_same_mfma_actbwd(void* y, float* gb, float* scratch, int64_t scratch_elems, int64_t* blocks_needed,
                               const void* x, const void* ref, const void* bands, int B, int C, int H, int W, float alpha,
                               float scale, void* stream);
+int dgv2_fir_same_mfma_mask(void* y, void* mask, const void* x, const void* bands, int B, int C, int H, int W, void* stream);
+int dgv2_fir_same_mfma_actbwd_mask(void* y, float* gb, float* scratch, int64_t scratch_elems, int64_t* blocks_needed,
+                                   const void* x, const void* mask, const void* bands, int B, int C, int H, int W,
+                                   float alpha, float scale, void* stream);
 
 int dgv2_fourier_feature(void* out, const float* angle, const float* shift,
                          const float* freqs, const float* phase,
@@ -272,6 +287,13 @@
                        const float* x, const float* w, const void* gsk, const int* idx_h, const float* coef_h,
                        const int* cnt_h, int Eh, const int* idx_w, const float* coef_w, const int* cnt_w, int Ew, int Hs,
                        int Ws, int B, int H, int W, int O, int ring, float alpha, float scale, int dtype, void* stream);
+int dgv2_stem_fwd_mask(void* y, void* mask, const float* x, const float* w, const float* bias, int B, int H, int W, int O,
+                       int ring, float alpha, float scale, int ydtype, void* stream);
+int dgv2_stem_bwd_skip_mask(float* gx, float* gw, float* gb, float* scratch, int64_t scratch_elems, const void* gy,
+                            const void* mask, const float* x, const float* w, const void* gsk, const int* idx_h,
+                            const float* coef_h, const int* cnt_h, int Eh, const int* idx_w, const float* coef_w,
+                            const int* cnt_w, int Ew, int Hs, int Ws, int B, int H, int W, int O, int ring, float alpha,
+                            float scale, int dtype, void* stream);
 
 int dgv2_gen_tail_fwd(float* image, float* image_orig, float* logit, float* mask,
                       const float* skip, const float* shift, const float* u,
```

Result: slower. 5284 range-images/s (-1.3%).
